# skygazer42/realtime-video-analytics-32streams

Hardware: AMD Instinct MI355X
Metric: aggregate detected FPS across streams + p99 per-frame latency, 32x1080p30 (higher is better)
Workload: dtype f16

## Files before the change

### include/rva.h

```cpp
#ifndef RVA_H
#define RVA_H

#include <stdint.h>

#ifdef __cplusplus
extern "C" {
#endif

#define RVA_ABI_VERSION 1

enum rva_status {
    RVA_OK = 0,
    RVA_ERR_ARG = 1,
    RVA_ERR_HIP = 2,
    RVA_ERR_CAPACITY = 3,
    RVA_ERR_UNAVAILABLE = 4
};

enum rva_dtype { RVA_F16 = 0, RVA_F32 = 1, RVA_F64 = 2  };

typedef struct rva_ctx rva_ctx;
typedef struct rva_tracker rva_tracker;
typedef void *rva_stream_t;

int rva_abi_version(void);
int rva_create(int device, rva_ctx **out);
void rva_destroy(rva_ctx *ctx);
const char *rva_last_error(const rva_ctx *ctx);

int rva_reserve(rva_ctx *ctx, int batch, int anchors);

typedef struct rva_letterbox {
    int32_t src_w, src_h;
    int32_t dst_w, dst_h;
    int32_t new_w, new_h;
    int32_t pad_left, pad_top;
    double scale;
} rva_letterbox;

int rva_letterbox_meta(int src_w, int src_h, int dst_w, int dst_h, rva_letterbox *out);

#define RVA_MAX_BATCH 64

int rva_preprocess_nv12_batch(rva_ctx *ctx, const void *const *y_ptrs, const void *const *uv_ptrs,
                              const int32_t *pitches, int n, int src_w, int src_h, void *out,
                              int out_dtype, int dst_w, int dst_h, rva_letterbox *meta_out,
                              rva_stream_t stream);

int rva_preprocess_nv12_content_batch(rva_ctx *ctx, const void *const *y_ptrs, const void *const *uv_ptrs,
                                      const int32_t *pitches, int n, int src_w, int src_h, void *out,
                                      int out_dtype, int dst_w, int dst_h, rva_letterbox *meta_out,
                                      rva_stream_t stream);

int rva_preprocess_bgr_batch(rva_ctx *ctx, const void *const *frames, const int32_t *row_bytes, int n,
                             int src_w, int src_h, void *out, int out_dtype, int dst_w, int dst_h,
                             rva_letterbox *meta_out, rva_stream_t stream);

int rva_profile_next_preprocess(rva_ctx *ctx, void *start_event, void *stop_event);

int rva_preprocess_clip_nv12_batch(rva_ctx *ctx, const void *const *y_ptrs, const void *const *uv_ptrs,
                                   const int32_t *pitches, int n, int src_w, int src_h, void *out,
                                   int out_dtype, int dst_w, int dst_h, rva_stream_t stream);

int rva_preprocess_clip_bgr_batch(rva_ctx *ctx, const void *const *frames, const int32_t *row_bytes,
                                  int n, int src_w, int src_h, void *out, int out_dtype, int dst_w,
                                  int dst_h, rva_stream_t stream);

enum rva_frame_norm { RVA_NORM_IMAGENET_F32 = 0, RVA_NORM_VIDEO_F32 = 1, RVA_NORM_IMAGENET_F64 = 2 };
enum rva_frame_layout { RVA_LAYOUT_NCHW = 0, RVA_LAYOUT_CNHW = 1 };
int rva_preprocess_frames_nv12_batch(rva_ctx *ctx, const void *const *y_ptrs, const void *const *uv_ptrs,
                                     const int32_t *pitches, int n, int src_w, int src_h, void *out,
                                     int out_dtype, int dst_w, int dst_h, int norm, int layout,
                                     rva_stream_t stream);
int rva_preprocess_frames_bgr_batch(rva_ctx *ctx, const void *const *frames, const int32_t *row_bytes,
                                    int n, int src_w, int src_h, void *out, int out_dtype, int dst_w,
                                    int dst_h, int norm, int layout, rva_stream_t stream);

int rva_postprocess_batch(rva_ctx *ctx, const void *raw, int raw_dtype, int batch, int d1, int d2,
                          double conf_thr, double iou_thr, const int32_t *classes, int n_classes,
                          const rva_letterbox *metas, int n_metas, int max_det, float *out_boxes,
                          float *out_scores, int32_t *out_cls, int32_t *out_anchor, int32_t *out_cand,
                          int32_t *out_counts, int32_t *out_ncand, rva_stream_t stream);

int rva_postprocess_boxes_batch(rva_ctx *ctx, const void *raw, int raw_dtype, const float *boxes, int batch, int channels,
                                int anchors, double conf_thr, double iou_thr, const int32_t *classes, int n_classes,
                                const rva_letterbox *metas, int n_metas, int max_det, float *out_boxes, float *out_scores,
                                int32_t *out_cls, int32_t *out_anchor, int32_t *out_cand, int32_t *out_counts,
                                int32_t *out_ncand, rva_stream_t stream);

int rva_post_status(rva_ctx *ctx, rva_stream_t stream, int *flags);

int rva_post_filter_stats(rva_ctx *ctx, rva_stream_t stream, int *binned_images);

int rva_tracker_create(rva_ctx *ctx, int n_streams, int capacity, int max_age, double max_iou_distance,
                       int min_hits, rva_tracker **out);
void rva_tracker_destroy(rva_tracker *trk);

int rva_tracker_update_f32(rva_tracker *trk, const int32_t *slot_of_stream, const float *boxes,
                           const float *scores, const int32_t *cls, const int32_t *counts, int max_det,
                           double filter_thr, rva_stream_t stream);

int rva_tracker_update_gated_f32(rva_tracker *trk, const int32_t *slot_of_stream, const float *boxes,
                                 const float *scores, const int32_t *cls, const int32_t *counts, int max_det,
                                 double filter_thr, const int32_t *motion_counts, const int32_t *motion_row,
                                 rva_stream_t stream);

int rva_tracker_set_gates(rva_tracker *trk, const int32_t *adaptive_enabled, const int32_t *max_process_every,
                          const int32_t *idle_tolerance, const int32_t *motion_min_count, int reset_state);

int rva_tracker_update_f64(rva_tracker *trk, const int32_t *active, const int32_t *offsets,
                           const double *boxes, const double *conf, const int64_t *cls,
                           rva_stream_t stream);

int rva_tracker_set_box_scale(rva_tracker *trk, const double *scales);

int32_t *rva_tracker_new_counts(rva_tracker *trk);

int rva_tracker_assign_ids(rva_tracker *trk, const int32_t *counts_all, int n_global,
                           const int32_t *global_index, rva_stream_t stream);

int rva_tracker_read(rva_tracker *trk, int stream_id, int cap, int64_t *ids, int32_t *cls, int32_t *age,
                     int32_t *hits, double *conf, double *boxes, int32_t *last_det, int32_t *n,
                     rva_stream_t stream);

int rva_tracker_read_all(rva_tracker *trk, int64_t *ids, int32_t *cls, int32_t *age, int32_t *hits,
                         double *conf, double *boxes, int32_t *last_det, int32_t *counts,
                         rva_stream_t stream);

#define RVA_SNAPSHOT_SLOTS 8
int rva_tracker_snapshot_async(rva_tracker *trk, int slot, rva_stream_t stream);
int rva_tracker_snapshot_fetch(rva_tracker *trk, int slot, int wait, int64_t *ids, int32_t *cls, int32_t *age,
                               int32_t *hits, double *conf, double *boxes, int32_t *last_det,
                               int32_t *counts);

int rva_tracker_snapshot_status(rva_tracker *trk, int slot, int32_t *emitted, int32_t *processed, int32_t *flags);

int rva_tracker_state(rva_tracker *trk, int64_t *next_id, int *flags, rva_stream_t stream);
int rva_tracker_set_next_id(rva_tracker *trk, int64_t next_id, rva_stream_t stream);

int rva_conv_cout_pad(int Cout);
int rva_conv_num_variants(void);
const char *rva_conv_variant_name(int variant);
int rva_conv2d_nhwc_f16(rva_ctx *ctx, const void *in, int ldi, const void *weights, const float *bias,
                        void *out, int ldo, const void *residual, int ldr, int batch, int H, int W, int Cin,
                        int Cout, int ksize, int stride, int act, rva_stream_t stream);
int rva_conv2d_nhwc_f16_v(rva_ctx *ctx, const void *in, int ldi, const void *weights, const float *bias,
                          void *out, int ldo, const void *residual, int ldr, int batch, int H, int W, int Cin,
                          int Cout, int ksize, int stride, int act, int variant, rva_stream_t stream);
int rva_conv2d_nhwc_f16_rows(rva_ctx *ctx, const void *in, int ldi, const void *weights, const float *bias,
                             void *out, int ldo, const void *residual, int ldr, int batch, int H, int W, int Cin,
                             int Cout, int ksize, int stride, int act, int variant, int y0, int y1, rva_stream_t stream);
int rva_conv_rows_through(int k, int stride, int H_in, int lo, int hi, int32_t *out_lo, int32_t *out_hi);
int rva_conv1x1_upcat_f16(rva_ctx *ctx, const void *low, int ld_low, int c_low, const void *skip, int ld_skip,
                          int c_skip, const void *weights, const float *bias, void *out, int ldo, int batch,
                          int H, int W, int Cout, int act, int variant, rva_stream_t stream);
int rva_conv1x1_head_f16(rva_ctx *ctx, const void *in, int ldi, const void *weights, const float *bias, int batch,
                         int H, int W, int Cin, int Cout, int mode, void *out, int nc, int anchors_total,
                         int anchor_offset, float stride_px, int variant, rva_stream_t stream);
int rva_conv1x1_head_box32_f16(rva_ctx *ctx, const void *in, int ldi, const void *weights, const float *bias, int batch,
                               int H, int W, int Cin, void *out, float *boxes32, int nc, int anchors_total, int anchor_offset,
                               float stride_px, int variant, rva_stream_t stream);
int rva_stem_conv_f16(rva_ctx *ctx, const void *in_planar, const void *weights, const float *bias,
                      void *out, int ldo, int batch, int H, int W, int Cout, rva_stream_t stream);

int rva_c2f_pair32_f16(rva_ctx *ctx, const void *in, int ldi, const void *w1, const float *b1, const void *w2, const float *b2, void *out,
                       int ldo, int batch, int H, int W, rva_stream_t stream);

int rva_stem2_f16(rva_ctx *ctx, const void *in_planar, const void *w1, const float *b1, const void *w2, const float *b2,
                  void *out, int ldo, int batch, int H, int W, rva_stream_t stream);
int rva_stem2_f16_rows(rva_ctx *ctx, const void *in_planar, const void *w1, const float *b1, const void *w2, const float *b2,
                       void *out, int ldo, int batch, int H, int W, int y0, int y1, rva_stream_t stream);

int rva_sppf_pool3_nhwc_f16(rva_ctx *ctx, const void *in, int ldi, void *out1, void *out2, void *out3, int ldo,
                            int batch, int H, int W, int C, rva_stream_t stream);
int rva_maxpool5_nhwc_f16(rva_ctx *ctx, const void *in, int ldi, void *out, int ldo, int batch, int H,
                          int W, int C, rva_stream_t stream);
int rva_upsample2x_nhwc_f16(rva_ctx *ctx, const void *in, int ldi, void *out, int ldo, int batch, int H,
                            int W, int C, rva_stream_t stream);
int rva_yolo_head_f16(rva_ctx *ctx, const void *box_logits, int ldb, const void *cls_logits, int ldc,
                      void *out, int batch, int h, int w, int nc, int anchors_total, int anchor_offset,
                      float stride, rva_stream_t stream);
int rva_yolo_head3_f16(rva_ctx *ctx, const void *const *box_logits, const int32_t *ldb, const void *const *cls_logits,
                       const int32_t *ldc, void *out, int batch, const int32_t *h, const int32_t *w, int nc,
                       int anchors_total, const float *strides, rva_stream_t stream);
int rva_yolo_head_box32_f16(rva_ctx *ctx, const void *box_logits, int ldb, const void *cls_logits, int ldc, void *out,
                            float *boxes32, int batch, int h, int w, int nc, int anchors_total, int anchor_offset, float stride,
                            rva_stream_t stream);
int rva_yolo_head3_box32_f16(rva_ctx *ctx, const void *const *box_logits, const int32_t *ldb, const void *const *cls_logits,
                             const int32_t *ldc, void *out, float *boxes32, int batch, const int32_t *h, const int32_t *w, int nc,
                             int anchors_total, const float *strides, rva_stream_t stream);

int rva_conv_f32_num_variants(void);
int rva_conv2d_nhwc_f32_v(rva_ctx *ctx, const void *in, int ldi, const void *weights, const float *bias,
                          void *out, int ldo, const void *residual, int ldr, int batch, int H, int W, int Cin,
                          int Cout, int ksize, int stride, int act, int variant, rva_stream_t stream);
int rva_stem_conv_f32(rva_ctx *ctx, const void *in_planar, const void *weights, const float *bias,
                      void *out, int ldo, int batch, int H, int W, int Cout, rva_stream_t stream);
int rva_maxpool5_nhwc_f32(rva_ctx *ctx, const void *in, int ldi, void *out, int ldo, int batch, int H,
                          int W, int C, rva_stream_t stream);
int rva_upsample2x_nhwc_f32(rva_ctx *ctx, const void *in, int ldi, void *out, int ldo, int batch, int H,
                            int W, int C, rva_stream_t stream);
int rva_yolo_head_f32(rva_ctx *ctx, const void *box_logits, int ldb, const void *cls_logits, int ldc,
                      void *out, int batch, int h, int w, int nc, int anchors_total, int anchor_offset,
                      float stride, rva_stream_t stream);

#define RVA_PLAN_NO_STEM2 1
#define RVA_PLAN_NO_CIN_PAD 2
#define RVA_PLAN_NO_PAIR32 4
#define RVA_PLAN_F32 8
#define RVA_PLAN_BOX_F32 16
typedef struct rva_yolov8_plan rva_yolov8_plan;
typedef struct rva_yolov8_desc {
    int32_t batch, height, width;
    int32_t widths[5];
    int32_t depth_backbone[4];
    int32_t depth_head;
    int32_t nc, reg_max;
    int32_t n_convs;
    int32_t flags;
} rva_yolov8_desc;
typedef struct rva_conv_weights {
    const float *weight;
    const float *bias;
    int32_t cout, cin, k, stride;
} rva_conv_weights;
int rva_yolov8_plan_create(rva_ctx *ctx, const rva_yolov8_desc *desc, const rva_conv_weights *convs, rva_yolov8_plan **out);
void rva_yolov8_plan_destroy(rva_yolov8_plan *plan);
int rva_yolov8_plan_info(const rva_yolov8_plan *plan, int32_t *anchors, int32_t *out_rows, int32_t *n_steps, int32_t *n_tunable,
                         int32_t *quiet_step);
int rva_yolov8_plan_output_layout(const rva_yolov8_plan *plan, int64_t *total_bytes, int64_t *boxes_offset);
int rva_yolov8_plan_run(rva_yolov8_plan *plan, const void *input, void *output, rva_stream_t stream);
int rva_yolov8_plan_run_lanes(rva_yolov8_plan *plan, const void *input, void *output, rva_stream_t stream, rva_stream_t side1,
                              rva_stream_t side2);
int rva_yolov8_plan_run_range(rva_yolov8_plan *plan, const void *input, void *output, int first, int last, rva_stream_t stream);
int rva_yolov8_plan_tunable_desc(const rva_yolov8_plan *plan, int index, char *buf, int len);
int rva_yolov8_plan_launch_tunable(rva_yolov8_plan *plan, int index, int variant, void *output, rva_stream_t stream);
int rva_yolov8_plan_set_variant(rva_yolov8_plan *plan, int index, int variant);
int rva_yolov8_plan_get_variant(const rva_yolov8_plan *plan, int index);
int rva_yolov8_plan_set_static_rows(rva_yolov8_plan *plan, int top, int bottom);
int rva_yolov8_plan_run_n(rva_yolov8_plan *plan, const void *input, void *output, int n, rva_stream_t stream);
int rva_yolov8_plan_run_lanes_n(rva_yolov8_plan *plan, const void *input, void *output, int n, rva_stream_t stream, rva_stream_t side1,
                                rva_stream_t side2);
int rva_yolov8_plan_run_range_n(rva_yolov8_plan *plan, const void *input, void *output, int n, int first, int last, rva_stream_t stream);
int rva_yolov8_plan_primed_images(const rva_yolov8_plan *plan);
int rva_yolov8_plan_step_rows(const rva_yolov8_plan *plan, int step, int32_t *y0, int32_t *y1);

typedef struct rva_cnnlstm_plan rva_cnnlstm_plan;
typedef struct rva_cnnlstm_desc {
    int32_t height, width;
    int32_t frames;
    int32_t hidden, classes;
    int32_t max_clips;
} rva_cnnlstm_desc;
typedef struct rva_cnnlstm_weights {
    const float *conv1_w, *conv1_b, *conv2_w, *conv2_b;
    const float *w_ih1, *b1, *w_hh1;
    const float *w_ih2, *w_hh2, *b2;
    const float *head_w, *head_b;
} rva_cnnlstm_weights;
int rva_cnnlstm_plan_create(rva_ctx *ctx, const rva_cnnlstm_desc *desc, const rva_cnnlstm_weights *weights, rva_cnnlstm_plan **out);
void rva_cnnlstm_plan_destroy(rva_cnnlstm_plan *plan);
int rva_cnnlstm_plan_info(const rva_cnnlstm_plan *plan, int32_t *pooled_h, int32_t *pooled_w, int32_t *conv2_tiles,
                          int32_t *n_launches);
int rva_cnnlstm_plan_run(rva_cnnlstm_plan *plan, const void *frames, const int32_t *frame_index, int n_clips, void *logits,
                         rva_stream_t stream);
int rva_cnnlstm_plan_run_post(rva_cnnlstm_plan *plan, const void *logits, const int32_t *rows, int n_rows, int max_det,
                              void *scores, void *cls, void *boxes, void *counts, rva_stream_t stream);
enum rva_cnnlstm_stage {
    RVA_CNNLSTM_STAGE_POOLED = 0, RVA_CNNLSTM_STAGE_PARTIAL = 1, RVA_CNNLSTM_STAGE_FEAT = 2, RVA_CNNLSTM_STAGE_GX = 3,
    RVA_CNNLSTM_STAGE_H1 = 4, RVA_CNNLSTM_STAGE_H2 = 5
};
int rva_cnnlstm_plan_stage(rva_cnnlstm_plan *plan, int stage, int n_clips, void *dst, int64_t dst_floats, int64_t *n_floats,
                           rva_stream_t stream);

typedef struct rva_cnnlstm_f16_plan rva_cnnlstm_f16_plan;
int rva_cnnlstm_f16_plan_create(rva_ctx *ctx, const rva_cnnlstm_desc *desc, const rva_cnnlstm_weights *weights,
                                rva_cnnlstm_f16_plan **out);
void rva_cnnlstm_f16_plan_destroy(rva_cnnlstm_f16_plan *plan);
int rva_cnnlstm_f16_plan_info(const rva_cnnlstm_f16_plan *plan, int32_t *pooled_h, int32_t *pooled_w, int32_t *conv2_tiles,
                              int32_t *n_launches);
int rva_cnnlstm_f16_plan_run(rva_cnnlstm_f16_plan *plan, const void *frames, const int32_t *frame_index, int n_clips, void *logits,
                             rva_stream_t stream);
int rva_cnnlstm_f16_plan_run_post(rva_cnnlstm_f16_plan *plan, const void *logits, const int32_t *rows, int n_rows, int max_det,
                                  void *scores, void *cls, void *boxes, void *counts, rva_stream_t stream);
int rva_cnnlstm_f16_plan_stage(rva_cnnlstm_f16_plan *plan, int stage, int n_clips, void *dst, int64_t dst_elems, int64_t *n_elems,
                               rva_stream_t stream);

typedef struct rva_cnn3d_plan rva_cnn3d_plan;
typedef struct rva_cnn3d_desc {
    int32_t height, width;
    int32_t frames;
    int32_t classes;
    int32_t max_clips;
} rva_cnn3d_desc;
typedef struct rva_cnn3d_weights {
    const float *conv1_w, *conv1_b, *conv2_w, *conv2_b, *conv3_w, *conv3_b;
    const float *head_w, *head_b;
} rva_cnn3d_weights;
int rva_cnn3d_plan_create(rva_ctx *ctx, const rva_cnn3d_desc *desc, const rva_cnn3d_weights *weights, rva_cnn3d_plan **out);
void rva_cnn3d_plan_destroy(rva_cnn3d_plan *plan);
int rva_cnn3d_plan_info(const rva_cnn3d_plan *plan, int32_t *pool1, int32_t *pool2, int32_t *tiles, int32_t *n_launches);
int rva_cnn3d_plan_run(rva_cnn3d_plan *plan, const void *frames, const int32_t *frame_index, int n_clips, void *logits,
                       rva_stream_t stream);
int rva_cnn3d_plan_run_post(rva_cnn3d_plan *plan, const void *logits, const int32_t *rows, int n_rows, int max_det,
                            void *scores, void *cls, void *boxes, void *counts, rva_stream_t stream);
enum rva_cnn3d_stage { RVA_CNN3D_STAGE_ACT1 = 0, RVA_CNN3D_STAGE_ACT2 = 1, RVA_CNN3D_STAGE_PARTIAL = 2, RVA_CNN3D_STAGE_FEAT = 3 };
int rva_cnn3d_plan_stage(rva_cnn3d_plan *plan, int stage, int n_clips, void *dst, int64_t dst_floats, int64_t *n_floats,
                         rva_stream_t stream);

typedef struct rva_cnn3d_f16_plan rva_cnn3d_f16_plan;
int rva_cnn3d_f16_plan_create(rva_ctx *ctx, const rva_cnn3d_desc *desc, const rva_cnn3d_weights *weights, rva_cnn3d_f16_plan **out);
void rva_cnn3d_f16_plan_destroy(rva_cnn3d_f16_plan *plan);
int rva_cnn3d_f16_plan_info(const rva_cnn3d_f16_plan *plan, int32_t *pool1, int32_t *pool2, int32_t *tiles, int32_t *n_launches);
int rva_cnn3d_f16_plan_run(rva_cnn3d_f16_plan *plan, const void *frames, const int32_t *frame_index, int n_clips, void *logits,
                           rva_stream_t stream);
int rva_cnn3d_f16_plan_run_post(rva_cnn3d_f16_plan *plan, const void *logits, const int32_t *rows, int n_rows, int max_det,
                                void *scores, void *cls, void *boxes, void *counts, rva_stream_t stream);
int rva_cnn3d_f16_plan_stage(rva_cnn3d_f16_plan *plan, int stage, int n_clips, void *dst, int64_t dst_elems, int64_t *n_elems,
                             rva_stream_t stream);

typedef struct rva_resnet_plan rva_resnet_plan;
typedef struct rva_resnet_desc {
    int32_t height, width;
    int32_t classes, top_k;
    int32_t max_frames;
} rva_resnet_desc;
typedef struct rva_resnet_conv {
    const float *w, *b;
} rva_resnet_conv;
typedef struct rva_resnet_weights {
    const float *stem_w, *stem_b;
    rva_resnet_conv conv[19];
    const float *head_w, *head_b;
} rva_resnet_weights;
int rva_resnet_plan_create(rva_ctx *ctx, const rva_resnet_desc *desc, const rva_resnet_weights *weights, rva_resnet_plan **out);
void rva_resnet_plan_destroy(rva_resnet_plan *plan);
int rva_resnet_plan_info(const rva_resnet_plan *plan, int32_t *maps, int64_t *workspace_bytes, int32_t *n_launches);
int rva_resnet_plan_run(rva_resnet_plan *plan, const void *frames, const int32_t *frame_index, int n, void *logits,
                        rva_stream_t stream);
int rva_resnet_plan_run_post(rva_resnet_plan *plan, const void *logits, const int32_t *rows, int n_rows, int max_det,
                             void *scores, void *cls, void *boxes, void *counts, rva_stream_t stream);
enum rva_resnet_stage {
    RVA_RESNET_STAGE_POOLED = 0, RVA_RESNET_STAGE_MID0 = 1, RVA_RESNET_STAGE_DOWN2 = 9, RVA_RESNET_STAGE_DOWN4 = 10,
    RVA_RESNET_STAGE_DOWN6 = 11, RVA_RESNET_STAGE_OUT0 = 12, RVA_RESNET_STAGE_FEAT = 20
};
int rva_resnet_plan_stage(rva_resnet_plan *plan, int stage, int n, void *dst, int64_t dst_floats, int64_t *n_floats,
                          rva_stream_t stream);

int rva_motion_nv12_batch(rva_ctx *ctx, const void *const *y_ptrs, const void *const *uv_ptrs,
                          const int32_t *pitches, const void *const *prev_blur, void *const *blur_out, int n,
                          int w, int h, int32_t *counts, rva_stream_t stream);
int rva_motion_nv12_masked_batch(rva_ctx *ctx, const void *const *y_ptrs, const void *const *uv_ptrs,
                                 const int32_t *pitches, const void *const *masks, const void *const *prev_blur,
                                 void *const *blur_out, int n, int w, int h, int32_t *counts, rva_stream_t stream);
int rva_motion_bgr_batch(rva_ctx *ctx, const void *const *frames, const int32_t *row_bytes,
                         const void *const *prev_blur, void *const *blur_out, int n, int w, int h, int32_t *counts,
                         rva_stream_t stream);

int rva_preprocess_nv12_masked_batch(rva_ctx *ctx, const void *const *y_ptrs, const void *const *uv_ptrs,
                                     const int32_t *pitches, const void *const *masks, int n, int src_w, int src_h,
                                     void *out, int out_dtype, int dst_w, int dst_h, rva_letterbox *meta_out,
                                     rva_stream_t stream);
int rva_resize_nv12_to_bgr_batch(rva_ctx *ctx, const void *const *y_ptrs, const void *const *uv_ptrs,
                                 const int32_t *pitches, const void *const *masks, int n, int src_w, int src_h,
                                 void *out_bgr, int dst_w, int dst_h, rva_stream_t stream);

int rva_preview_nv12(rva_ctx *ctx, const void *y, const void *uv, int pitch, int src_w, int src_h, int ratio,
                     void *out_bgr, int dst_w, int dst_h, const int32_t *rects, const uint8_t *colors, int n_rects,
                     const int32_t *glyphs, int n_glyphs, int glyph_scale, rva_stream_t stream);

typedef struct rva_preview_item {
    const void *y, *uv;
    void *out_bgr;
    int32_t pitch, src_w, src_h, ratio, dst_w, dst_h;
    int32_t rect_first, n_rects, glyph_first, n_glyphs;
} rva_preview_item;
int rva_preview_nv12_batch(rva_ctx *ctx, const void *table_host, void *table_dev, int64_t table_bytes, int n, int n_rects,
                           int n_glyphs, int glyph_scale, rva_stream_t stream);

typedef struct rva_decoder rva_decoder;
enum rva_codec { RVA_CODEC_H264 = 0, RVA_CODEC_HEVC = 1 };

int rva_decode_available(char *detail, int detail_len);

int rva_decoder_create(rva_ctx *ctx, int codec, int num_surfaces, rva_decoder **out);
void rva_decoder_destroy(rva_decoder *dec);

int rva_decoder_feed(rva_decoder *dec, const uint8_t *data, int size, int64_t pts, int end_of_stream);

int rva_decoder_next_frame(rva_decoder *dec, void **y, void **uv, int32_t *pitch, int32_t *width, int32_t *height,
                           int64_t *pts, int32_t *pic_index);
int rva_decoder_release(rva_decoder *dec, int pic_index);

int rva_jpeg_max_bytes(int width, int height);
int rva_jpeg_encode_bgr(rva_ctx *ctx, const void *bgr, int pitch, int width, int height, int quality, void *out,
                        int out_capacity, int32_t *out_size, rva_stream_t stream);
int rva_jpeg_status(rva_ctx *ctx, rva_stream_t stream, int *flags);

typedef struct rva_jpeg_batch rva_jpeg_batch;
int rva_jpeg_batch_create(rva_ctx *ctx, int max_images, int max_width, int max_height, rva_jpeg_batch **out);
void rva_jpeg_batch_destroy(rva_jpeg_batch *enc);
int rva_jpeg_batch_encode(rva_jpeg_batch *enc, int n, const void *const *bgr, const int32_t *pitch, const int32_t *width,
                          const int32_t *height, const int32_t *quality, void *out, int64_t out_capacity, int32_t *out_sizes,
                          rva_stream_t stream);

#ifdef __cplusplus
}
#endif
#endif
```

### realtime_video_analytics_32streams_amd/_native.py

```python
from __future__ import annotations

import ctypes as C
import os
import shutil
import subprocess
from pathlib import Path
from typing import Optional

PKG = Path(__file__).resolve().parent
ROOT = PKG.parent
CSRC = PKG / "csrc"
LIB_PATH = Path(os.environ["RVA_LIB_PATH"]) if os.environ.get("RVA_LIB_PATH") else PKG / "librva.so"
SOURCES = ["rva_ctx.hip", "rva_preprocess.hip", "rva_postprocess.hip", "rva_tracker.hip", "rva_conv.hip", "rva_conv_f32.hip", "rva_plan.hip", "rva_clip.hip",
           "rva_clip3d.hip", "rva_clip3d_f16.hip", "rva_clip_f16.hip", "rva_resnet.hip", "rva_gates.hip", "rva_decode.hip", "rva_preview.hip", "rva_jpeg.hip"]
HIPCC_FLAGS = ["--offload-arch=gfx950", "-O3", "-fPIC", "-shared", "-std=c++17", "-ffp-contract=off",
               "-Wall", "-Wno-unused-function"]

RVA_OK, RVA_ERR_ARG, RVA_ERR_HIP, RVA_ERR_CAPACITY, RVA_ERR_UNAVAILABLE = range(5)
RVA_F16, RVA_F32, RVA_F64 = 0, 1, 2
NORM_IMAGENET_F32, NORM_VIDEO_F32, NORM_IMAGENET_F64 = 0, 1, 2
LAYOUT_NCHW, LAYOUT_CNHW = 0, 1
RVA_MAX_BATCH = 64
RVA_CODEC_H264, RVA_CODEC_HEVC = 0, 1


class Letterbox(C.Structure):
    _fields_ = [("src_w", C.c_int32), ("src_h", C.c_int32), ("dst_w", C.c_int32), ("dst_h", C.c_int32),
                ("new_w", C.c_int32), ("new_h", C.c_int32), ("pad_left", C.c_int32), ("pad_top", C.c_int32),
                ("scale", C.c_double)]

    def as_meta(self) -> dict:
        return {"orig_shape": (self.src_h, self.src_w), "scale": self.scale, "pad": (self.pad_left, self.pad_top)}


class YoloV8Desc(C.Structure):
    _fields_ = [("batch", C.c_int32), ("height", C.c_int32), ("width", C.c_int32), ("widths", C.c_int32 * 5),
                ("depth_backbone", C.c_int32 * 4), ("depth_head", C.c_int32), ("nc", C.c_int32), ("reg_max", C.c_int32),
                ("n_convs", C.c_int32), ("flags", C.c_int32)]


class ConvWeights(C.Structure):
    _fields_ = [("weight", C.POINTER(C.c_float)), ("bias", C.POINTER(C.c_float)), ("cout", C.c_int32), ("cin", C.c_int32),
                ("k", C.c_int32), ("stride", C.c_int32)]


class CnnLstmDesc(C.Structure):
    _fields_ = [("height", C.c_int32), ("width", C.c_int32), ("frames", C.c_int32), ("hidden", C.c_int32), ("classes", C.c_int32),
                ("max_clips", C.c_int32)]


class CnnLstmWeights(C.Structure):
    NAMES = ("conv1_w", "conv1_b", "conv2_w", "conv2_b", "w_ih1", "b1", "w_hh1", "w_ih2", "w_hh2", "b2", "head_w", "head_b")
    _fields_ = [(n, C.POINTER(C.c_float)) for n in NAMES]


class Cnn3dDesc(C.Structure):
    _fields_ = [("height", C.c_int32), ("width", C.c_int32), ("frames", C.c_int32), ("classes", C.c_int32), ("max_clips", C.c_int32)]


class Cnn3dWeights(C.Structure):
    NAMES = ("conv1_w", "conv1_b", "conv2_w", "conv2_b", "conv3_w", "conv3_b", "head_w", "head_b")
    _fields_ = [(n, C.POINTER(C.c_float)) for n in NAMES]


class ResNetDesc(C.Structure):
    _fields_ = [("height", C.c_int32), ("width", C.c_int32), ("classes", C.c_int32), ("top_k", C.c_int32), ("max_frames", C.c_int32)]


class ResNetWeights(C.Structure):
    NAMES = ("stem_w", "stem_b") + tuple(f"c{i}_{x}" for i in range(19) for x in "wb") + ("head_w", "head_b")
    _fields_ = [(n, C.POINTER(C.c_float)) for n in NAMES]


class PreviewItem(C.Structure):
    _fields_ = [("y", C.c_void_p), ("uv", C.c_void_p), ("out_bgr", C.c_void_p)] + [
        (n, C.c_int32) for n in ("pitch", "src_w", "src_h", "ratio", "dst_w", "dst_h", "rect_first", "n_rects", "glyph_first", "n_glyphs")]


RVA_PLAN_NO_STEM2 = 1
RVA_PLAN_NO_CIN_PAD = 2
RVA_PLAN_NO_PAIR32 = 4
RVA_PLAN_F32 = 8
RVA_PLAN_BOX_F32 = 16


def _stale() -> bool:
    if not LIB_PATH.exists():
        return True
    t = LIB_PATH.stat().st_mtime
    deps = [CSRC / s for s in SOURCES] + [CSRC / "rva_internal.h", CSRC / "rva_mfma_f32.h", CSRC / "rva_mfma_f16.h", ROOT / "include" / "rva.h"]
    return any(d.exists() and d.stat().st_mtime > t for d in deps)


def build(force: bool = False, verbose: bool = False) -> Path:
    if not force and not _stale():
        return LIB_PATH
    hipcc = shutil.which("hipcc") or "/opt/rocm/bin/hipcc"
    if not Path(hipcc).exists():
        if LIB_PATH.exists():
            return LIB_PATH
        raise RuntimeError("hipcc not found and librva.so is not built")
    cmd = [hipcc, *HIPCC_FLAGS, f"-I{ROOT / 'include'}", "-o", str(LIB_PATH), *[str(CSRC / s) for s in SOURCES], "-ldl"]
    if verbose:
        print(" ".join(cmd))
    subprocess.check_call(cmd, cwd=str(CSRC))
    return LIB_PATH


_LIB: Optional[C.CDLL] = None
_P = C.c_void_p


def lib() -> C.CDLL:
    global _LIB
    if _LIB is not None:
        return _LIB
    if not LIB_PATH.exists():
        if os.environ.get("RVA_NO_AUTOBUILD"):
            raise RuntimeError(f"{LIB_PATH} is missing: run `python -c 'import __graft_entry__ as g; g.build()'`")
        build()
    try:
        L = C.CDLL(str(LIB_PATH))
    except OSError as exc:
        raise RuntimeError(f"cannot load {LIB_PATH}: {exc}. The HIP hot path has no CPU fallback.") from exc
    i32p, i64p, f32p, f64p = (C.POINTER(C.c_int32), C.POINTER(C.c_int64), C.POINTER(C.c_float), C.POINTER(C.c_double))
    pp = C.POINTER(_P)
    sig = {
        "rva_abi_version": (C.c_int, []),
        "rva_create": (C.c_int, [C.c_int, C.POINTER(_P)]),
        "rva_destroy": (None, [_P]),
        "rva_last_error": (C.c_char_p, [_P]),
        "rva_reserve": (C.c_int, [_P, C.c_int, C.c_int]),
        "rva_letterbox_meta": (C.c_int, [C.c_int] * 4 + [C.POINTER(Letterbox)]),
        "rva_preprocess_nv12_batch": (C.c_int, [_P, pp, pp, i32p, C.c_int, C.c_int, C.c_int, _P, C.c_int, C.c_int,
                                                C.c_int, C.POINTER(Letterbox), _P]),
        "rva_preprocess_nv12_content_batch": (C.c_int, [_P, pp, pp, i32p, C.c_int, C.c_int, C.c_int, _P, C.c_int, C.c_int,
                                                        C.c_int, C.POINTER(Letterbox), _P]),
        "rva_preprocess_bgr_batch": (C.c_int, [_P, pp, i32p, C.c_int, C.c_int, C.c_int, _P, C.c_int, C.c_int, C.c_int,
                                               C.POINTER(Letterbox), _P]),
        "rva_preprocess_clip_nv12_batch": (C.c_int, [_P, pp, pp, i32p, C.c_int, C.c_int, C.c_int, _P, C.c_int, C.c_int,
                                                     C.c_int, _P]),
        "rva_preprocess_clip_bgr_batch": (C.c_int, [_P, pp, i32p, C.c_int, C.c_int, C.c_int, _P, C.c_int, C.c_int,
                                                    C.c_int, _P]),
        "rva_profile_next_preprocess": (C.c_int, [_P, _P, _P]),
        "rva_preprocess_frames_nv12_batch": (C.c_int, [_P, pp, pp, i32p, C.c_int, C.c_int, C.c_int, _P, C.c_int, C.c_int,
                                                       C.c_int, C.c_int, C.c_int, _P]),
        "rva_preprocess_frames_bgr_batch": (C.c_int, [_P, pp, i32p, C.c_int, C.c_int, C.c_int, _P, C.c_int, C.c_int,
                                                      C.c_int, C.c_int, C.c_int, _P]),
        "rva_postprocess_batch": (C.c_int, [_P, _P, C.c_int, C.c_int, C.c_int, C.c_int, C.c_double, C.c_double, i32p,
                                            C.c_int, C.POINTER(Letterbox), C.c_int, C.c_int, _P, _P, _P, _P, _P, _P, _P,
                                            _P]),
        "rva_postprocess_boxes_batch": (C.c_int, [_P, _P, C.c_int, _P, C.c_int, C.c_int, C.c_int, C.c_double, C.c_double, i32p,
                                                  C.c_int, C.POINTER(Letterbox), C.c_int, C.c_int, _P, _P, _P, _P, _P, _P, _P,
                                                  _P]),
        "rva_post_status": (C.c_int, [_P, _P, C.POINTER(C.c_int)]),
        "rva_post_filter_stats": (C.c_int, [_P, _P, C.POINTER(C.c_int)]),
        "rva_tracker_create": (C.c_int, [_P, C.c_int, C.c_int, C.c_int, C.c_double, C.c_int, C.POINTER(_P)]),
        "rva_tracker_destroy": (None, [_P]),
        "rva_tracker_update_f32": (C.c_int, [_P, i32p, _P, _P, _P, _P, C.c_int, C.c_double, _P]),
        "rva_tracker_update_f64": (C.c_int, [_P, i32p, i32p, _P, _P, _P, _P]),
        "rva_tracker_update_gated_f32": (C.c_int, [_P, i32p, _P, _P, _P, _P, C.c_int, C.c_double, _P, i32p, _P]),
        "rva_tracker_set_gates": (C.c_int, [_P, i32p, i32p, i32p, i32p, C.c_int]),
        "rva_tracker_snapshot_status": (C.c_int, [_P, C.c_int, _P, _P, C.POINTER(C.c_int32)]),
        "rva_tracker_new_counts": (_P, [_P]),
        "rva_tracker_assign_ids": (C.c_int, [_P, _P, C.c_int, i32p, _P]),
        "rva_tracker_read": (C.c_int, [_P, C.c_int, C.c_int, _P, _P, _P, _P, _P, _P, _P, i32p, _P]),
        "rva_tracker_read_all": (C.c_int, [_P, _P, _P, _P, _P, _P, _P, _P, _P, _P]),
        "rva_tracker_snapshot_async": (C.c_int, [_P, C.c_int, _P]),
        "rva_tracker_snapshot_fetch": (C.c_int, [_P, C.c_int, C.c_int, _P, _P, _P, _P, _P, _P, _P, _P]),
        "rva_tracker_state": (C.c_int, [_P, i64p, C.POINTER(C.c_int), _P]),
        "rva_tracker_set_next_id": (C.c_int, [_P, C.c_int64, _P]),
        "rva_preview_nv12": (C.c_int, [_P, _P, _P, C.c_int, C.c_int, C.c_int, C.c_int, _P, C.c_int, C.c_int, _P, _P, C.c_int, _P, C.c_int,
                                       C.c_int, _P]),
        "rva_decode_available": (C.c_int, [C.c_char_p, C.c_int]),
        "rva_decoder_create": (C.c_int, [_P, C.c_int, C.c_int, C.POINTER(_P)]),
        "rva_decoder_destroy": (None, [_P]),
        "rva_decoder_feed": (C.c_int, [_P, C.c_char_p, C.c_int, C.c_int64, C.c_int]),
        "rva_decoder_next_frame": (C.c_int, [_P, C.POINTER(_P), C.POINTER(_P), i32p, i32p, i32p, i64p, i32p]),
        "rva_decoder_release": (C.c_int, [_P, C.c_int]),
        "rva_motion_nv12_batch": (C.c_int, [_P, pp, pp, i32p, pp, pp, C.c_int, C.c_int, C.c_int, _P, _P]),
        "rva_motion_nv12_masked_batch": (C.c_int, [_P, pp, pp, i32p, pp, pp, pp, C.c_int, C.c_int, C.c_int, _P, _P]),
        "rva_motion_bgr_batch": (C.c_int, [_P, pp, i32p, pp, pp, C.c_int, C.c_int, C.c_int, _P, _P]),
        "rva_preprocess_nv12_masked_batch": (C.c_int, [_P, pp, pp, i32p, pp, C.c_int, C.c_int, C.c_int, _P, C.c_int, C.c_int,
                                                       C.c_int, C.POINTER(Letterbox), _P]),
        "rva_resize_nv12_to_bgr_batch": (C.c_int, [_P, pp, pp, i32p, pp, C.c_int, C.c_int, C.c_int, _P, C.c_int, C.c_int, _P]),
        "rva_tracker_set_box_scale": (C.c_int, [_P, f64p]),
        "rva_conv_cout_pad": (C.c_int, [C.c_int]),
        "rva_conv_num_variants": (C.c_int, []),
        "rva_conv_variant_name": (C.c_char_p, [C.c_int]),
        "rva_conv2d_nhwc_f16": (C.c_int, [_P, _P, C.c_int, _P, _P, _P, C.c_int, _P, C.c_int] + [C.c_int] * 8 + [_P]),
        "rva_conv2d_nhwc_f16_v": (C.c_int, [_P, _P, C.c_int, _P, _P, _P, C.c_int, _P, C.c_int] + [C.c_int] * 9 + [_P]),
        "rva_conv2d_nhwc_f16_rows": (C.c_int, [_P, _P, C.c_int, _P, _P, _P, C.c_int, _P, C.c_int] + [C.c_int] * 11 + [_P]),
        "rva_conv_rows_through": (C.c_int, [C.c_int] * 5 + [i32p, i32p]),
        "rva_stem2_f16_rows": (C.c_int, [_P, _P, _P, _P, _P, _P, _P, C.c_int, C.c_int, C.c_int, C.c_int, C.c_int, C.c_int, _P]),
        "rva_stem_conv_f16": (C.c_int, [_P, _P, _P, _P, _P, C.c_int, C.c_int, C.c_int, C.c_int, C.c_int, _P]),
        "rva_stem2_f16": (C.c_int, [_P, _P, _P, _P, _P, _P, _P, C.c_int, C.c_int, C.c_int, C.c_int, _P]),
        "rva_c2f_pair32_f16": (C.c_int, [_P, _P, C.c_int, _P, _P, _P, _P, _P, C.c_int, C.c_int, C.c_int, C.c_int, _P]),
        "rva_conv1x1_head_f16": (C.c_int, [_P, _P, C.c_int, _P, _P, C.c_int, C.c_int, C.c_int, C.c_int, C.c_int, C.c_int, _P, C.c_int,
                                           C.c_int, C.c_int, C.c_float, C.c_int, _P]),
        "rva_conv1x1_head_box32_f16": (C.c_int, [_P, _P, C.c_int, _P, _P, C.c_int, C.c_int, C.c_int, C.c_int, _P, _P, C.c_int,
                                                 C.c_int, C.c_int, C.c_float, C.c_int, _P]),
        "rva_yolo_head_box32_f16": (C.c_int, [_P, _P, C.c_int, _P, C.c_int, _P, _P, C.c_int, C.c_int, C.c_int, C.c_int, C.c_int,
                                              C.c_int, C.c_float, _P]),
        "rva_yolo_head3_box32_f16": (C.c_int, [_P, pp, i32p, pp, i32p, _P, _P, C.c_int, i32p, i32p, C.c_int, C.c_int,
                                               C.POINTER(C.c_float), _P]),
        "rva_conv1x1_upcat_f16": (C.c_int, [_P, _P, C.c_int, C.c_int, _P, C.c_int, C.c_int, _P, _P, _P, C.c_int, C.c_int, C.c_int,
                                            C.c_int, C.c_int, C.c_int, C.c_int, _P]),
        "rva_yolo_head3_f16": (C.c_int, [_P, pp, i32p, pp, i32p, _P, C.c_int, i32p, i32p, C.c_int, C.c_int, C.POINTER(C.c_float), _P]),
        "rva_sppf_pool3_nhwc_f16": (C.c_int, [_P, _P, C.c_int, _P, _P, _P, C.c_int, C.c_int, C.c_int, C.c_int, C.c_int, _P]),
        "rva_maxpool5_nhwc_f16": (C.c_int, [_P, _P, C.c_int, _P, C.c_int, C.c_int, C.c_int, C.c_int, C.c_int, _P]),
        "rva_upsample2x_nhwc_f16": (C.c_int, [_P, _P, C.c_int, _P, C.c_int, C.c_int, C.c_int, C.c_int, C.c_int, _P]),
        "rva_yolo_head_f16": (C.c_int, [_P, _P, C.c_int, _P, C.c_int, _P, C.c_int, C.c_int, C.c_int, C.c_int, C.c_int,
                                        C.c_int, C.c_float, _P]),
        "rva_conv_f32_num_variants": (C.c_int, []),
        "rva_conv2d_nhwc_f32_v": (C.c_int, [_P, _P, C.c_int, _P, _P, _P, C.c_int, _P, C.c_int] + [C.c_int] * 9 + [_P]),
        "rva_stem_conv_f32": (C.c_int, [_P, _P, _P, _P, _P, C.c_int, C.c_int, C.c_int, C.c_int, C.c_int, _P]),
        "rva_maxpool5_nhwc_f32": (C.c_int, [_P, _P, C.c_int, _P, C.c_int, C.c_int, C.c_int, C.c_int, C.c_int, _P]),
        "rva_upsample2x_nhwc_f32": (C.c_int, [_P, _P, C.c_int, _P, C.c_int, C.c_int, C.c_int, C.c_int, C.c_int, _P]),
        "rva_yolo_head_f32": (C.c_int, [_P, _P, C.c_int, _P, C.c_int, _P, C.c_int, C.c_int, C.c_int, C.c_int, C.c_int,
                                        C.c_int, C.c_float, _P]),
        "rva_yolov8_plan_create": (C.c_int, [_P, C.POINTER(YoloV8Desc), C.POINTER(ConvWeights), C.POINTER(_P)]),
        "rva_yolov8_plan_destroy": (None, [_P]),
        "rva_yolov8_plan_info": (C.c_int, [_P, i32p, i32p, i32p, i32p, i32p]),
        "rva_yolov8_plan_output_layout": (C.c_int, [_P, i64p, i64p]),
        "rva_yolov8_plan_run": (C.c_int, [_P, _P, _P, _P]),
        "rva_yolov8_plan_run_lanes": (C.c_int, [_P, _P, _P, _P, _P, _P]),
        "rva_yolov8_plan_run_range": (C.c_int, [_P, _P, _P, C.c_int, C.c_int, _P]),
        "rva_yolov8_plan_tunable_desc": (C.c_int, [_P, C.c_int, C.c_char_p, C.c_int]),
        "rva_yolov8_plan_launch_tunable": (C.c_int, [_P, C.c_int, C.c_int, _P, _P]),
        "rva_yolov8_plan_set_variant": (C.c_int, [_P, C.c_int, C.c_int]),
        "rva_yolov8_plan_get_variant": (C.c_int, [_P, C.c_int]),
        "rva_yolov8_plan_set_static_rows": (C.c_int, [_P, C.c_int, C.c_int]),
        "rva_yolov8_plan_step_rows": (C.c_int, [_P, C.c_int, i32p, i32p]),
        "rva_yolov8_plan_run_n": (C.c_int, [_P, _P, _P, C.c_int, _P]),
        "rva_yolov8_plan_run_lanes_n": (C.c_int, [_P, _P, _P, C.c_int, _P, _P, _P]),
        "rva_yolov8_plan_run_range_n": (C.c_int, [_P, _P, _P, C.c_int, C.c_int, C.c_int, _P]),
        "rva_yolov8_plan_primed_images": (C.c_int, [_P]),
        "rva_cnnlstm_plan_create": (C.c_int, [_P, C.POINTER(CnnLstmDesc), C.POINTER(CnnLstmWeights), C.POINTER(_P)]),
        "rva_cnnlstm_plan_destroy": (None, [_P]),
        "rva_cnnlstm_plan_info": (C.c_int, [_P, i32p, i32p, i32p, i32p]),
        "rva_cnnlstm_plan_run": (C.c_int, [_P, _P, _P, C.c_int, _P, _P]),
        "rva_cnnlstm_plan_run_post": (C.c_int, [_P, _P, _P, C.c_int, C.c_int, _P, _P, _P, _P, _P]),
        "rva_cnnlstm_plan_stage": (C.c_int, [_P, C.c_int, C.c_int, _P, C.c_int64, i64p, _P]),
        "rva_cnnlstm_f16_plan_create": (C.c_int, [_P, C.POINTER(CnnLstmDesc), C.POINTER(CnnLstmWeights), C.POINTER(_P)]),
        "rva_cnnlstm_f16_plan_destroy": (None, [_P]),
        "rva_cnnlstm_f16_plan_info": (C.c_int, [_P, i32p, i32p, i32p, i32p]),
        "rva_cnnlstm_f16_plan_run": (C.c_int, [_P, _P, _P, C.c_int, _P, _P]),
        "rva_cnnlstm_f16_plan_run_post": (C.c_int, [_P, _P, _P, C.c_int, C.c_int, _P, _P, _P, _P, _P]),
        "rva_cnnlstm_f16_plan_stage": (C.c_int, [_P, C.c_int, C.c_int, _P, C.c_int64, i64p, _P]),
        "rva_cnn3d_plan_create": (C.c_int, [_P, C.POINTER(Cnn3dDesc), C.POINTER(Cnn3dWeights), C.POINTER(_P)]),
        "rva_cnn3d_plan_destroy": (None, [_P]),
        "rva_cnn3d_plan_info": (C.c_int, [_P, i32p, i32p, i32p, i32p]),
        "rva_cnn3d_plan_run": (C.c_int, [_P, _P, _P, C.c_int, _P, _P]),
        "rva_cnn3d_plan_run_post": (C.c_int, [_P, _P, _P, C.c_int, C.c_int, _P, _P, _P, _P, _P]),
        "rva_cnn3d_plan_stage": (C.c_int, [_P, C.c_int, C.c_int, _P, C.c_int64, i64p, _P]),
        "rva_cnn3d_f16_plan_create": (C.c_int, [_P, C.POINTER(Cnn3dDesc), C.POINTER(Cnn3dWeights), C.POINTER(_P)]),
        "rva_cnn3d_f16_plan_destroy": (None, [_P]),
        "rva_cnn3d_f16_plan_info": (C.c_int, [_P, i32p, i32p, i32p, i32p]),
        "rva_cnn3d_f16_plan_run": (C.c_int, [_P, _P, _P, C.c_int, _P, _P]),
        "rva_cnn3d_f16_plan_run_post": (C.c_int, [_P, _P, _P, C.c_int, C.c_int, _P, _P, _P, _P, _P]),
        "rva_cnn3d_f16_plan_stage": (C.c_int, [_P, C.c_int, C.c_int, _P, C.c_int64, i64p, _P]),
        "rva_resnet_plan_create": (C.c_int, [_P, C.POINTER(ResNetDesc), C.POINTER(ResNetWeights), C.POINTER(_P)]),
        "rva_resnet_plan_destroy": (None, [_P]),
        "rva_resnet_plan_info": (C.c_int, [_P, i32p, i64p, i32p]),
        "rva_resnet_plan_run": (C.c_int, [_P, _P, _P, C.c_int, _P, _P]),
        "rva_resnet_plan_run_post": (C.c_int, [_P, _P, _P, C.c_int, C.c_int, _P, _P, _P, _P, _P]),
        "rva_resnet_plan_stage": (C.c_int, [_P, C.c_int, C.c_int, _P, C.c_int64, i64p, _P]),
        "rva_jpeg_max_bytes": (C.c_int, [C.c_int, C.c_int]),
        "rva_jpeg_encode_bgr": (C.c_int, [_P, _P, C.c_int, C.c_int, C.c_int, C.c_int, _P, C.c_int, _P, _P]),
        "rva_jpeg_status": (C.c_int, [_P, _P, C.POINTER(C.c_int)]),
        "rva_jpeg_batch_create": (C.c_int, [_P, C.c_int, C.c_int, C.c_int, C.POINTER(_P)]),
        "rva_jpeg_batch_destroy": (None, [_P]),
        "rva_jpeg_batch_encode": (C.c_int, [_P, C.c_int, pp, i32p, i32p, i32p, i32p, _P, C.c_int64, _P, _P]),
        "rva_preview_nv12_batch": (C.c_int, [_P, _P, _P, C.c_int64, C.c_int, C.c_int, C.c_int, C.c_int, _P]),
    }
    for name, (res, args) in sig.items():
        fn = getattr(L, name)
        fn.restype = res
        fn.argtypes = args
    if L.rva_abi_version() != 1:
        raise RuntimeError("librva.so ABI version mismatch; rebuild it")
    _LIB = L
    return L


EXPORTS = [
    "rva_abi_version", "rva_create", "rva_destroy", "rva_last_error", "rva_reserve", "rva_letterbox_meta",
    "rva_preprocess_nv12_batch", "rva_preprocess_nv12_content_batch", "rva_preprocess_bgr_batch", "rva_preprocess_clip_nv12_batch",
    "rva_preprocess_clip_bgr_batch", "rva_profile_next_preprocess", "rva_preprocess_frames_nv12_batch", "rva_preprocess_frames_bgr_batch", "rva_postprocess_batch", "rva_post_status", "rva_post_filter_stats", "rva_tracker_create",
    "rva_tracker_destroy", "rva_tracker_update_f32", "rva_tracker_update_f64", "rva_tracker_update_gated_f32",
    "rva_tracker_set_gates", "rva_tracker_snapshot_status", "rva_tracker_new_counts",
    "rva_tracker_assign_ids", "rva_tracker_read", "rva_tracker_read_all", "rva_tracker_snapshot_async",
    "rva_tracker_snapshot_fetch", "rva_tracker_state",
    "rva_tracker_set_next_id", "rva_preview_nv12", "rva_decode_available", "rva_decoder_create", "rva_decoder_destroy", "rva_decoder_feed",
    "rva_decoder_next_frame", "rva_decoder_release", "rva_motion_nv12_batch", "rva_motion_nv12_masked_batch", "rva_motion_bgr_batch",
    "rva_preprocess_nv12_masked_batch", "rva_resize_nv12_to_bgr_batch", "rva_tracker_set_box_scale", "rva_conv_cout_pad", "rva_conv_num_variants", "rva_conv_variant_name", "rva_conv2d_nhwc_f16", "rva_conv2d_nhwc_f16_v", "rva_stem_conv_f16", "rva_stem2_f16", "rva_c2f_pair32_f16",
    "rva_conv1x1_head_f16", "rva_conv1x1_upcat_f16", "rva_sppf_pool3_nhwc_f16", "rva_maxpool5_nhwc_f16", "rva_upsample2x_nhwc_f16", "rva_yolo_head_f16", "rva_yolo_head3_f16",
    "rva_conv_f32_num_variants", "rva_conv2d_nhwc_f32_v", "rva_stem_conv_f32", "rva_maxpool5_nhwc_f32", "rva_upsample2x_nhwc_f32",
    "rva_yolo_head_f32",
    "rva_postprocess_boxes_batch", "rva_conv1x1_head_box32_f16", "rva_yolo_head_box32_f16", "rva_yolo_head3_box32_f16",
    "rva_yolov8_plan_output_layout",
    "rva_yolov8_plan_create", "rva_yolov8_plan_destroy", "rva_yolov8_plan_info", "rva_yolov8_plan_run", "rva_yolov8_plan_run_lanes",
    "rva_yolov8_plan_run_range", "rva_yolov8_plan_tunable_desc", "rva_yolov8_plan_launch_tunable", "rva_yolov8_plan_set_variant",
    "rva_yolov8_plan_get_variant", "rva_yolov8_plan_set_static_rows", "rva_yolov8_plan_step_rows", "rva_yolov8_plan_run_n",
    "rva_yolov8_plan_run_lanes_n", "rva_yolov8_plan_run_range_n", "rva_yolov8_plan_primed_images", "rva_conv2d_nhwc_f16_rows",
    "rva_stem2_f16_rows", "rva_conv_rows_through", "rva_cnnlstm_plan_create", "rva_cnnlstm_plan_destroy", "rva_cnnlstm_plan_info", "rva_cnnlstm_plan_run",
    "rva_cnnlstm_plan_run_post", "rva_cnnlstm_plan_stage", "rva_cnnlstm_f16_plan_create", "rva_cnnlstm_f16_plan_destroy", "rva_cnnlstm_f16_plan_info",
    "rva_cnnlstm_f16_plan_run", "rva_cnnlstm_f16_plan_run_post", "rva_cnnlstm_f16_plan_stage", "rva_cnn3d_plan_create", "rva_cnn3d_plan_destroy", "rva_cnn3d_plan_info", "rva_cnn3d_plan_run",
    "rva_cnn3d_plan_run_post", "rva_cnn3d_plan_stage", "rva_cnn3d_f16_plan_create", "rva_cnn3d_f16_plan_destroy", "rva_cnn3d_f16_plan_info",
    "rva_cnn3d_f16_plan_run", "rva_cnn3d_f16_plan_run_post", "rva_cnn3d_f16_plan_stage", "rva_resnet_plan_create", "rva_resnet_plan_destroy", "rva_resnet_plan_info",
    "rva_resnet_plan_run", "rva_resnet_plan_run_post", "rva_resnet_plan_stage", "rva_jpeg_max_bytes", "rva_jpeg_encode_bgr", "rva_jpeg_status",
    "rva_jpeg_batch_create", "rva_jpeg_batch_destroy", "rva_jpeg_batch_encode", "rva_preview_nv12_batch",
]


class Context:

    def __init__(self, device: int = 0):
        L = lib()
        h = _P()
        rc = L.rva_create(device, C.byref(h))
        if rc != RVA_OK or not h:
            raise RuntimeError(
                f"rva_create(device={device}) failed with status {rc}: no usable HIP device. "
                "The MI355X hot path has no CPU fallback.")
        self.handle = h
        self.device = device

    def check(self, rc: int, what: str = "") -> None:
        if rc != RVA_OK:
            msg = lib().rva_last_error(self.handle)
            raise RuntimeError(f"{what or 'librva'} failed (status {rc}): {msg.decode() if msg else ''}")

    def close(self) -> None:
        if getattr(self, "handle", None):
            lib().rva_destroy(self.handle)
            self.handle = None

    def __del__(self):
        try:
            self.close()
        except Exception:
            pass


def letterbox(src_w: int, src_h: int, dst_w: int, dst_h: int) -> Letterbox:
    m = Letterbox()
    rc = lib().rva_letterbox_meta(src_w, src_h, dst_w, dst_h, C.byref(m))
    if rc != RVA_OK:
        raise ValueError(f"bad letterbox geometry {(src_w, src_h)} -> {(dst_w, dst_h)}")
    return m


def ptr_array(ptrs):
    arr = (_P * len(ptrs))(*[_P(int(p)) for p in ptrs])
    return C.cast(arr, C.POINTER(_P)), arr


def i32_array(vals):
    arr = (C.c_int32 * len(vals))(*[int(v) for v in vals])
    return C.cast(arr, C.POINTER(C.c_int32)), arr
```

### realtime_video_analytics_32streams_amd/csrc/rva_internal.h

```cpp
#pragma once

#include <hip/hip_runtime.h>

#include <algorithm>
#include <cstdarg>
#include <cstdint>
#include <cstdio>
#include <map>
#include <string>
#include <vector>

#include "rva.h"

struct rva_resize_table {
    int32_t *ofs = nullptr;
    int16_t *w0 = nullptr;
    int16_t *w1 = nullptr;
    int n = 0;
};

struct rva_geom_cache {
    rva_resize_table x, y;
};

struct rva_jpeg_state;

struct rva_ctx {
    int device = 0;
    rva_jpeg_state *jpeg = nullptr;
    std::string err;
    int cap_batch = 0, cap_anchors = 0;
    float *sp_box = nullptr;
    float *sp_score = nullptr;
    int32_t *sp_cls = nullptr;
    uint32_t *cand_bits = nullptr;
    int32_t *post_flags = nullptr;
    std::map<uint64_t, rva_resize_table> taps_x, taps_y;
    hipEvent_t k1_start = nullptr, k1_stop = nullptr;
    int k1_px = -1;
    int k1_nt = -1;
    int num_cus = 0;
};

inline int rva_fail(rva_ctx *ctx, int code, const char *fmt, ...)
{
    char buf[512];
    va_list ap;
    va_start(ap, fmt);
    vsnprintf(buf, sizeof buf, fmt, ap);
    va_end(ap);
    if (ctx) ctx->err = buf;
    return code;
}

#define RVA_HIP(ctx, call)                                                                          \
    do {                                                                                            \
        hipError_t e_ = (call);                                                                     \
        if (e_ != hipSuccess)                                                                       \
            return rva_fail((ctx), RVA_ERR_HIP, "%s failed: %s (%s:%d)", #call, hipGetErrorString(e_), \
                            __FILE__, __LINE__);                                                    \
    } while (0)

int rva_get_taps(rva_ctx *ctx, int src, int dst, bool is_x, rva_resize_table *out);

static inline int rva_ceil_div(int a, int b) { return (a + b - 1) / b; }

hipError_t rva_func_smem(const void *fn, size_t bytes);

int rva_num_cus(rva_ctx *ctx);

bool rva_conv_variant_is_gather64(int variant);
bool rva_conv_variant_rows(int variant, int Cin, int ksize, int stride);

int rva_conv2d_nhwc_f16_sel(rva_ctx *ctx, const void *in, int ldi, const void *weights, const float *bias, void *out, int ldo,
                            const void *residual, int ldr, int batch, int sel_batch, int H, int W, int Cin, int Cout, int ksize, int stride,
                            int act, int variant, int y0, int y1, rva_stream_t stream);

void rva_jpeg_free(rva_ctx *ctx);

struct rva_dev_arena {
    std::vector<void *> allocs;

    int alloc(rva_ctx *ctx, float **dst, size_t n)
    {
        void *m = nullptr;
        RVA_HIP(ctx, hipMalloc(&m, std::max<size_t>(n, 1) * sizeof(float)));
        allocs.push_back(m);
        *dst = (float *)m;
        return RVA_OK;
    }

    int upload(rva_ctx *ctx, float **dst, const float *src, size_t n)
    {
        const int rc = alloc(ctx, dst, n);
        if (rc != RVA_OK) return rc;
        RVA_HIP(ctx, hipMemcpy(*dst, src, n * sizeof(float), hipMemcpyHostToDevice));
        return RVA_OK;
    }

    void release()
    {
        for (void *m : allocs) (void)hipFree(m);
        allocs.clear();
    }
};

int rva_clip_stem_prepare(rva_ctx *ctx);
int rva_clip_stem_launch(rva_ctx *ctx, const float *frames, const int32_t *frame_index, const float *w1, const float *b1, float *pooled,
                         int H, int W, int n_frames, hipStream_t st);
int rva_clip_mean_launch(rva_ctx *ctx, const float *partial, int tiles, float n, float *feat, int rows, int channels, hipStream_t st);
int rva_clip_head_prepare(rva_ctx *ctx, int hidden);
int rva_clip_head_launch(rva_ctx *ctx, const float *x, const float *wh, const float *bh, float *logits, int hidden, int classes,
                         int n_clips, hipStream_t st);
int rva_clip_post_prepare(rva_ctx *ctx, int classes);
int rva_clip_post_launch(rva_ctx *ctx, const char *who, const float *logits, int classes, int k, const int32_t *rows, int n_rows,
                         int max_det, float *scores, int32_t *cls, float *boxes, int32_t *counts, hipStream_t st);

int rva_clip_stage_copy(rva_ctx *ctx, const char *who, int stage, int n_clips, const float *src, int64_t count, int64_t rows,
                        int64_t row_floats, int64_t pitch_floats, void *dst, int64_t dst_floats, int64_t *n_floats, hipStream_t st);
```

### realtime_video_analytics_32streams_amd/csrc/rva_plan.hip

```cpp
#include <cstring>
#include <memory>

#include "rva_internal.h"

namespace {

enum StepKind { K_CONV, K_UPCAT, K_HEAD, K_STEM2, K_STEM, K_SPPF3, K_POOL5, K_UP2, K_HEAD3, K_PAIR32,
                K_CONV_F32, K_STEM_F32, K_POOL5_F32, K_UP2_F32, K_HEAD_F32 };

struct View {
    char *base = nullptr; int ld = 0, off = 0, ch = 0, es = 2;
    void *ptr() const { return base + (size_t)es * off; }
    View sub(int o, int c) const { View v = *this; v.off += o; v.ch = c; return v; }
};

struct Step {
    StepKind kind;
    int lane = 0;
    int tunable = -1;
    const void *in = nullptr, *in2 = nullptr; int ldi = 0, ldi2 = 0, c_in = 0, c_in2 = 0;
    const void *w = nullptr, *w2 = nullptr; const float *b = nullptr, *b2 = nullptr;
    void *out = nullptr, *out2 = nullptr, *out3 = nullptr; int ldo = 0;
    const void *res = nullptr; int ldr = 0;
    int H = 0, W = 0, Cin = 0, Cout = 0, k = 0, stride = 0, act = 0, variant = 0;
    int mode = 0, a0 = 0; float stride_px = 0.f;
    int c_real = 0;
    int Ho = 0, y0 = 0, y1 = 0;
    const void *hb[3] = {nullptr, nullptr, nullptr}, *hk[3] = {nullptr, nullptr, nullptr};
    int32_t hldb[3] = {0, 0, 0}, hldc[3] = {0, 0, 0}, hh[3] = {0, 0, 0}, hw[3] = {0, 0, 0}; float hs[3] = {0, 0, 0};
};

struct Tunable { int step; std::string base, desc; };

}

struct rva_yolov8_plan {
    rva_ctx *ctx = nullptr;
    rva_yolov8_desc d{};
    int B = 0, H = 0, W = 0, nc = 0, A = 0;
    std::vector<void *> allocs;
    std::vector<Step> steps;
    std::vector<Tunable> tunables;
    int fork_step[3] = {-1, -1, -1};
    int quiet_step = 0;
    hipEvent_t fork_ev[3] = {nullptr, nullptr, nullptr}, join_ev[3] = {nullptr, nullptr, nullptr};
    bool fused_stem = false, fused_head = false;
    bool f32 = false;
    bool box32 = false;
    size_t box_off = 0;
    int rows_top = 0, rows_bottom = 0;
    bool windowed = false;
    int primed = 0;
};

namespace {

struct Builder {
    rva_yolov8_plan *p;
    const rva_conv_weights *convs;
    int next = 0;
    int lane = 0;
    std::string err;

    bool fail(const std::string &m) { if (err.empty()) err = m; return false; }

    void *dev_alloc(size_t bytes, bool zero)
    {
        void *ptr = nullptr;
        if (hipMalloc(&ptr, bytes ? bytes : 16) != hipSuccess) { fail("hipMalloc failed"); return nullptr; }
        p->allocs.push_back(ptr);
        if (zero && hipMemset(ptr, 0, bytes) != hipSuccess) { fail("hipMemset failed"); return nullptr; }
        return ptr;
    }
    View buf(long m, int ch)
    {
        View v;
        v.es = p->f32 ? 4 : 2;
        v.base = (char *)dev_alloc((size_t)m * ch * v.es + 64, true);
        v.ld = ch; v.off = 0; v.ch = ch;
        return v;
    }
    bool upload(const void *host, size_t bytes, const void **dev)
    {
        void *d = dev_alloc(bytes, false);
        if (!d) return false;
        if (hipMemcpy(d, host, bytes, hipMemcpyHostToDevice) != hipSuccess) return fail("weight upload failed");
        *dev = d;
        return true;
    }
    bool pack_f32(const rva_conv_weights *const *cv, int n, const void **w_dev, const float **b_dev, int *cin, int *cout, int *k, int *stride)
    {
        const rva_conv_weights &c0 = *cv[0];
        int co = 0;
        for (int i = 0; i < n; ++i) {
            if (!cv[i]->weight || cv[i]->cin != c0.cin || cv[i]->k != c0.k || cv[i]->stride != c0.stride) return fail("sibling convolutions differ");
            co += cv[i]->cout;
        }
        const int kk = c0.k * c0.k;
        std::vector<float> hw((size_t)co * kk * c0.cin, 0.f), hb(co, 0.f);
        int o = 0;
        for (int i = 0; i < n; ++i) {
            const rva_conv_weights &c = *cv[i];
            for (int oc = 0; oc < c.cout; ++oc) {
                for (int ic = 0; ic < c.cin; ++ic)
                    for (int t = 0; t < kk; ++t)
                        hw[((size_t)(o + oc) * kk + t) * c.cin + ic] = c.weight[((size_t)oc * c.cin + ic) * kk + t];
                if (c.bias) hb[o + oc] = c.bias[oc];
            }
            o += c.cout;
        }
        const void *db = nullptr;
        if (!upload(hw.data(), hw.size() * 4, w_dev) || !upload(hb.data(), hb.size() * 4, &db)) return false;
        *b_dev = (const float *)db; *cin = c0.cin; *cout = co; *k = c0.k; *stride = c0.stride;
        return true;
    }
    bool pack(const rva_conv_weights *const *cv, int n, const void **w_dev, const float **b_dev, int *cin, int *cout, int *k, int *stride)
    {
        const rva_conv_weights &c0 = *cv[0];
        int co = 0;
        for (int i = 0; i < n; ++i) {
            if (!cv[i]->weight || cv[i]->cin != c0.cin || cv[i]->k != c0.k || cv[i]->stride != c0.stride) return fail("sibling convolutions differ");
            co += cv[i]->cout;
        }
        const int kk = c0.k * c0.k, cpad = rva_conv_cout_pad(co), cinp = (c0.cin + 31) / 32 * 32;
        std::vector<_Float16> hw((size_t)cpad * kk * cinp, (_Float16)0.f);
        std::vector<float> hb(cpad, 0.f);
        int o = 0;
        for (int i = 0; i < n; ++i) {
            const rva_conv_weights &c = *cv[i];
            for (int oc = 0; oc < c.cout; ++oc) {
                for (int ic = 0; ic < c.cin; ++ic)
                    for (int t = 0; t < kk; ++t)
                        hw[((size_t)(o + oc) * kk + t) * cinp + ic] = (_Float16)c.weight[((size_t)oc * c.cin + ic) * kk + t];
                if (c.bias) hb[o + oc] = c.bias[oc];
            }
            o += c.cout;
        }
        void *dw = dev_alloc(hw.size() * 2, false), *db = dev_alloc(hb.size() * 4, false);
        if (!dw || !db) return false;
        if (hipMemcpy(dw, hw.data(), hw.size() * 2, hipMemcpyHostToDevice) != hipSuccess ||
            hipMemcpy(db, hb.data(), hb.size() * 4, hipMemcpyHostToDevice) != hipSuccess) return fail("weight upload failed");
        *w_dev = dw; *b_dev = (const float *)db; *cin = c0.cin; *cout = co; *k = c0.k; *stride = c0.stride;
        return true;
    }
    const rva_conv_weights *take(int cin, int cout, int k, int stride, const char *what)
    {
        if (next >= p->d.n_convs) { fail(std::string("convolution list too short at ") + what); return nullptr; }
        const rva_conv_weights *c = &convs[next++];
        if (c->cin != cin || c->cout != cout || c->k != k || c->stride != stride) {
            char m[200];
            snprintf(m, sizeof m, "convolution %d (%s): expected %d->%d k%d s%d, got %d->%d k%d s%d", next - 1, what, cin, cout, k, stride,
                     c->cin, c->cout, c->k, c->stride);
            fail(m);
            return nullptr;
        }
        return c;
    }
    void push(Step &s, const char *desc_fmt, ...)
    {
        s.lane = lane;
        if (desc_fmt) {
            char d[96];
            va_list ap; va_start(ap, desc_fmt); vsnprintf(d, sizeof d, desc_fmt, ap); va_end(ap);
            s.tunable = (int)p->tunables.size();
            p->tunables.push_back(Tunable{(int)p->steps.size(), d, d});
        }
        p->steps.push_back(s);
    }
    bool conv(const rva_conv_weights *const *cv, int n, View src, View dst, int h, int w, int act, const View *res = nullptr)
    {
        Step s{}; s.kind = p->f32 ? K_CONV_F32 : K_CONV;
        const bool packed = p->f32 ? pack_f32(cv, n, &s.w, &s.b, &s.Cin, &s.Cout, &s.k, &s.stride)
                                   : pack(cv, n, &s.w, &s.b, &s.Cin, &s.Cout, &s.k, &s.stride);
        if (!packed) return false;
        if (s.Cin != src.ch || s.Cout != dst.ch) return fail("convolution does not fit its buffers");
        s.in = src.ptr(); s.ldi = src.ld; s.out = dst.ptr(); s.ldo = dst.ld; s.H = h; s.W = w; s.act = act;
        if (res) { s.res = res->ptr(); s.ldr = res->ld; }
        const int cin_real = s.Cin;
        s.c_real = cin_real;
        if (p->f32) {
            if (s.Cin % 16) return fail("fp32 plan: convolution input channels must be multiples of 16");
            push(s, "%d->%d k%ds%d %dx%d", cin_real, s.Cout, s.k, s.stride, h, w);
            return true;
        }
        if (s.Cin % 32 && !(p->d.flags & RVA_PLAN_NO_CIN_PAD)) s.Cin = (s.Cin + 31) / 32 * 32;
        push(s, "%d->%d k%ds%d %dx%d", cin_real, s.Cout, s.k, s.stride, h, w);
        return true;
    }
    bool conv1(const rva_conv_weights *c, View src, View dst, int h, int w, int act, const View *res = nullptr)
    {
        return c && conv(&c, 1, src, dst, h, w, act, res);
    }
    bool upcat(const rva_conv_weights *c, View low, View skip, View dst, int h, int w)
    {
        if (!c) return false;
        Step s{}; s.kind = K_UPCAT;
        if (!pack(&c, 1, &s.w, &s.b, &s.Cin, &s.Cout, &s.k, &s.stride)) return false;
        if (s.k != 1 || s.stride != 1 || s.Cin != low.ch + skip.ch || s.Cout != dst.ch) return fail("upsample + concat convolution does not fit");
        s.in = low.ptr(); s.ldi = low.ld; s.c_in = low.ch; s.in2 = skip.ptr(); s.ldi2 = skip.ld; s.c_in2 = skip.ch;
        s.out = dst.ptr(); s.ldo = dst.ld; s.H = h; s.W = w; s.act = 1;
        push(s, "up%d+%d->%d k1s1 %dx%d", low.ch, skip.ch, s.Cout, h, w);
        return true;
    }
    bool head(const rva_conv_weights *c, View src, int mode, int h, int w, int a0, float stride_px)
    {
        if (!c) return false;
        Step s{}; s.kind = K_HEAD;
        if (!pack(&c, 1, &s.w, &s.b, &s.Cin, &s.Cout, &s.k, &s.stride)) return false;
        if (s.k != 1 || s.stride != 1 || s.Cin != src.ch) return fail("head convolution does not fit");
        s.in = src.ptr(); s.ldi = src.ld; s.H = h; s.W = w; s.mode = mode; s.a0 = a0; s.stride_px = stride_px;
        push(s, "head%d:%d->%d k1s1 %dx%d", mode, s.Cin, s.Cout, h, w);
        return true;
    }
    bool c2f(int c1, int c2, int n, bool shortcut, const View *src, const View *low, const View *skip, View dst, int h, int w, const char *what)
    {
        const int c = c2 / 2;
        const long m = (long)p->B * h * w;
        const rva_conv_weights *cv1 = take(c1, 2 * c, 1, 1, what), *cv2 = take((2 + n) * c, c2, 1, 1, what);
        if (!cv1 || !cv2) return false;
        View cat = buf(m, (2 + n) * c);
        if (!cat.base) return false;
        if (low) { if (!upcat(cv1, *low, *skip, cat.sub(0, 2 * c), h, w)) return false; }
        else if (!conv1(cv1, *src, cat.sub(0, 2 * c), h, w, 1)) return false;
        for (int i = 0; i < n; ++i) {
            const rva_conv_weights *b1 = take(c, c, 3, 1, what), *b2 = take(c, c, 3, 1, what);
            View x = cat.sub((1 + i) * c, c);
            if (c == 32 && shortcut && !p->f32 && !(p->d.flags & RVA_PLAN_NO_PAIR32)) {
                Step s{}; s.kind = K_PAIR32;
                int ci, co, kk, st;
                if (!pack(&b1, 1, &s.w, &s.b, &ci, &co, &kk, &st) || !pack(&b2, 1, &s.w2, &s.b2, &ci, &co, &kk, &st)) return false;
                View y = cat.sub((2 + i) * c, c);
                s.in = x.ptr(); s.ldi = x.ld; s.out = y.ptr(); s.ldo = y.ld; s.H = h; s.W = w; s.Cin = s.Cout = c; s.k = 3; s.stride = 1; s.act = 1;
                push(s, nullptr);
                continue;
            }
            View tmp = buf(m, c);
            if (!tmp.base) return false;
            if (!conv1(b1, x, tmp, h, w, 1)) return false;
            if (!conv1(b2, tmp, cat.sub((2 + i) * c, c), h, w, 1, shortcut ? &x : nullptr)) return false;
        }
        return conv1(cv2, cat, dst, h, w, 1);
    }

    bool build()
    {
        const rva_yolov8_desc &d = p->d;
        const int B = d.batch, H = d.height, W = d.width;
        const int c1 = d.widths[0], c2 = d.widths[1], c3 = d.widths[2], c4 = d.widths[3], c5 = d.widths[4];
        const int h1 = H / 2, w1 = W / 2, h2 = H / 4, w2 = W / 4, h3 = H / 8, w3 = W / 8, h4 = H / 16, w4 = W / 16, h5 = H / 32, w5 = W / 32;
        const int nh = d.depth_head;
        const rva_conv_weights *b0 = take(3, c1, 3, 2, "b0"), *b1 = take(c1, c2, 3, 2, "b1");
        if (!b0 || !b1) return false;
        View x1;
        if (p->f32) {
            Step s{}; s.kind = K_STEM_F32;
            std::vector<float> sb(c1, 0.f);
            if (b0->bias) memcpy(sb.data(), b0->bias, sizeof(float) * c1);
            const void *db = nullptr;
            if (!b0->weight || !upload(b0->weight, sizeof(float) * c1 * 27, &s.w) || !upload(sb.data(), sizeof(float) * c1, &db)) return false;
            s.b = (const float *)db;
            View x0 = buf((long)B * h1 * w1, c1);
            x1 = buf((long)B * h2 * w2, c2);
            if (!x0.base || !x1.base) return false;
            s.out = x0.ptr(); s.ldo = x0.ld; s.H = H; s.W = W; s.Cout = c1;
            push(s, nullptr);
            if (!conv1(b1, x0, x1, h1, w1, 1)) return false;
        } else {
            if (c1 > 64) return fail("stem wider than 64 channels");
            std::vector<_Float16> sw(64 * 32, (_Float16)0.f);
            std::vector<float> sb(64, 0.f);
            for (int co = 0; co < c1; ++co) {
                for (int j = 0; j < 9; ++j)
                    for (int kx = 0; kx < 3; ++kx) {
                        const float v = b0->weight[((size_t)co * 3 + j / 3) * 9 + (j % 3) * 3 + kx];
                        sw[co * 32 + (kx < 2 ? 2 * j + kx : 18 + j)] = (_Float16)v;
                    }
                if (b0->bias) sb[co] = b0->bias[co];
            }
            void *dsw = dev_alloc(sw.size() * 2, false), *dsb = dev_alloc(sb.size() * 4, false);
            if (!dsw || !dsb) return false;
            if (hipMemcpy(dsw, sw.data(), sw.size() * 2, hipMemcpyHostToDevice) != hipSuccess ||
                hipMemcpy(dsb, sb.data(), sb.size() * 4, hipMemcpyHostToDevice) != hipSuccess) return fail("stem upload failed");
            x1 = buf((long)B * h2 * w2, c2);
            if (!x1.base) return false;
            p->fused_stem = c1 == 32 && c2 == 64 && !(d.flags & RVA_PLAN_NO_STEM2);
            if (p->fused_stem) {
                Step s{}; s.kind = K_STEM2; s.w = dsw; s.b = (const float *)dsb; s.out = x1.ptr(); s.ldo = x1.ld; s.H = H; s.W = W;
                int ci, co, k, st;
                if (!pack(&b1, 1, &s.w2, &s.b2, &ci, &co, &k, &st)) return false;
                push(s, nullptr);
            } else {
                View x0 = buf((long)B * h1 * w1, c1);
                if (!x0.base) return false;
                Step s{}; s.kind = K_STEM; s.w = dsw; s.b = (const float *)dsb; s.out = x0.ptr(); s.ldo = x0.ld; s.H = H; s.W = W; s.Cout = c1;
                push(s, nullptr);
                if (!conv1(b1, x0, x1, h1, w1, 1)) return false;
            }
        }
        View x2 = buf((long)B * h2 * w2, c2);
        if (!x2.base || !c2f(c2, c2, d.depth_backbone[0], true, &x1, nullptr, nullptr, x2, h2, w2, "b2")) return false;
        View cat15 = buf((long)B * h3 * w3, c4 + c3), cat12 = buf((long)B * h4 * w4, c5 + c4), cat18 = buf((long)B * h4 * w4, c3 + c4),
             cat21 = buf((long)B * h5 * w5, c4 + c5);
        if (!cat15.base || !cat12.base || !cat18.base || !cat21.base) return false;
        View p3 = cat15.sub(c4, c3), p4 = cat12.sub(c5, c4), n4 = cat18.sub(c3, c4), p5 = cat21.sub(c4, c5);
        View t3 = buf((long)B * h3 * w3, c3);
        if (!t3.base || !conv1(take(c2, c3, 3, 2, "b3"), x2, t3, h2, w2, 1)) return false;
        if (!c2f(c3, c3, d.depth_backbone[1], true, &t3, nullptr, nullptr, p3, h3, w3, "b4")) return false;
        View t4 = buf((long)B * h4 * w4, c4);
        if (!t4.base || !conv1(take(c3, c4, 3, 2, "b5"), p3, t4, h3, w3, 1)) return false;
        if (!c2f(c4, c4, d.depth_backbone[2], true, &t4, nullptr, nullptr, p4, h4, w4, "b6")) return false;
        View t5 = buf((long)B * h5 * w5, c5);
        p->quiet_step = (int)p->steps.size();
        if (!t5.base || !conv1(take(c4, c5, 3, 2, "b7"), p4, t5, h4, w4, 1)) return false;
        View t5b = buf((long)B * h5 * w5, c5);
        if (!t5b.base || !c2f(c5, c5, d.depth_backbone[3], true, &t5, nullptr, nullptr, t5b, h5, w5, "b8")) return false;
        {
            const int c_ = c5 / 2;
            const rva_conv_weights *cv1 = take(c5, c_, 1, 1, "b9.cv1"), *cv2 = take(4 * c_, c5, 1, 1, "b9.cv2");
            View cat = buf((long)B * h5 * w5, 4 * c_);
            if (!cat.base || !conv1(cv1, t5b, cat.sub(0, c_), h5, w5, 1)) return false;
            if (h5 * w5 <= 2400 && !p->f32) {
                Step s{}; s.kind = K_SPPF3; s.in = cat.sub(0, c_).ptr(); s.ldi = cat.ld; s.out = cat.sub(c_, c_).ptr(); s.out2 = cat.sub(2 * c_, c_).ptr();
                s.out3 = cat.sub(3 * c_, c_).ptr(); s.ldo = cat.ld; s.H = h5; s.W = w5; s.Cin = c_;
                push(s, nullptr);
            } else {
                for (int i = 0; i < 3; ++i) {
                    Step s{}; s.kind = p->f32 ? K_POOL5_F32 : K_POOL5; s.in = cat.sub(i * c_, c_).ptr(); s.ldi = cat.ld; s.out = cat.sub((i + 1) * c_, c_).ptr(); s.ldo = cat.ld;
                    s.H = h5; s.W = w5; s.Cin = c_;
                    push(s, nullptr);
                }
            }
            if (!conv1(cv2, cat, p5, h5, w5, 1)) return false;
        }
        const bool fuse_up = !p->f32 && c5 % 64 == 0 && c4 % 64 == 0 && c3 % 64 == 0 && h4 == 2 * h5 && w4 == 2 * w5 && h3 == 2 * h4 && w3 == 2 * w4;
        View n3 = buf((long)B * h3 * w3, c3);
        if (!n3.base) return false;
        if (fuse_up) {
            if (!c2f(c5 + c4, c4, nh, false, nullptr, &p5, &p4, n4, h4, w4, "h12")) return false;
            if (!c2f(c4 + c3, c3, nh, false, nullptr, &n4, &p3, n3, h3, w3, "h15")) return false;
        } else {
            Step u1{}; u1.kind = p->f32 ? K_UP2_F32 : K_UP2; u1.in = p5.ptr(); u1.ldi = p5.ld; u1.out = cat12.sub(0, c5).ptr(); u1.ldo = cat12.ld; u1.H = h5; u1.W = w5; u1.Cin = c5;
            push(u1, nullptr);
            if (!c2f(c5 + c4, c4, nh, false, &cat12, nullptr, nullptr, n4, h4, w4, "h12")) return false;
            Step u2{}; u2.kind = p->f32 ? K_UP2_F32 : K_UP2; u2.in = n4.ptr(); u2.ldi = n4.ld; u2.out = cat15.sub(0, c4).ptr(); u2.ldo = cat15.ld; u2.H = h4; u2.W = w4; u2.Cin = c4;
            push(u2, nullptr);
            if (!c2f(c4 + c3, c3, nh, false, &cat15, nullptr, nullptr, n3, h3, w3, "h15")) return false;
        }
        const int fork_n3 = (int)p->steps.size();
        if (!conv1(take(c3, c3, 3, 2, "h16"), n3, cat18.sub(0, c3), h3, w3, 1)) return false;
        View m4 = buf((long)B * h4 * w4, c4);
        if (!m4.base || !c2f(c3 + c4, c4, nh, false, &cat18, nullptr, nullptr, m4, h4, w4, "h18")) return false;
        const int fork_m4 = (int)p->steps.size();
        if (!conv1(take(c4, c4, 3, 2, "h19"), m4, cat21.sub(0, c4), h4, w4, 1)) return false;
        View m5 = buf((long)B * h5 * w5, c5);
        if (!m5.base || !c2f(c4 + c5, c5, nh, false, &cat21, nullptr, nullptr, m5, h5, w5, "h21")) return false;
        const int rm4 = 4 * d.reg_max;
        int cb = c3 / 4 > rm4 ? c3 / 4 : rm4;
        if (cb < 16) cb = 16;
        int cc = c3 > (d.nc < 100 ? d.nc : 100) ? c3 : (d.nc < 100 ? d.nc : 100);
        p->A = h3 * w3 + h4 * w4 + h5 * w5;
        const rva_conv_weights *box[3][3], *cls[3][3];
        const int chs[3] = {c3, c4, c5};
        for (int l = 0; l < 3; ++l) {
            box[l][0] = take(chs[l], cb, 3, 1, "detect.box.0"); box[l][1] = take(cb, cb, 3, 1, "detect.box.1"); box[l][2] = take(cb, rm4, 1, 1, "detect.box.2");
            if (!box[l][0] || !box[l][1] || !box[l][2]) return false;
        }
        for (int l = 0; l < 3; ++l) {
            cls[l][0] = take(chs[l], cc, 3, 1, "detect.cls.0"); cls[l][1] = take(cc, cc, 3, 1, "detect.cls.1"); cls[l][2] = take(cc, d.nc, 1, 1, "detect.cls.2");
            if (!cls[l][0] || !cls[l][1] || !cls[l][2]) return false;
        }
        if (next != d.n_convs) return fail("convolution list longer than the architecture");
        p->fused_head = !p->f32 && cb % 64 == 0 && cc % 64 == 0 && rm4 == 64 && d.nc % 8 == 0;
        const View feats[3] = {n3, m4, m5};
        const int hs[3] = {h3, h4, h5}, ws[3] = {w3, w4, w5};
        const float strides[3] = {8.f, 16.f, 32.f};
        Step h3s{}; h3s.kind = K_HEAD3;
        int a0 = 0;
        for (int l = 0; l < 3; ++l) {
            lane = ((p->fused_head || p->f32) && l < 2) ? l + 1 : 0;
            if (lane) p->fork_step[lane] = l == 0 ? fork_n3 : fork_m4;
            const long m = (long)B * hs[l] * ws[l];
            View first = buf(m, cb + cc), b2 = buf(m, cb), k2 = buf(m, cc);
            if (!first.base || !b2.base || !k2.base) return false;
            const rva_conv_weights *sib[2] = {box[l][0], cls[l][0]};
            if (!conv(sib, 2, feats[l], first, hs[l], ws[l], 1)) return false;
            if (p->fused_head) {
                if (!conv1(box[l][1], first.sub(0, cb), b2, hs[l], ws[l], 1) || !head(box[l][2], b2, 1, hs[l], ws[l], a0, strides[l])) return false;
                if (!conv1(cls[l][1], first.sub(cb, cc), k2, hs[l], ws[l], 1) || !head(cls[l][2], k2, 2, hs[l], ws[l], a0, strides[l])) return false;
            } else {
                View bo = buf(m, rm4), ko = buf(m, d.nc);
                if (!bo.base || !ko.base) return false;
                if (!conv1(box[l][1], first.sub(0, cb), b2, hs[l], ws[l], 1) || !conv1(box[l][2], b2, bo, hs[l], ws[l], 0)) return false;
                if (!conv1(cls[l][1], first.sub(cb, cc), k2, hs[l], ws[l], 1) || !conv1(cls[l][2], k2, ko, hs[l], ws[l], 0)) return false;
                h3s.hb[l] = bo.ptr(); h3s.hldb[l] = bo.ld; h3s.hk[l] = ko.ptr(); h3s.hldc[l] = ko.ld; h3s.hh[l] = hs[l]; h3s.hw[l] = ws[l]; h3s.hs[l] = strides[l];
                if (p->f32) {
                    Step hs1{}; hs1.kind = K_HEAD_F32; hs1.in = bo.ptr(); hs1.ldi = bo.ld; hs1.in2 = ko.ptr(); hs1.ldi2 = ko.ld;
                    hs1.H = hs[l]; hs1.W = ws[l]; hs1.a0 = a0; hs1.stride_px = strides[l];
                    push(hs1, nullptr);
                }
            }
            a0 += hs[l] * ws[l];
        }
        lane = 0;
        if (!p->fused_head && !p->f32) push(h3s, nullptr);
        return err.empty();
    }
};

bool step_takes_rows(const Step &s, int variant)
{
    if (s.kind == K_STEM2) return true;
    return s.kind == K_CONV && rva_conv_variant_rows(variant, s.Cin, s.k, s.stride);
}

int launch_step(rva_yolov8_plan *p, const Step &s, int variant, const void *input, void *output, int n, rva_stream_t st, bool win)
{
    rva_ctx *c = p->ctx;
    if (win && (s.y0 > 0 || s.y1 < s.Ho) && step_takes_rows(s, variant)) {
        if (s.kind == K_STEM2) return rva_stem2_f16_rows(c, input, s.w, s.b, s.w2, s.b2, s.out, s.ldo, n, s.H, s.W, s.y0, s.y1, st);
        return rva_conv2d_nhwc_f16_sel(c, s.in, s.ldi, s.w, s.b, s.out, s.ldo, s.res, s.ldr, n, p->B, s.H, s.W, s.Cin, s.Cout, s.k, s.stride, s.act,
                                       variant, s.y0, s.y1, st);
    }
    if (p->box32 && output) {
        float *boxes = (float *)((char *)output + p->box_off);
        if (s.kind == K_HEAD && s.mode == 1)
            return rva_conv1x1_head_box32_f16(c, s.in, s.ldi, s.w, s.b, n, s.H, s.W, s.Cin, output, boxes, p->nc, p->A, s.a0, s.stride_px, variant, st);
        if (s.kind == K_HEAD3)
            return rva_yolo_head3_box32_f16(c, s.hb, s.hldb, s.hk, s.hldc, output, boxes, n, s.hh, s.hw, p->nc, p->A, s.hs, st);
    }
    switch (s.kind) {
    case K_CONV: return rva_conv2d_nhwc_f16_sel(c, s.in, s.ldi, s.w, s.b, s.out, s.ldo, s.res, s.ldr, n, p->B, s.H, s.W, s.Cin, s.Cout, s.k, s.stride, s.act, variant,
                                                0, -1, st);
    case K_UPCAT: return rva_conv1x1_upcat_f16(c, s.in, s.ldi, s.c_in, s.in2, s.ldi2, s.c_in2, s.w, s.b, s.out, s.ldo, n, s.H, s.W, s.Cout, s.act, variant, st);
    case K_HEAD: return rva_conv1x1_head_f16(c, s.in, s.ldi, s.w, s.b, n, s.H, s.W, s.Cin, s.Cout, s.mode, output, p->nc, p->A, s.a0, s.stride_px, variant, st);
    case K_PAIR32: return rva_c2f_pair32_f16(c, s.in, s.ldi, s.w, s.b, s.w2, s.b2, s.out, s.ldo, n, s.H, s.W, st);
    case K_STEM2: return rva_stem2_f16(c, input, s.w, s.b, s.w2, s.b2, s.out, s.ldo, n, s.H, s.W, st);
    case K_STEM: return rva_stem_conv_f16(c, input, s.w, s.b, s.out, s.ldo, n, s.H, s.W, s.Cout, st);
    case K_SPPF3: return rva_sppf_pool3_nhwc_f16(c, s.in, s.ldi, s.out, s.out2, s.out3, s.ldo, n, s.H, s.W, s.Cin, st);
    case K_POOL5: return rva_maxpool5_nhwc_f16(c, s.in, s.ldi, s.out, s.ldo, n, s.H, s.W, s.Cin, st);
    case K_UP2: return rva_upsample2x_nhwc_f16(c, s.in, s.ldi, s.out, s.ldo, n, s.H, s.W, s.Cin, st);
    case K_HEAD3: return rva_yolo_head3_f16(c, s.hb, s.hldb, s.hk, s.hldc, output, n, s.hh, s.hw, p->nc, p->A, s.hs, st);
    case K_CONV_F32: return rva_conv2d_nhwc_f32_v(c, s.in, s.ldi, s.w, s.b, s.out, s.ldo, s.res, s.ldr, n, s.H, s.W, s.Cin, s.Cout, s.k, s.stride, s.act, variant, st);
    case K_STEM_F32: return rva_stem_conv_f32(c, input, s.w, s.b, s.out, s.ldo, n, s.H, s.W, s.Cout, st);
    case K_POOL5_F32: return rva_maxpool5_nhwc_f32(c, s.in, s.ldi, s.out, s.ldo, n, s.H, s.W, s.Cin, st);
    case K_UP2_F32: return rva_upsample2x_nhwc_f32(c, s.in, s.ldi, s.out, s.ldo, n, s.H, s.W, s.Cin, st);
    case K_HEAD_F32: return rva_yolo_head_f32(c, s.in, s.ldi, s.in2, s.ldi2, output, n, s.H, s.W, p->nc, p->A, s.a0, s.stride_px, st);
    }
    return RVA_ERR_ARG;
}

bool variant_fits(const Step &s, int variant)
{
    if (s.kind == K_CONV) return variant >= 0;
    if (s.kind == K_CONV_F32) return variant >= 0 && variant <= rva_conv_f32_num_variants();
    return variant == 0 || rva_conv_variant_is_gather64(variant);
}

int out_rows(int H, int k, int stride) { return (H + 2 * (k / 2) - k) / stride + 1; }

void propagate_rows(rva_yolov8_plan *p)
{
    struct Slice { const char *lo, *hi; int H, y0, y1; };
    std::vector<Slice> written;
    const int es = p->f32 ? 4 : 2;
    const bool off = p->f32 || (p->rows_top <= 0 && p->rows_bottom >= p->H);
    auto read = [&](const void *ptr, int ch, int H, int *lo, int *hi) {
        const char *a = (const char *)ptr, *b = a + (size_t)ch * es;
        long covered = 0;
        int y0 = H, y1 = 0;
        for (const Slice &w : written) {
            const char *l = w.lo > a ? w.lo : a, *h = w.hi < b ? w.hi : b;
            if (l >= h) continue;
            if (w.H != H) return false;
            covered += h - l;
            if (w.y0 < y0) y0 = w.y0;
            if (w.y1 > y1) y1 = w.y1;
        }
        if (covered != b - a || y0 >= y1) return false;
        *lo = y0; *hi = y1;
        return true;
    };
    auto through = [](int k, int stride, int H, int *lo, int *hi) {
        int32_t a = 0, b = 0;
        (void)rva_conv_rows_through(k, stride, H, *lo, *hi, &a, &b);
        *lo = a; *hi = b;
        return out_rows(H, k, stride);
    };
    p->windowed = false;
    for (Step &s : p->steps) {
        int lo = 0, hi = 0, Ho = s.H;
        bool known = false;
        switch (s.kind) {
        case K_STEM2: case K_STEM:
            lo = p->rows_top; hi = p->rows_bottom; known = true;
            Ho = through(3, 2, s.H, &lo, &hi);
            if (s.kind == K_STEM2) Ho = through(3, 2, Ho, &lo, &hi);
            break;
        case K_CONV:
            known = read(s.in, s.c_real, s.H, &lo, &hi);
            Ho = out_rows(s.H, s.k, s.stride);
            if (known) {
                (void)through(s.k, s.stride, s.H, &lo, &hi);
                int rl = 0, rh = 0;
                if (s.res) {
                    known = read(s.res, s.Cout, Ho, &rl, &rh);
                    if (rl < lo) lo = rl;
                    if (rh > hi) hi = rh;
                }
            }
            break;
        case K_PAIR32:
            known = read(s.in, 32, s.H, &lo, &hi);
            if (known) { (void)through(3, 1, s.H, &lo, &hi); (void)through(3, 1, s.H, &lo, &hi); }
            break;
        case K_UPCAT: {
            int l2 = 0, h2 = 0;
            known = read(s.in, s.c_in, s.H / 2, &lo, &hi) && read(s.in2, s.c_in2, s.H, &l2, &h2);
            lo = 2 * lo < l2 ? 2 * lo : l2;
            hi = 2 * hi > h2 ? 2 * hi : h2;
            break;
        }
        default: break;
        }
        s.Ho = Ho;
        if (off || !known || lo >= hi) { lo = 0; hi = Ho; }
        s.y0 = lo; s.y1 = hi;
        if (lo > 0 || hi < Ho) p->windowed = true;
        if (s.kind == K_STEM2 || s.kind == K_STEM || s.kind == K_CONV || s.kind == K_PAIR32 || s.kind == K_UPCAT) {
            const int ch = s.kind == K_STEM2 ? 64 : s.kind == K_PAIR32 ? 32 : s.Cout;
            written.push_back(Slice{(const char *)s.out, (const char *)s.out + (size_t)ch * es, Ho, lo, hi});
        }
    }
    for (Tunable &t : p->tunables) {
        const Step &s = p->steps[t.step];
        t.desc = t.base;
        if (s.y0 > 0 || s.y1 < s.Ho) {
            char w[32];
            snprintf(w, sizeof w, " r[%d,%d)", s.y0, s.y1);
            t.desc += w;
        }
    }
    p->primed = 0;
}

bool stream_is_capturing(rva_stream_t stream)
{
    hipStreamCaptureStatus cs = hipStreamCaptureStatusNone;
    if (hipStreamIsCapturing((hipStream_t)stream, &cs) != hipSuccess) { (void)hipGetLastError(); return false; }
    return cs != hipStreamCaptureStatusNone;
}

int run_steps(rva_yolov8_plan *p, const void *input, void *output, int n, int first, int last, rva_stream_t stream, bool win)
{
    for (int i = first; i < last; ++i) {
        const Step &s = p->steps[i];
        const int rc = launch_step(p, s, s.variant, input, output, n, stream, win);
        if (rc != RVA_OK) return rc;
    }
    return RVA_OK;
}

int check_run(rva_yolov8_plan *p, const void *input, void *output, int n)
{
    if (!p || !input || !output) return RVA_ERR_ARG;
    if (n <= 0 || n > p->B) return rva_fail(p->ctx, RVA_ERR_ARG, "rva_yolov8_plan_run: n = %d is not 1 .. %d, the plan's capacity", n, p->B);
    if (((uintptr_t)input | (uintptr_t)output) % 16) return rva_fail(p->ctx, RVA_ERR_ARG, "rva_yolov8_plan_run: input and output must be 16-byte aligned");
    return RVA_OK;
}

void note_complete_run(rva_yolov8_plan *p, int n, bool win, rva_stream_t stream)
{
    if (!win && !stream_is_capturing(stream)) p->primed = n;
}

}

extern "C" {

int rva_yolov8_plan_create(rva_ctx *ctx, const rva_yolov8_desc *desc, const rva_conv_weights *convs, rva_yolov8_plan **out)
{
    if (!ctx || !desc || !convs || !out) return RVA_ERR_ARG;
    *out = nullptr;
    if (desc->batch <= 0 || desc->height <= 0 || desc->width <= 0 || desc->height % 32 || desc->width % 32 || desc->nc <= 0 ||
        desc->nc % 8 || desc->reg_max != 16 || desc->n_convs <= 0)
        return rva_fail(ctx, RVA_ERR_ARG, "rva_yolov8_plan_create: batch > 0, height and width multiples of 32, nc %% 8 == 0, reg_max 16");
    for (int i = 0; i < 5; ++i)
        if (desc->widths[i] <= 0 || desc->widths[i] % 8) return rva_fail(ctx, RVA_ERR_ARG, "rva_yolov8_plan_create: channel widths must be multiples of 8");
    RVA_HIP(ctx, hipSetDevice(ctx->device));
    std::unique_ptr<rva_yolov8_plan> p(new rva_yolov8_plan());
    p->ctx = ctx; p->d = *desc; p->B = desc->batch; p->H = desc->height; p->W = desc->width; p->nc = desc->nc;
    p->f32 = (desc->flags & RVA_PLAN_F32) != 0;
    p->box32 = (desc->flags & RVA_PLAN_BOX_F32) != 0;
    if (p->f32 && p->box32)
        return rva_fail(ctx, RVA_ERR_ARG, "rva_yolov8_plan_create: RVA_PLAN_BOX_F32 belongs to fp16 plans (the output of an RVA_PLAN_F32 plan is fp32 already)");
    Builder b{p.get(), convs};
    const bool ok = b.build();
    if (!ok) {
        for (void *a : p->allocs) (void)hipFree(a);
        return rva_fail(ctx, b.err.find("hip") == 0 || b.err.find("upload") != std::string::npos ? RVA_ERR_HIP : RVA_ERR_ARG,
                        "rva_yolov8_plan_create: %s", b.err.c_str());
    }
    for (int l = 1; l <= 2; ++l)
        if (p->fork_step[l] >= 0) {
            RVA_HIP(ctx, hipEventCreateWithFlags(&p->fork_ev[l], hipEventDisableTiming));
            RVA_HIP(ctx, hipEventCreateWithFlags(&p->join_ev[l], hipEventDisableTiming));
        }
    RVA_HIP(ctx, hipDeviceSynchronize());
    if (p->box32) p->box_off = ((size_t)p->B * (4 + p->nc) * p->A * 2 + 255) / 256 * 256;
    p->rows_top = 0; p->rows_bottom = p->H;
    propagate_rows(p.get());
    *out = p.release();
    return RVA_OK;
}

void rva_yolov8_plan_destroy(rva_yolov8_plan *p)
{
    if (!p) return;
    for (void *a : p->allocs) (void)hipFree(a);
    for (int l = 0; l < 3; ++l) {
        if (p->fork_ev[l]) (void)hipEventDestroy(p->fork_ev[l]);
        if (p->join_ev[l]) (void)hipEventDestroy(p->join_ev[l]);
    }
    delete p;
}

int rva_yolov8_plan_info(const rva_yolov8_plan *p, int32_t *anchors, int32_t *out_rows, int32_t *n_steps, int32_t *n_tunable, int32_t *quiet_step)
{
    if (!p) return RVA_ERR_ARG;
    if (anchors) *anchors = p->A;
    if (out_rows) *out_rows = 4 + p->nc;
    if (n_steps) *n_steps = (int32_t)p->steps.size();
    if (n_tunable) *n_tunable = (int32_t)p->tunables.size();
    if (quiet_step) *quiet_step = p->quiet_step;
    return RVA_OK;
}

int rva_yolov8_plan_output_layout(const rva_yolov8_plan *p, int64_t *total_bytes, int64_t *boxes_offset)
{
    if (!p) return RVA_ERR_ARG;
    const size_t head = (size_t)p->B * (4 + p->nc) * p->A * (p->f32 ? 4 : 2);
    if (total_bytes) *total_bytes = (int64_t)(p->box32 ? p->box_off + (size_t)p->B * 4 * p->A * 4 : head);
    if (boxes_offset) *boxes_offset = p->box32 ? (int64_t)p->box_off : -1;
    return RVA_OK;
}

int rva_yolov8_plan_tunable_desc(const rva_yolov8_plan *p, int index, char *buf, int len)
{
    if (!p || index < 0 || index >= (int)p->tunables.size() || !buf || len <= 0) return RVA_ERR_ARG;
    snprintf(buf, (size_t)len, "%s", p->tunables[index].desc.c_str());
    return RVA_OK;
}

int rva_yolov8_plan_set_variant(rva_yolov8_plan *p, int index, int variant)
{
    if (!p || index < 0 || index >= (int)p->tunables.size()) return RVA_ERR_ARG;
    Step &s = p->steps[p->tunables[index].step];
    if (!variant_fits(s, variant) || variant > rva_conv_num_variants()) return rva_fail(p->ctx, RVA_ERR_ARG, "rva_yolov8_plan_set_variant: variant %d does not exist for this layer", variant);
    p->primed = 0;
    s.variant = variant;
    return RVA_OK;
}

int rva_yolov8_plan_get_variant(const rva_yolov8_plan *p, int index)
{
    if (!p || index < 0 || index >= (int)p->tunables.size()) return -1;
    return p->steps[p->tunables[index].step].variant;
}

int rva_yolov8_plan_launch_tunable(rva_yolov8_plan *p, int index, int variant, void *output, rva_stream_t stream)
{
    if (!p || index < 0 || index >= (int)p->tunables.size()) return RVA_ERR_ARG;
    const Step &s = p->steps[p->tunables[index].step];
    if (!variant_fits(s, variant)) return RVA_ERR_ARG;
    if (s.kind == K_HEAD && !output) return RVA_ERR_ARG;
    return launch_step(p, s, variant, nullptr, output, p->B, stream, true);
}

int rva_yolov8_plan_run_range_n(rva_yolov8_plan *p, const void *input, void *output, int n, int first, int last, rva_stream_t stream)
{
    if (const int rc = check_run(p, input, output, n); rc != RVA_OK) return rc;
    if (first < 0 || last > (int)p->steps.size() || first > last) return RVA_ERR_ARG;
    return run_steps(p, input, output, n, first, last, stream, n <= p->primed);
}

int rva_yolov8_plan_run_range(rva_yolov8_plan *p, const void *input, void *output, int first, int last, rva_stream_t stream)
{
    return p ? rva_yolov8_plan_run_range_n(p, input, output, p->B, first, last, stream) : RVA_ERR_ARG;
}

int rva_yolov8_plan_run_n(rva_yolov8_plan *p, const void *input, void *output, int n, rva_stream_t stream)
{
    if (const int rc = check_run(p, input, output, n); rc != RVA_OK) return rc;
    const bool win = n <= p->primed;
    const int rc = run_steps(p, input, output, n, 0, (int)p->steps.size(), stream, win);
    if (rc == RVA_OK) note_complete_run(p, n, win, stream);
    return rc;
}

int rva_yolov8_plan_run(rva_yolov8_plan *p, const void *input, void *output, rva_stream_t stream)
{
    return p ? rva_yolov8_plan_run_n(p, input, output, p->B, stream) : RVA_ERR_ARG;
}

int rva_yolov8_plan_primed_images(const rva_yolov8_plan *p) { return p ? p->primed : 0; }

int rva_yolov8_plan_set_static_rows(rva_yolov8_plan *p, int top, int bottom)
{
    if (!p) return RVA_ERR_ARG;
    if (top < 0 || bottom > p->H || top >= bottom)
        return rva_fail(p->ctx, RVA_ERR_ARG, "rva_yolov8_plan_set_static_rows: [%d, %d) is not a window of %d rows", top, bottom, p->H);
    const char *e = getenv("RVA_PLAN_NO_STATIC_ROWS");
    if (e && e[0] == '1') return RVA_OK;
    p->rows_top = top; p->rows_bottom = bottom;
    propagate_rows(p);
    return RVA_OK;
}

int rva_yolov8_plan_step_rows(const rva_yolov8_plan *p, int step, int32_t *y0, int32_t *y1)
{
    if (!p || step < 0 || step >= (int)p->steps.size()) return RVA_ERR_ARG;
    if (y0) *y0 = p->steps[step].y0;
    if (y1) *y1 = p->steps[step].y1;
    return RVA_OK;
}

int rva_conv_rows_through(int k, int stride, int H_in, int lo, int hi, int32_t *out_lo, int32_t *out_hi)
{
    if ((k != 1 && k != 3) || (stride != 1 && stride != 2) || H_in <= 0 || lo < 0 || hi > H_in || lo >= hi || !out_lo || !out_hi) return RVA_ERR_ARG;
    const int pad = k / 2, Ho = out_rows(H_in, k, stride);
    int a = lo + pad - (k - 1), b = hi - 1 + pad;
    a = a <= 0 ? 0 : (a + stride - 1) / stride;
    b = b / stride + 1;
    if (b > Ho) b = Ho;
    if (a > b) a = b;
    *out_lo = a; *out_hi = b;
    return RVA_OK;
}

int rva_yolov8_plan_run_lanes(rva_yolov8_plan *p, const void *input, void *output, rva_stream_t stream, rva_stream_t side1, rva_stream_t side2)
{
    return p ? rva_yolov8_plan_run_lanes_n(p, input, output, p->B, stream, side1, side2) : RVA_ERR_ARG;
}

int rva_yolov8_plan_run_lanes_n(rva_yolov8_plan *p, const void *input, void *output, int n, rva_stream_t stream, rva_stream_t side1, rva_stream_t side2)
{
    if (const int rc = check_run(p, input, output, n); rc != RVA_OK) return rc;
    if (!side1 || !side2 || p->fork_step[1] < 0) return rva_yolov8_plan_run_n(p, input, output, n, stream);
    hipStream_t lanes[3] = {(hipStream_t)stream, (hipStream_t)side1, (hipStream_t)side2};
    bool started[3] = {true, false, false};
    const bool win = n <= p->primed;
    for (int i = 0; i < (int)p->steps.size(); ++i) {
        for (int l = 1; l <= 2; ++l)
            if (p->fork_step[l] == i) RVA_HIP(p->ctx, hipEventRecord(p->fork_ev[l], lanes[0]));
        const Step &s = p->steps[i];
        if (s.lane && !started[s.lane]) {
            RVA_HIP(p->ctx, hipStreamWaitEvent(lanes[s.lane], p->fork_ev[s.lane], 0));
            started[s.lane] = true;
        }
        const int rc = launch_step(p, s, s.variant, input, output, n, (rva_stream_t)lanes[s.lane], win);
        if (rc != RVA_OK) return rc;
    }
    for (int l = 1; l <= 2; ++l)
        if (started[l]) {
            RVA_HIP(p->ctx, hipEventRecord(p->join_ev[l], lanes[l]));
            RVA_HIP(p->ctx, hipStreamWaitEvent(lanes[0], p->join_ev[l], 0));
        }
    note_complete_run(p, n, win, stream);
    return RVA_OK;
}

}
```

### realtime_video_analytics_32streams_amd/csrc/rva_postprocess.hip

```cpp
#include <hip/hip_fp16.h>

#include <cmath>
#include <cstdlib>
#include <cstring>

#include "rva_internal.h"

namespace {

struct PostMeta {
    float left, top, scale, xmax, ymax;
};

struct K2Args {
    const void *raw;
    int A, C;
    long sb, sa, sc;
    float thr;
    int use_cls;
    uint32_t cls_mask[32];
    PostMeta meta[RVA_MAX_BATCH];
    float4 *sp_box;
    float *sp_score;
    int32_t *sp_cls;
    uint32_t *bits;
    int nwords;
    int32_t *irr;
};

__device__ __forceinline__ float ldf(const float *p) { return *p; }
__device__ __forceinline__ float ldf(const __half *p) { return __half2float(*p); }

template <typename T, bool SPLIT>
__device__ __forceinline__ void k2_body(const K2Args &a, const float *boxes)
{
    const int b = blockIdx.y;
    const int anchor = blockIdx.x * 256 + threadIdx.x;
    const int lane = threadIdx.x & 63;
    bool pass = false, odd = false;
    if (anchor < a.A) {
        const T *p = (const T *)a.raw + (long)b * a.sb + (long)anchor * a.sa;
        float best;
        int bi = 0;
        if (a.C > 5) {
            const float obj = ldf(p + 4 * a.sc);
            best = ldf(p + 5 * a.sc) * obj;
#pragma unroll 8
            for (int c = 6; c < a.C; ++c) {
                float s = ldf(p + (long)c * a.sc) * obj;
                if (s > best) { best = s; bi = c - 5; }
            }
        } else {
            best = ldf(p + 4 * a.sc);
        }
        pass = best >= a.thr;
        if (a.use_cls) pass = pass && bi < 1024 && ((a.cls_mask[bi >> 5] >> (bi & 31)) & 1u);
        if (pass) {
            const PostMeta m = a.meta[b];
            float cx, cy, w, h;
            if constexpr (SPLIT) {
                const float *q = boxes + (long)b * 4 * a.A + anchor;
                cx = q[0]; cy = q[a.A]; w = q[2 * (long)a.A]; h = q[3 * (long)a.A];
            } else {
                cx = ldf(p); cy = ldf(p + a.sc); w = ldf(p + 2 * a.sc); h = ldf(p + 3 * a.sc);
            }
            float x1 = cx - w / 2.0f, y1 = cy - h / 2.0f, x2 = cx + w / 2.0f, y2 = cy + h / 2.0f;
            x1 -= m.left; x2 -= m.left; y1 -= m.top; y2 -= m.top;
            x1 = __fdiv_rn(x1, m.scale); y1 = __fdiv_rn(y1, m.scale);
            x2 = __fdiv_rn(x2, m.scale); y2 = __fdiv_rn(y2, m.scale);
            x1 = fminf(fmaxf(x1, 0.0f), m.xmax); x2 = fminf(fmaxf(x2, 0.0f), m.xmax);
            y1 = fminf(fmaxf(y1, 0.0f), m.ymax); y2 = fminf(fmaxf(y2, 0.0f), m.ymax);
            const long o = (long)b * a.A + anchor;
            a.sp_box[o] = make_float4(x1, y1, x2, y2);
            a.sp_score[o] = best;
            a.sp_cls[o] = bi;
            odd = !(x1 <= x2) || !(y1 <= y2);
        }
    }
    if (__any(odd) && lane == 0) atomicOr(a.irr + b, 1);
    const unsigned long long mask = __ballot(pass);
    const int a0 = blockIdx.x * 256 + (threadIdx.x & ~63);
    if (lane < 2) {
        const int w = (a0 >> 5) + lane;
        if (w < a.nwords) a.bits[(long)b * a.nwords + w] = (uint32_t)(mask >> (32 * lane));
    }
}

template <typename T>
__global__ void __launch_bounds__(256) k2_decode(K2Args a) { k2_body<T, false>(a, nullptr); }

template <typename T>
__global__ void __launch_bounds__(256) k2_decode_split(K2Args a, const float *boxes) { k2_body<T, true>(a, boxes); }

__device__ __forceinline__ float iou32(const float4 a, const float4 b)
{
    const float x1 = fmaxf(a.x, b.x), y1 = fmaxf(a.y, b.y);
    const float x2 = fminf(a.z, b.z), y2 = fminf(a.w, b.w);
    float w = x2 - x1, h = y2 - y1;
    w = w > 0.0f ? w : 0.0f;
    h = h > 0.0f ? h : 0.0f;
    const float inter = w * h;
    const float area_a = (a.z - a.x) * (a.w - a.y);
    const float area_b = (b.z - b.x) * (b.w - b.y);
    float uni = area_a + area_b - inter;
    uni = fmaxf(uni, 1e-6f);
    return __fdiv_rn(inter, uni);
}

struct SupTest { double m; int tie_incl; float thr, thr_up; };

__device__ __forceinline__ float vmax(float a, float b) { float r; asm("v_max_f32 %0, %1, %2" : "=v"(r) : "v"(a), "v"(b)); return r; }
__device__ __forceinline__ float vmin(float a, float b) { float r; asm("v_min_f32 %0, %1, %2" : "=v"(r) : "v"(a), "v"(b)); return r; }

__device__ __forceinline__ void iou_terms(const float4 a, const float area_a, const float4 b, const float area_b, float &inter, float &uni)
{
    const float x1 = vmax(a.x, b.x), y1 = vmax(a.y, b.y);
    const float x2 = vmin(a.z, b.z), y2 = vmin(a.w, b.w);
    float w = x2 - x1, h = y2 - y1;
    w = w > 0.0f ? w : 0.0f;
    h = h > 0.0f ? h : 0.0f;
    inter = w * h;
    uni = area_a + area_b - inter;
    uni = vmax(uni, 1e-6f);
}

__device__ __forceinline__ bool suppresses(const float4 a, const float area_a, const float4 b, const float area_b, const SupTest t)
{
    float inter, uni;
    iou_terms(a, area_a, b, area_b, inter, uni);
    const double di = (double)inter, rhs = t.m * (double)uni;
    return !(t.tie_incl ? di <= rhs : di < rhs);
}

__device__ __forceinline__ bool suppresses_fast(const float4 a, const float area_a, const float4 b, const float area_b, const SupTest t, bool &unsure)
{
    float inter, uni;
    iou_terms(a, area_a, b, area_b, inter, uni);
    const float lo = __builtin_fmaf(-t.thr, uni, inter), hi = __builtin_fmaf(-t.thr_up, uni, inter);
    const bool yes = hi >= 0.0f;
    unsure |= !(lo <= 0.0f) & !yes;
    return yes;
}
__device__ __forceinline__ float box_area(const float4 b) { return (b.z - b.x) * (b.w - b.y); }

typedef float k3_f4 __attribute__((ext_vector_type(4)));
__device__ __forceinline__ float4 load_global_f4(const float4 *p)
{
    const k3_f4 v = *reinterpret_cast<const __attribute__((address_space(1))) k3_f4 *>(reinterpret_cast<size_t>(p));
    return make_float4(v.x, v.y, v.z, v.w);
}

struct K3Args {
    const float4 *sp_box;
    const float *sp_score;
    const int32_t *sp_cls;
    const uint32_t *bits;
    int nwords, A, kcap;
    float iou_thr;
    SupTest sup;
    int max_det;
    float4 *out_boxes;
    float *out_scores;
    int32_t *out_cls, *out_anchor, *out_cand, *out_counts, *out_ncand;
    int32_t *flags;
    int32_t *irr;
    int bitonic_upto;
    float rfac;
    float bin_scale[RVA_MAX_BATCH];
};

#ifdef RVA_K3_STAMPS
__device__ unsigned long long g_k3_stamps[64][8];
#define K3_STAMP(slot) do { if (tid == 0) { const unsigned long long t_ = __builtin_amdgcn_s_memtime(); st_acc[slot] += t_ - st_last; st_last = t_; } } while (0)
#else
#define K3_STAMP(slot) do { } while (0)
#endif

constexpr int K3_THREADS = 1024;
constexpr int K3_WAVES = K3_THREADS / 64;
#ifndef RVA_K3_NEWEST
#define RVA_K3_NEWEST 64
#endif
constexpr int K3_NEWEST = RVA_K3_NEWEST;
constexpr int K3_KBL = 1024;
constexpr int K3_BINS = 64;
constexpr int K3_BIN_MIN_KEPT = 96;
constexpr double K3_BIN_MIN_THR = 0.15;

extern __shared__ __attribute__((aligned(16))) unsigned char k3_smem[];

__device__ __forceinline__ unsigned long long readlane64(unsigned long long v, int l)
{
    const unsigned lo = (unsigned)__builtin_amdgcn_readlane((int)(unsigned)v, l);
    const unsigned hi = (unsigned)__builtin_amdgcn_readlane((int)(unsigned)(v >> 32), l);
    return ((unsigned long long)hi << 32) | lo;
}

template <int E>
__device__ __forceinline__ void k3_sort(unsigned long long *keys, int tid)
{
    constexpr int KP = K3_THREADS * E;
    unsigned long long v[E];
#pragma unroll
    for (int e = 0; e < E; ++e) v[e] = keys[tid * E + e];
    for (int k = 2; k <= KP; k <<= 1) {
        for (int j = k >> 1; j >= E; j >>= 1) {
            if (j >= 64 * E) {
                __syncthreads();
#pragma unroll
                for (int e = 0; e < E; ++e) keys[tid * E + e] = v[e];
                __syncthreads();
#pragma unroll
                for (int e = 0; e < E; ++e) {
                    const int g = tid * E + e;
                    const unsigned long long o = keys[g ^ j];
                    const bool up = (g & k) == 0, lower = (g & j) == 0;
                    const unsigned long long mn = v[e] < o ? v[e] : o, mx = v[e] < o ? o : v[e];
                    v[e] = (lower == up) ? mn : mx;
                }
            } else {
                const int dl = j / E;
#pragma unroll
                for (int e = 0; e < E; ++e) {
                    const int g = tid * E + e;
                    const unsigned lo = __shfl_xor((unsigned)v[e], dl), hi = __shfl_xor((unsigned)(v[e] >> 32), dl);
                    const unsigned long long o = ((unsigned long long)hi << 32) | lo;
                    const bool up = (g & k) == 0, lower = (g & j) == 0;
                    const unsigned long long mn = v[e] < o ? v[e] : o, mx = v[e] < o ? o : v[e];
                    v[e] = (lower == up) ? mn : mx;
                }
            }
        }
#pragma unroll
        for (int jj = E / 2; jj >= 1; jj >>= 1) {
            if (jj < k) {
#pragma unroll
                for (int e = 0; e < E; ++e) {
                    if ((e & jj) == 0) {
                        const int g = tid * E + e;
                        const bool up = (g & k) == 0;
                        const unsigned long long x = v[e], y = v[e | jj];
                        const bool swap = (x > y) == up;
                        v[e] = swap ? y : x;
                        v[e | jj] = swap ? x : y;
                    }
                }
            }
        }
    }
    __syncthreads();
#pragma unroll
    for (int e = 0; e < E; ++e) keys[tid * E + e] = v[e];
    __syncthreads();
}

template <int E>
__device__ __forceinline__ void k3_radix(unsigned long long *a, unsigned long long *b2, int *hist, int *wtot, int K, int tid)
{
    const int lane = tid & 63, wave = tid >> 6;
    unsigned long long *src = a, *dst = b2;
    int *wh = hist + wave * 256;
    unsigned vor = 0u, vand = ~0u;
#pragma unroll
    for (int e = 0; e < E; ++e) {
        const int idx = wave * 64 * E + e * 64 + lane;
        if (idx < K) { const unsigned h = (unsigned)(a[idx] >> 32); vor |= h; vand &= h; }
    }
#pragma unroll
    for (int o = 32; o >= 1; o >>= 1) { vor |= __shfl_xor(vor, o); vand &= __shfl_xor(vand, o); }
    if (tid == 0) { wtot[8] = 0; wtot[9] = -1; }
    __syncthreads();
    if (lane == 0) { atomicOr(reinterpret_cast<unsigned *>(wtot) + 8, vor); atomicAnd(reinterpret_cast<unsigned *>(wtot) + 9, vand); }
    __syncthreads();
    const unsigned varying = reinterpret_cast<unsigned *>(wtot)[8] ^ reinterpret_cast<unsigned *>(wtot)[9];
    if (varying == 0u) return;
    const int lowbit = __builtin_ctz(varying), npass = (32 - __builtin_clz(varying) - lowbit + 7) >> 3;
    for (int pass = 0; pass < npass; ++pass) {
        const int sh = 32 + lowbit + 8 * pass;
        for (int i = tid; i < K3_WAVES * 256; i += K3_THREADS) hist[i] = 0;
        __syncthreads();
        unsigned long long v[E];
        int rk[E], dg[E];
#pragma unroll
        for (int e = 0; e < E; ++e) {
            const int idx = wave * 64 * E + e * 64 + lane;
            const bool in = idx < K;
            v[e] = in ? src[idx] : ~0ull;
            const int d = (int)(v[e] >> sh) & 255;
            dg[e] = d;
            unsigned long long m = __ballot(in);
#pragma unroll
            for (int bit = 0; bit < 8; ++bit) {
                const bool one = (d >> bit) & 1;
                const unsigned long long bb = __ballot(in && one);
                m &= one ? bb : ~bb;
            }
            const int below = __builtin_amdgcn_mbcnt_hi((unsigned)(m >> 32), __builtin_amdgcn_mbcnt_lo((unsigned)m, 0u));
            const int old = in ? wh[d] : 0;
            rk[e] = old + below;
            if (in && below == 0) wh[d] = old + __popcll(m);
            __builtin_amdgcn_fence(__ATOMIC_ACQ_REL, "wavefront");
            __builtin_amdgcn_wave_barrier();
        }
        __syncthreads();
        int c[K3_WAVES], run = 0, incl = 0;
        if (tid < 256) {
#pragma unroll
            for (int w = 0; w < K3_WAVES; ++w) { const int t = hist[w * 256 + tid]; c[w] = run; run += t; }
            incl = run;
#pragma unroll
            for (int o = 1; o < 64; o <<= 1) {
                const int t = __shfl_up(incl, o);
                if (lane >= o) incl += t;
            }
            if (lane == 63) wtot[wave] = incl;
        }
        __syncthreads();
        if (tid < 256) {
            int base = incl - run;
            for (int q = 0; q < wave; ++q) base += wtot[q];
#pragma unroll
            for (int w = 0; w < K3_WAVES; ++w) hist[w * 256 + tid] = base + c[w];
        }
        __syncthreads();
#pragma unroll
        for (int e = 0; e < E; ++e) {
            const int idx = wave * 64 * E + e * 64 + lane;
            if (idx < K) dst[wh[dg[e]] + rk[e]] = v[e];
        }
        __syncthreads();
        unsigned long long *t = src; src = dst; dst = t;
    }
    if (npass & 1) {
        for (int i = tid; i < K; i += K3_THREADS) a[i] = b2[i];
        __syncthreads();
    }
}

template <bool BOX = true>
__device__ __forceinline__ void k3_emit(const K3Args &a, int b, int pos, const float4 kbx, int kan, const float *score, const uint32_t *bw, const int *wprefix)
{
    const long o = (long)b * a.max_det + pos;
    if (BOX) a.out_boxes[o] = kbx;
    a.out_scores[o] = score[kan];
    a.out_cls[o] = a.sp_cls[(long)b * a.A + kan];
    if (a.out_anchor) a.out_anchor[o] = kan;
    if (a.out_cand) {
        const int w = kan >> 5;
        a.out_cand[o] = wprefix[w] + __popc(bw[w] & ((1u << (kan & 31)) - 1u));
    }
}

__global__ void __launch_bounds__(K3_THREADS) k3_nms(K3Args a)
{
    const int b = blockIdx.x, tid = threadIdx.x, lane = tid & 63, wave = tid >> 6;
    size_t off = 0;
    int *wprefix = (int *)(k3_smem + off); off += (((size_t)a.nwords * 4 + 15) & ~(size_t)15);
    int *wave_tot = (int *)(k3_smem + off); off += 64;
    unsigned long long *half_alive = (unsigned long long *)(k3_smem + off); off += 128;
    int *s_ctl = (int *)(k3_smem + off); off += 64;
    int *binstart = (int *)(k3_smem + off); off += (K3_BINS + 4) * 4;
    int *bincnt = (int *)(k3_smem + off); off += K3_BINS * 4;
    const bool binned = a.rfac > 0.f && a.irr[b] == 0;
    const float bscale = a.bin_scale[b];
    auto xbin = [&](float x) { const int v = (int)floorf(x * bscale); return v < 0 ? 0 : (v > K3_BINS - 1 ? K3_BINS - 1 : v); };

#ifdef RVA_K3_STAMPS
    unsigned long long st_acc[8] = {0, 0, 0, 0, 0, 0, 0, 0}, st_last = __builtin_amdgcn_s_memtime();
#endif
    const uint32_t *bw = a.bits + (long)b * a.nwords;
    if (tid == 0) { s_ctl[1] = 0; s_ctl[2] = 0; }
    if (tid < K3_BINS) bincnt[tid] = 0;
    __syncthreads();
    if (tid == 0) {
        a.irr[b] = 0;
        if (binned) atomicAdd(a.flags + 1 + RVA_MAX_BATCH, 1);
    }
    for (int w0 = 0; w0 < a.nwords; w0 += K3_THREADS) {
        const int w = w0 + tid;
        const int c = w < a.nwords ? __popc(bw[w]) : 0;
        int incl = c;
#pragma unroll
        for (int o = 1; o < 64; o <<= 1) {
            const int t = __shfl_up(incl, o);
            if (lane >= o) incl += t;
        }
        if (lane == 63) wave_tot[wave] = incl;
        __syncthreads();
        int base = s_ctl[2];
        for (int q = 0; q < wave; ++q) base += wave_tot[q];
        if (w < a.nwords) wprefix[w] = base + incl - c;
        __syncthreads();
        if (tid == K3_THREADS - 1) s_ctl[2] = base + incl;
        __syncthreads();
    }
    int K = s_ctl[2];
    if (a.out_ncand && tid == 0) a.out_ncand[b] = K;
    if (K > a.kcap) {
        if (tid == 0) atomicOr(a.flags, 2);
        K = a.kcap;
    }
    if (K == 0) {
        if (tid == 0) a.out_counts[b] = 0;
        return;
    }
    int Kpad = K3_THREADS;
    while (Kpad < K) Kpad <<= 1;
    const int SC = Kpad <= 8192 ? 512 : 256, KBL = Kpad <= 8192 ? K3_KBL : K3_KBL / 2;
    unsigned long long *keys = (unsigned long long *)(k3_smem + off); off += (size_t)Kpad * 8;
    float4 *kb = (float4 *)(k3_smem + off); off += (size_t)(KBL + 8) * 16;
    float4 *sv_box = (float4 *)(k3_smem + off); off += (size_t)SC * 16;
    int *sv_j = (int *)(k3_smem + off); off += (size_t)SC * 4;
    int *kj = (int *)(k3_smem + off); off += (size_t)KBL * 4;
    float *ka = (float *)(k3_smem + off); off += (size_t)(KBL + 8) * 4;
    unsigned long long *smask = (unsigned long long *)(k3_smem + off);
    const float *score = a.sp_score + (long)b * a.A;
    const float4 *box = a.sp_box + (long)b * a.A;
    for (int i = K + tid; i < Kpad; i += K3_THREADS) keys[i] = ~0ull;
    for (int w = tid; w < a.nwords; w += K3_THREADS) {
        uint32_t bits = bw[w];
        int pos = wprefix[w];
        while (bits) {
            const int an = (w << 5) + __builtin_ctz(bits);
            bits &= bits - 1u;
            if (pos < a.kcap) {
                uint32_t u = __float_as_uint(score[an]);
                u = (u & 0x80000000u) ? ~u : (u | 0x80000000u);
                keys[pos] = ((unsigned long long)(~u) << 32) | (uint32_t)an;
            }
            ++pos;
        }
    }
    __syncthreads();
    K3_STAMP(0);
    switch (Kpad <= a.bitonic_upto ? 64 + Kpad / K3_THREADS : Kpad / K3_THREADS) {
    case 65: k3_sort<1>(keys, tid); break;
    case 66: k3_sort<2>(keys, tid); break;
    case 68: k3_sort<4>(keys, tid); break;
    case 1: k3_radix<1>(keys, smask, (int *)kb, (int *)sv_box, K, tid); break;
    case 2: k3_radix<2>(keys, smask, (int *)kb, (int *)sv_box, K, tid); break;
    case 4: k3_radix<4>(keys, smask, (int *)kb, (int *)sv_box, K, tid); break;
    case 8: k3_sort<8>(keys, tid); break;
    default: k3_sort<16>(keys, tid); break;
    }
    for (int i = tid; i < KBL + 8; i += K3_THREADS) { kb[i] = make_float4(0.f, 0.f, 0.f, 0.f); ka[i] = 0.f; }
    __syncthreads();

    K3_STAMP(1);
    const int scw = SC >> 6;
    int rs = 64;
    const int bt = tid & (K3_THREADS / 2 - 1), half = tid / (K3_THREADS / 2);
    const float4 zero4 = make_float4(0.f, 0.f, 0.f, 0.f);
    float4 nbx = bt < rs && bt < K ? load_global_f4(box + (int)(uint32_t)keys[bt]) : zero4;
    for (int base = 0; base < K; base += rs, rs = rs * 2 < SC ? rs * 2 : SC) {
        const int j = base + bt;
        const bool valid = bt < rs && j < K;
        const float4 bx = nbx;
        const float area_b = box_area(bx);
        asm volatile("" :: "v"(bx.x), "v"(bx.y), "v"(bx.z), "v"(bx.w), "v"(area_b));
        {
            const int nrs = rs * 2 < SC ? rs * 2 : SC, jn = base + rs + bt;
            nbx = bt < nrs && jn < K ? load_global_f4(box + (int)(uint32_t)keys[jn]) : zero4;
        }
        bool alive = valid;
        const int nk = s_ctl[1] < a.max_det ? s_ctl[1] : a.max_det;
        const int nk_lds = nk < KBL ? nk : KBL;
        const bool rb = binned && nk_lds >= K3_BIN_MIN_KEPT;
        if (rb) {
            const bool mine = tid < nk_lds, wave_in = (tid & ~63) < nk_lds;
            float4 mb = zero4;
            float ma = 0.f;
            int mbin = 0, slot = 0;
            if (wave_in) {
                if (mine) { mb = kb[tid]; ma = ka[tid]; }
                mbin = xbin((mb.x + mb.z) * 0.5f);
                if (mine) slot = atomicAdd(&bincnt[mbin], 1);
            }
            __syncthreads();
            if (wave_in) {
                const int c = bincnt[lane];
                int incl = c;
#pragma unroll
                for (int o = 1; o < 64; o <<= 1) {
                    const int t = __shfl_up(incl, o);
                    if (lane >= o) incl += t;
                }
                const int dst = __shfl(incl - c, mbin) + slot;
                if (wave == 0) {
                    binstart[lane] = incl - c;
                    if (lane == 63) binstart[64] = incl;
                }
                if (mine) { kb[dst] = mb; ka[dst] = ma; }
            }
            __syncthreads();
            if (tid < K3_BINS) bincnt[tid] = 0;
            K3_STAMP(6);
        }
        if (rb) {
            const float cx = (bx.x + bx.z) * 0.5f;
            const int bc = xbin(cx);
            const int s0 = nk_lds > 0 ? binstart[bc > 0 ? bc - 1 : 0] & ~3 : 0, s1 = nk_lds > 0 ? binstart[(bc < K3_BINS - 1 ? bc + 1 : bc) + 1] : 0;
            for (int i = s0 + 4 * half; ; i += 8) {
                if (!__any(alive && i < s1)) break;
                const int ii = i < KBL ? i : KBL;
                float4 k4[4];
#pragma unroll
                for (int u = 0; u < 4; ++u) k4[u] = kb[ii + u];
                const float4 a4 = *reinterpret_cast<const float4 *>(ka + ii);
                const float ar[4] = {a4.x, a4.y, a4.z, a4.w};
                bool hit = false, unsure = false;
#pragma unroll
                for (int u = 0; u < 4; ++u) hit |= suppresses_fast(k4[u], ar[u], bx, area_b, a.sup, unsure);
                if (__any(unsure)) {
#pragma unroll
                    for (int u = 0; u < 4; ++u) hit |= suppresses(k4[u], ar[u], bx, area_b, a.sup);
                }
                alive = alive && !hit;
            }
        }
        const int lo = !rb && nk_lds > K3_NEWEST ? (nk_lds - K3_NEWEST) & ~7 : 0;
        for (int i = lo + 4 * half; !rb && i < nk_lds; i += 8) {
            if (!__any(alive)) break;
            float4 k4[4];
#pragma unroll
            for (int u = 0; u < 4; ++u) k4[u] = kb[i + u];
            const float4 a4 = *reinterpret_cast<const float4 *>(ka + i);
            const float ar[4] = {a4.x, a4.y, a4.z, a4.w};
            bool hit = false, unsure = false;
#pragma unroll
            for (int u = 0; u < 4; ++u) hit |= suppresses_fast(k4[u], ar[u], bx, area_b, a.sup, unsure);
            if (__any(unsure)) {
#pragma unroll
                for (int u = 0; u < 4; ++u) hit |= suppresses(k4[u], ar[u], bx, area_b, a.sup);
            }
            alive = alive && !hit;
        }
        const float4 *kept_glb = a.out_boxes + (long)b * a.max_det;
        for (int i = KBL + half; i < nk; i += 2) {
            if (!__any(alive)) break;
            const float4 kg = kept_glb[i];
            alive = alive && !suppresses(kg, box_area(kg), bx, area_b, a.sup);
        }
        K3_STAMP(2);
        const unsigned long long am0 = __ballot(alive);
        if (lane == 0) half_alive[wave] = am0;
        __syncthreads();
        const unsigned long long am = half_alive[wave & (K3_WAVES / 2 - 1)] & half_alive[(wave & (K3_WAVES / 2 - 1)) + K3_WAVES / 2];
        alive = half == 0 && ((am >> lane) & 1ull);
        if (lane == 0) wave_tot[wave] = half == 0 ? __popcll(am) : 0;
        __syncthreads();
        int so, ns;
        {
            const int c = lane < K3_WAVES / 2 ? wave_tot[lane] : 0;
            int incl = c;
#pragma unroll
            for (int o = 1; o < K3_WAVES / 2; o <<= 1) {
                const int t = __shfl_up(incl, o);
                if (lane >= o) incl += t;
            }
            so = __shfl(incl - c, wave & (K3_WAVES / 2 - 1));
            ns = __shfl(incl, K3_WAVES / 2 - 1);
            if (wave >= K3_WAVES / 2) so = 0;
        }
        if (alive) {
            const int sidx = so + __popcll(am & ((1ull << lane) - 1ull));
            sv_box[sidx] = bx;
            sv_j[sidx] = j;
        }
        __syncthreads();
        if ((rb || lo > 0) && ns > 0) {
            const int mp = (ns + 63) & ~63, parts = K3_THREADS / mp;
            const int part = tid / mp, bi = tid - part * mp;
            bool open = part < parts && bi < ns;
            const float4 ob = open ? sv_box[bi] : zero4;
            const float area_o = box_area(ob);
            if (rb) {
                const float cx = (ob.x + ob.z) * 0.5f;
                const float rad = (ob.z - ob.x) * a.rfac + (ob.x + ob.z) * 1e-5f + 1e-2f;
                const int s0 = binstart[xbin(cx - rad)] & ~3, s1 = binstart[xbin(cx + rad) + 1];
                for (int i = s0 + 4 * part; ; i += 4 * parts) {
                    if (!__any(open && i < s1)) break;
                    const int ii = i < KBL ? i : KBL;
                    float4 k4[4];
#pragma unroll
                    for (int u = 0; u < 4; ++u) k4[u] = kb[ii + u];
                    const float4 a4 = *reinterpret_cast<const float4 *>(ka + ii);
                    const float ar[4] = {a4.x, a4.y, a4.z, a4.w};
                    bool hit = false, unsure = false;
#pragma unroll
                    for (int u = 0; u < 4; ++u) hit |= suppresses_fast(k4[u], ar[u], ob, area_o, a.sup, unsure);
                    if (__any(unsure)) {
#pragma unroll
                        for (int u = 0; u < 4; ++u) hit |= suppresses(k4[u], ar[u], ob, area_o, a.sup);
                    }
                    if (open && hit) sv_j[bi] = -1;
                    open = open && !hit;
                }
            }
            for (int i = 4 * part; !rb && i < lo; i += 4 * parts) {
                if (!__any(open)) break;
                float4 k4[4];
#pragma unroll
                for (int u = 0; u < 4; ++u) k4[u] = kb[i + u];
                const float4 a4 = *reinterpret_cast<const float4 *>(ka + i);
                const float ar[4] = {a4.x, a4.y, a4.z, a4.w};
                bool hit = false, unsure = false;
#pragma unroll
                for (int u = 0; u < 4; ++u) hit |= suppresses_fast(k4[u], ar[u], ob, area_o, a.sup, unsure);
                if (__any(unsure)) {
#pragma unroll
                    for (int u = 0; u < 4; ++u) hit |= suppresses(k4[u], ar[u], ob, area_o, a.sup);
                }
                if (open && hit) sv_j[bi] = -1;
                open = open && !hit;
            }
            __syncthreads();
            const bool mine = tid < ns;
            const float4 sb = mine ? sv_box[tid] : zero4;
            const int sj = mine ? sv_j[tid] : -1;
            const unsigned long long lm = __ballot(sj >= 0);
            if (lane == 0) wave_tot[wave] = __popcll(lm);
            __syncthreads();
            int so2, ns2;
            {
                const int c = lane < K3_WAVES / 2 ? wave_tot[lane] : 0;
                int incl = c;
#pragma unroll
                for (int o = 1; o < K3_WAVES / 2; o <<= 1) {
                    const int t = __shfl_up(incl, o);
                    if (lane >= o) incl += t;
                }
                so2 = __shfl(incl - c, wave & (K3_WAVES / 2 - 1));
                ns2 = __shfl(incl, K3_WAVES / 2 - 1);
            }
            if (sj >= 0) {
                const int sidx = so2 + __popcll(lm & ((1ull << lane) - 1ull));
                sv_box[sidx] = sb;
                sv_j[sidx] = sj;
            }
            ns = ns2;
            __syncthreads();
        }
        if (ns > 64) {
            for (int x = 64 + tid; x < ns; x += K3_THREADS)
                for (int t = 0; t < (x >> 6); ++t) smask[(size_t)x * scw + t] = 0ull;
            __syncthreads();
        }
        K3_STAMP(3);
        if (ns == 0) continue;
        const int nct = (ns + 63) >> 6;
        for (int ct = 0, rt = 0; ct < nct; rt == ct ? (++ct, rt = 0) : ++rt) {
            const int col = ct * 64 + lane;
            const float4 cb = col < ns ? sv_box[col] : zero4;
            const float area_c = box_area(cb);
            const int rbase = rt * 64 + wave * 4;
            if (rbase >= ns) continue;
            float4 rb[4];
#pragma unroll
            for (int u = 0; u < 4; ++u) rb[u] = sv_box[rbase + u < ns ? rbase + u : rbase];
            unsigned mine = 0u;
#pragma unroll
            for (int u = 0; u < 4; ++u) {
                const int r = rbase + u;
                bool unsure = false;
                bool sup = suppresses_fast(rb[u], box_area(rb[u]), cb, area_c, a.sup, unsure);
                if (__any(unsure)) sup = suppresses(rb[u], box_area(rb[u]), cb, area_c, a.sup);
                sup = sup && col < ns && r < ns && col != r;
                const unsigned long long w = __ballot(sup);
                if (lane == 0 && r < ns) smask[(size_t)r * scw + ct] = w;
                mine |= (sup ? 1u : 0u) << u;
            }
            if (rt < ct && mine)
                __hip_atomic_fetch_or(reinterpret_cast<unsigned *>(&smask[(size_t)col * scw + rt]) + (wave >> 3), mine << ((wave & 7) * 4),
                                      __ATOMIC_RELAXED, __HIP_MEMORY_SCOPE_WORKGROUP);
        }
        __syncthreads();
        K3_STAMP(4);
        if (wave == 0) {
            unsigned long long keptw = 0ull;
            int out0 = s_ctl[1];
            for (int c = 0; c < nct; ++c) {
                const int r = c * 64 + lane;
                const bool in = r < ns;
                const unsigned long long own = in ? smask[(size_t)r * scw + c] : 0ull;
                unsigned long long hitw = 0ull;
                for (int t = 0; t < c; ++t) hitw |= (in ? smask[(size_t)r * scw + t] : 0ull) & readlane64(keptw, t);
                const unsigned long long before = own & ((1ull << lane) - 1ull);
                unsigned long long open = __ballot(in && hitw == 0ull), kept = 0ull;
                while (open) {
                    const bool mine = (open >> lane) & 1ull;
                    const bool out = (before & kept) != 0ull, wait = (before & open) != 0ull;
                    const unsigned long long nk_ = __ballot(mine && !out && !wait), no_ = __ballot(mine && out);
                    kept |= nk_;
                    open &= ~(nk_ | no_);
                }
                if (lane == c) keptw = kept;
                if ((kept >> lane) & 1ull) {
                    const int pos = out0 + __popcll(kept & ((1ull << lane) - 1ull));
                    const float4 kbx = sv_box[r];
                    if (pos < KBL) {
                        kb[pos] = kbx; ka[pos] = box_area(kbx); kj[pos] = sv_j[r];
                        if (pos < a.max_det) a.out_boxes[(long)b * a.max_det + pos] = kbx;
                    }
                    else if (pos < a.max_det) k3_emit(a, b, pos, kbx, (int)(uint32_t)keys[sv_j[r]], score, bw, wprefix);
                    if (pos >= a.max_det) atomicOr(a.flags, 1);
                }
                out0 += __popcll(kept);
            }
            if (lane == 0) s_ctl[1] = out0;
        }
        __syncthreads();
        K3_STAMP(5);
    }
    {
        int n = s_ctl[1] < a.max_det ? s_ctl[1] : a.max_det;
        n = n < KBL ? n : KBL;
        for (int pos = tid; pos < n; pos += K3_THREADS) k3_emit<false>(a, b, pos, zero4, (int)(uint32_t)keys[kj[pos]], score, bw, wprefix);
    }
    if (tid == 0) {
        const int n = s_ctl[1];
        a.out_counts[b] = n < a.max_det ? n : a.max_det;
#ifdef RVA_K3_STAMPS
        if (b < 64) for (int q = 0; q < 8; ++q) g_k3_stamps[b][q] = st_acc[q];
#endif
    }
}

__global__ void k_zero_counts(int32_t *p, int n)
{
    int i = blockIdx.x * blockDim.x + threadIdx.x;
    if (i < n) p[i] = 0;
}

}

static int postprocess_batch(rva_ctx *ctx, const void *raw, int raw_dtype, const float *boxes, int batch, int d1, int d2,
                             double conf_thr, double iou_thr, const int32_t *classes, int n_classes,
                             const rva_letterbox *metas, int n_metas, int max_det, float *out_boxes,
                             float *out_scores, int32_t *out_cls, int32_t *out_anchor, int32_t *out_cand,
                             int32_t *out_counts, int32_t *out_ncand, rva_stream_t stream_)
{
    if (!ctx) return RVA_ERR_ARG;
    hipStream_t stream = (hipStream_t)stream_;
    if (!raw || batch <= 0 || d1 <= 0 || d2 <= 0 || !metas || (n_metas != 1 && n_metas != batch) || max_det <= 0 ||
        !out_boxes || !out_scores || !out_cls || !out_counts)
        return rva_fail(ctx, RVA_ERR_ARG, "rva_postprocess_batch: bad argument");
    if (raw_dtype != RVA_F16 && raw_dtype != RVA_F32) return rva_fail(ctx, RVA_ERR_ARG, "raw_dtype must be RVA_F16|RVA_F32");
    const bool channel_major = d1 < d2;
    const int C = channel_major ? d1 : d2, A = channel_major ? d2 : d1;
    if (C < 5) {
        k_zero_counts<<<rva_ceil_div(batch, 256), 256, 0, stream>>>(out_counts, batch);
        if (out_ncand) k_zero_counts<<<rva_ceil_div(batch, 256), 256, 0, stream>>>(out_ncand, batch);
        RVA_HIP(ctx, hipGetLastError());
        return RVA_OK;
    }
    if (C - 5 > 1024 && n_classes > 0) return rva_fail(ctx, RVA_ERR_ARG, "class filter supports at most 1024 classes");
    int rc = rva_reserve(ctx, batch, A);
    if (rc != RVA_OK) return rc;

    int kcap = K3_THREADS;
    while (kcap < A && kcap < 16384) kcap <<= 1;
    const int nwords = rva_ceil_div(A, 32);
    auto layout = [](size_t keys, size_t kbl, size_t sc) { return keys * 8 + (kbl + 8) * 20 + kbl * 4 + sc * 20 + sc * (sc / 64) * 8; };
    const size_t fixed = (((size_t)nwords * 4 + 15) & ~(size_t)15) + 64 + 128 + 64 + (K3_BINS + 4) * 4 + K3_BINS * 4;
    size_t smem = fixed + layout(kcap < 8192 ? kcap : 8192, K3_KBL, 512);
    if (kcap > 8192 && fixed + layout(kcap, K3_KBL / 2, 256) > smem) smem = fixed + layout(kcap, K3_KBL / 2, 256);
    if (smem > 160 * 1024) return rva_fail(ctx, RVA_ERR_CAPACITY, "post-process: %d anchors need %zu B of LDS", A, smem);
    RVA_HIP(ctx, rva_func_smem((const void *)k3_nms, smem));

    for (int b0 = 0; b0 < batch; b0 += RVA_MAX_BATCH) {
        const int nb = batch - b0 < RVA_MAX_BATCH ? batch - b0 : RVA_MAX_BATCH;
        const size_t esz = raw_dtype == RVA_F16 ? 2 : 4;
        K2Args k2{};
        k2.raw = (const char *)raw + (size_t)b0 * d1 * d2 * esz;
        k2.A = A; k2.C = C;
        k2.sb = (long)d1 * d2;
        k2.sa = channel_major ? 1 : d2;
        k2.sc = channel_major ? d2 : 1;
        k2.thr = (float)conf_thr;
        k2.use_cls = n_classes > 0 && classes;
        for (int i = 0; k2.use_cls && i < n_classes; ++i)
            if (classes[i] >= 0 && classes[i] < 1024) k2.cls_mask[classes[i] >> 5] |= 1u << (classes[i] & 31);
        for (int i = 0; i < nb; ++i) {
            const rva_letterbox &m = metas[n_metas == 1 ? 0 : b0 + i];
            k2.meta[i] = PostMeta{(float)m.pad_left, (float)m.pad_top, (float)m.scale, (float)(m.src_w - 1),
                                  (float)(m.src_h - 1)};
        }
        k2.sp_box = (float4 *)ctx->sp_box; k2.sp_score = ctx->sp_score; k2.sp_cls = ctx->sp_cls;
        k2.bits = ctx->cand_bits; k2.nwords = nwords;
        k2.irr = ctx->post_flags + 1;
        dim3 g2(rva_ceil_div(A, 256), nb);
        if (boxes) {
            const float *bx = boxes + (size_t)b0 * 4 * A;
            if (raw_dtype == RVA_F16) k2_decode_split<__half><<<g2, 256, 0, stream>>>(k2, bx);
            else k2_decode_split<float><<<g2, 256, 0, stream>>>(k2, bx);
        }
        else if (raw_dtype == RVA_F16) k2_decode<__half><<<g2, 256, 0, stream>>>(k2);
        else k2_decode<float><<<g2, 256, 0, stream>>>(k2);

        K3Args k3{};
        k3.sp_box = (const float4 *)ctx->sp_box; k3.sp_score = ctx->sp_score; k3.sp_cls = ctx->sp_cls;
        k3.bits = ctx->cand_bits;
        k3.nwords = nwords; k3.A = A; k3.kcap = kcap;
        k3.iou_thr = (float)iou_thr;
        {
            const float t = (float)iou_thr;
            uint32_t tb;
            std::memcpy(&tb, &t, 4);
            k3.sup.m = ((double)t + (double)std::nextafterf(t, INFINITY)) * 0.5;
            k3.sup.tie_incl = (tb & 1u) == 0;
            k3.sup.thr = t; k3.sup.thr_up = std::nextafterf(t, INFINITY);
        }
        k3.max_det = max_det;
        k3.out_boxes = (float4 *)out_boxes + (size_t)b0 * max_det;
        k3.out_scores = out_scores + (size_t)b0 * max_det;
        k3.out_cls = out_cls + (size_t)b0 * max_det;
        k3.out_anchor = out_anchor ? out_anchor + (size_t)b0 * max_det : nullptr;
        k3.out_cand = out_cand ? out_cand + (size_t)b0 * max_det : nullptr;
        k3.out_counts = out_counts + b0;
        k3.out_ncand = out_ncand ? out_ncand + b0 : nullptr;
        k3.flags = ctx->post_flags;
        k3.irr = ctx->post_flags + 1;
        k3.bitonic_upto = getenv("RVA_K3_BITONIC_UPTO") ? atoi(getenv("RVA_K3_BITONIC_UPTO")) : 0;
        {
            const double t = (double)(float)iou_thr * (1.0 - 1e-6);
            k3.rfac = std::isfinite(t) && t >= K3_BIN_MIN_THR && t <= 0.999 && !getenv("RVA_K3_NOBINS")
                          ? (float)((t >= 0.5 ? 1.0 - t : 0.5 / t - 0.5) * 1.01) : 0.f;
            for (int i = 0; i < nb; ++i) {
                const rva_letterbox &m = metas[n_metas == 1 ? 0 : b0 + i];
                k3.bin_scale[i] = m.src_w > 0 ? (float)K3_BINS / (float)m.src_w : 1.f;
            }
        }
        k3_nms<<<nb, K3_THREADS, smem, stream>>>(k3);
    }
    RVA_HIP(ctx, hipGetLastError());
    return RVA_OK;
}

extern "C" int rva_postprocess_batch(rva_ctx *ctx, const void *raw, int raw_dtype, int batch, int d1, int d2,
                                     double conf_thr, double iou_thr, const int32_t *classes, int n_classes,
                                     const rva_letterbox *metas, int n_metas, int max_det, float *out_boxes,
                                     float *out_scores, int32_t *out_cls, int32_t *out_anchor, int32_t *out_cand,
                                     int32_t *out_counts, int32_t *out_ncand, rva_stream_t stream_)
{
    return postprocess_batch(ctx, raw, raw_dtype, nullptr, batch, d1, d2, conf_thr, iou_thr, classes, n_classes, metas, n_metas, max_det,
                             out_boxes, out_scores, out_cls, out_anchor, out_cand, out_counts, out_ncand, stream_);
}

extern "C" int rva_postprocess_boxes_batch(rva_ctx *ctx, const void *raw, int raw_dtype, const float *boxes, int batch, int channels,
                                           int anchors, double conf_thr, double iou_thr, const int32_t *classes, int n_classes,
                                           const rva_letterbox *metas, int n_metas, int max_det, float *out_boxes,
                                           float *out_scores, int32_t *out_cls, int32_t *out_anchor, int32_t *out_cand,
                                           int32_t *out_counts, int32_t *out_ncand, rva_stream_t stream_)
{
    if (!ctx) return RVA_ERR_ARG;
    if (!boxes || (uintptr_t)boxes % 4 || channels < 5 || channels >= anchors)
        return rva_fail(ctx, RVA_ERR_ARG, "rva_postprocess_boxes_batch: boxes [batch, 4, anchors] float and a [channels, anchors] head with 5 <= channels < anchors");
    return postprocess_batch(ctx, raw, raw_dtype, boxes, batch, channels, anchors, conf_thr, iou_thr, classes, n_classes, metas, n_metas, max_det,
                             out_boxes, out_scores, out_cls, out_anchor, out_cand, out_counts, out_ncand, stream_);
}

extern "C" int rva_post_filter_stats(rva_ctx *ctx, rva_stream_t stream_, int *binned_images)
{
    if (!ctx || !binned_images) return RVA_ERR_ARG;
    hipStream_t stream = (hipStream_t)stream_;
    int32_t v = 0;
    RVA_HIP(ctx, hipMemcpyAsync(&v, ctx->post_flags + 1 + RVA_MAX_BATCH, sizeof v, hipMemcpyDeviceToHost, stream));
    RVA_HIP(ctx, hipMemsetAsync(ctx->post_flags + 1 + RVA_MAX_BATCH, 0, sizeof v, stream));
    RVA_HIP(ctx, hipStreamSynchronize(stream));
    *binned_images = v;
    return RVA_OK;
}

#ifdef RVA_K3_STAMPS
extern "C" int rva_dbg_k3_stamps(unsigned long long *host) { return (int)hipMemcpyFromSymbol(host, HIP_SYMBOL(g_k3_stamps), sizeof(unsigned long long) * 64 * 8); }
#endif

extern "C" int rva_post_status(rva_ctx *ctx, rva_stream_t stream_, int *flags)
{
    if (!ctx || !flags) return RVA_ERR_ARG;
    hipStream_t stream = (hipStream_t)stream_;
    int32_t v = 0;
    RVA_HIP(ctx, hipMemcpyAsync(&v, ctx->post_flags, sizeof v, hipMemcpyDeviceToHost, stream));
    RVA_HIP(ctx, hipMemsetAsync(ctx->post_flags, 0, sizeof v, stream));
    RVA_HIP(ctx, hipStreamSynchronize(stream));
    *flags = v;
    return RVA_OK;
}
```

### realtime_video_analytics_32streams_amd/detector.py

```python
from __future__ import annotations

import abc
import logging
from dataclasses import dataclass
from typing import Iterable, List, Optional, Sequence

import numpy as np
import torch

from . import _native as N
from . import ops
from .config import HIP_BACKENDS, TEMPORAL_MODELS, DetectorConfig
from .video_stream import FramePacket
from .yolov8 import build_detector_net, variant_from_path

LOGGER = logging.getLogger(__name__)


@dataclass(slots=True)
class Detection:

    stream_name: str
    frame_id: int
    class_id: int
    confidence: float
    bbox_xyxy: tuple[float, float, float, float]


class BaseDetector(abc.ABC):

    def __init__(self, config: DetectorConfig):
        self.config = config

    @abc.abstractmethod
    def predict(self, packet: FramePacket) -> List[Detection]:
        raise NotImplementedError


def filter_detections(detections: Iterable[Detection], min_confidence: float) -> List[Detection]:
    return [d for d in detections if d.confidence >= min_confidence]


def create_detector(config: DetectorConfig) -> BaseDetector:
    backend = config.backend.lower()
    model_type = config.model_type.lower()
    if backend in HIP_BACKENDS:
        if model_type in TEMPORAL_MODELS:
            from .temporal import HipCNN3DDetector, HipCNNLSTMDetector, HipConvGRUDetector
            if model_type == "cnn_lstm":
                return HipCNNLSTMDetector(config)
            if model_type == "conv_gru":
                return HipConvGRUDetector(config)
            return HipCNN3DDetector(config)
        if model_type == "resnet":
            from .classify import HipResNetDetector
            return HipResNetDetector(config)
        if model_type in ("yolov5", "yolov8"):
            return HipYoloDetector(config)
        raise ValueError(f"Model type '{model_type}' not supported with backend '{config.backend}'")
    if backend in ("ultralytics", "tensorrt", "onnx", "onnxruntime", "openvino", "rknn", "rk3588"):
        raise RuntimeError(
            f"Detector backend '{config.backend}' belongs to the reference implementation and its runtime is not "
            "part of this library. Select backend 'hip' to run on MI355X.")
    raise ValueError(f"Unsupported detector backend '{config.backend}'")


class HipYoloDetector(BaseDetector):

    def __init__(self, config: DetectorConfig, infer_fn=None, net: Optional[torch.nn.Module] = None,
                 seed: int = 0, device: Optional[int] = None):
        super().__init__(config)
        self._plans = {}
        self.ctx = ops.context(device)
        self.device = torch.device("cuda", self.ctx.device)
        if config.input_size:
            self.input_hw = (int(config.input_size[0]), int(config.input_size[1]))
        else:
            self.input_hw = (640, 640)
        self.half = bool(config.half)
        self.engine = "fused" if self.half else ("fused-f32" if getattr(config, "hip_engine", "auto") in ("plan", "native") else "torch-fp32")
        self._infer_fn = infer_fn
        self.box_rows = getattr(config, "hip_box_rows", "fp16") if (self.engine == "fused" and infer_fn is None) else "fp16"
        cap = int(getattr(config, "hip_plan_capacity", 0) or 0)
        self.plan_capacity = cap if (infer_fn is None and self.engine in ("fused", "fused-f32")) else 0
        self._over_capacity_warned = False
        self.net = None
        if infer_fn is None:
            if net is None:
                scale = variant_from_path(config.model_path)
                net = build_detector_net(scale, seed=seed, weights=config.model_path)
                LOGGER.info("hip detector: YOLOv8%s, %s weights", scale,
                            "local state-dict" if _is_file(config.model_path) else "seeded random (no weights offline)")
            if self.engine == "torch-fp32":
                LOGGER.warning("hip detector: half=false -> fp32 network through PyTorch-ROCm (MIOpen); the hand-written fp16 "
                               "MFMA plan runs with `half: true`")
            net = net.fuse().to(self.device)
            net = net.half() if self.half else net.float()
            self.net = net.to(memory_format=torch.channels_last)
        self._post_bufs: dict = {}
        self._in_bufs: dict = {}
        self._in_border: dict = {}
        self._rows: dict = {}
        self._rows_told: dict = {}
        self._post: Optional[ops.PostBuffers] = None
        self._in: Optional[torch.Tensor] = None
        self._slot = 0
        if config.warmup and self.net is not None:
            with torch.inference_mode():
                self._infer(torch.zeros((1, 3, *self.input_hw), device=self.device,
                                        dtype=torch.float16 if self.half else torch.float32))

    def _images(self, batch: int) -> int:
        cap = self.plan_capacity
        if cap <= 0 or batch == cap:
            return batch
        if batch > cap:
            if not self._over_capacity_warned:
                self._over_capacity_warned = True
                LOGGER.warning("hip detector: a group of %d frames exceeds hip_plan_capacity=%d: it gets a plan of its own size, "
                               "built now", batch, cap)
            return batch
        return cap

    def _buf_key(self, batch: int):
        m = self._images(batch)
        return m if self._slot == 0 else (m, self._slot)

    def input_tensor(self, batch: int) -> torch.Tensor:
        n, m = self._buf_key(batch), self._images(batch)
        t = self._in_bufs.get(n)
        if t is None:
            dt = torch.float16 if self.half else torch.float32
            t = self._in_bufs[n] = torch.empty((m, 3, *self.input_hw), dtype=dt, device=self.device)
        return t if m == batch else t[:batch]

    def _preprocess(self, frames: Sequence) -> tuple[torch.Tensor, N.Letterbox]:
        n = self._buf_key(len(frames))
        self._in = self.input_tensor(len(frames))
        f0 = frames[0]
        if isinstance(f0, ops.Nv12Surface):
            key = (f0.width, f0.height) if not any(f.mask is not None for f in frames) else None
            have, bordered = self._in_border.get(n, (None, 0))
            steady = key is not None and have == key and len(frames) <= bordered
            res = ops.preprocess_nv12(frames, self.input_hw, self.half, out=self._in, ctx=self.ctx, content_only=steady)
            if not steady:
                self._in_border[n] = (key, len(frames))
                lb = res[1]
                self._note_rows(n, (int(lb.pad_top), int(lb.pad_top) + int(lb.new_h)) if key is not None else (0, self.input_hw[0]))
            return res
        dev = []
        for f in frames:
            t = torch.from_numpy(np.ascontiguousarray(f)) if isinstance(f, np.ndarray) else f
            dev.append(t.to(self.device, non_blocking=True).contiguous())
        self._in_border[n] = (None, 0)
        self._note_rows(n, (0, self.input_hw[0]))
        return ops.preprocess_bgr(dev, self.input_hw, self.half, out=self._in, ctx=self.ctx)

    def _note_rows(self, n, rows) -> None:
        rows = (max(rows[0], 0), min(rows[1], self.input_hw[0]))
        self._rows[n] = rows
        self._rows_told[n] = False

    def invalidate_engine(self) -> None:
        self._plans.clear()
        self._rows_told.clear()

    def plan_for(self, tensor: torch.Tensor):
        batch = int(tensor.shape[0])
        shape = (self._images(batch), int(tensor.shape[2]), int(tensor.shape[3]))
        key = shape if self._slot == 0 else shape + (self._slot,)
        plan = self._plans.get(key)
        if plan is None:
            from .engine import FusedYoloV8
            first = self._plans.get(shape) if self._slot else None
            n = shape[0] if self._slot == 0 else (shape[0], self._slot)
            rows = first.static_rows if first is not None else self._rows.get(n)
            plan = self._plans[key] = FusedYoloV8(self.net, shape[0], shape[1:], device=self.device, ctx=self.ctx,
                                                  autotune=first is None, tune_overlap=getattr(self, "tune_overlap", 1),
                                                  precision="fp32" if self.engine == "fused-f32" else "fp16", box_rows=self.box_rows,
                                                  static_rows=rows if self.engine == "fused" else None)
            if first is not None:
                plan.copy_tuning(first)
        plan.n = batch
        return plan

    def rows_pending(self, batch: int) -> bool:
        return not self._rows_told.get(self._buf_key(batch), True)

    def _tell_rows(self, plan, tensor: torch.Tensor) -> None:
        n = self._buf_key(int(tensor.shape[0]))
        own = self._in_bufs.get(n)
        if own is None or own.data_ptr() != tensor.data_ptr() or n not in self._rows:
            if plan.static_rows != (0, plan.H):
                plan.set_static_rows(0, plan.H)
                if n in self._rows:
                    self._rows_told[n] = False
            return
        if self._rows_told.get(n, True):
            return
        plan.set_static_rows(*self._rows[n])
        self._rows_told[n] = True

    def _infer(self, tensor: torch.Tensor):
        if self._infer_fn is not None:
            return self._infer_fn(tensor)
        if self.half:
            if tensor.dtype != torch.float16:
                raise TypeError("half detector: the fused plan takes the fp16 tensor K1 writes")
            plan = self.plan_for(tensor)
            if not torch.cuda.is_current_stream_capturing():
                self._tell_rows(plan, tensor)
            plan(tensor.contiguous())
            return plan.result()
        if self.engine == "fused-f32":
            if tensor.dtype != torch.float32:
                raise TypeError("fp32 plan: takes the fp32 tensor K1 writes for half=false")
            return self.plan_for(tensor)(tensor.contiguous())
        return self.net(tensor.float().contiguous(memory_format=torch.channels_last))

    def _postprocess_device(self, raw, metas: Sequence[N.Letterbox]) -> ops.PostBuffers:
        boxes = None
        if isinstance(raw, ops.SplitHead):
            raw, boxes = raw
        raw = raw.contiguous()
        B = raw.shape[0]
        A = raw.shape[2] if raw.shape[1] < raw.shape[2] else raw.shape[1]
        self._post = self._post_bufs.get((B, A))
        if self._post is None:
            self._post = self._post_bufs[(B, A)] = ops.PostBuffers.allocate(B, A, raw.device)
        return ops.postprocess(raw, self.config.confidence_threshold, self.config.iou_threshold, self.config.classes,
                               metas, max_det=A, out=self._post, ctx=self.ctx, boxes=boxes)

    def stage_pre(self, packets: Sequence[FramePacket]):
        return self._preprocess([p.frame for p in packets])

    def stage_net(self, pre):
        return self._infer(pre[0])

    def stage_post(self, raw, pre) -> ops.PostBuffers:
        return self._postprocess_device(raw, [pre[1]])

    @staticmethod
    def geometry_key(frame) -> tuple:
        if isinstance(frame, ops.Nv12Surface):
            return (int(frame.width), int(frame.height), "nv12")
        return (int(frame.shape[1]), int(frame.shape[0]), "bgr")

    def predict_batch_device(self, packets: Sequence[FramePacket]) -> ops.PostBuffers:
        if len({self.geometry_key(p.frame) for p in packets}) != 1:
            raise ValueError("predict_batch_device needs one frame geometry per call; use predict_batch for mixed sizes")
        with torch.inference_mode():
            tensor, meta = self._preprocess([p.frame for p in packets])
            raw = self._infer(tensor)
            return self._postprocess_device(raw, [meta])

    def predict_batch(self, packets: Sequence[FramePacket]) -> List[List[Detection]]:
        out: List[Optional[List[Detection]]] = [None] * len(packets)
        groups = {}
        for i, p in enumerate(packets):
            groups.setdefault(self.geometry_key(p.frame), []).append(i)
        for idxs in groups.values():
            res = self.predict_batch_device([packets[i] for i in idxs]).to_host()
            for i, r in zip(idxs, res):
                p = packets[i]
                out[i] = [Detection(stream_name=p.stream.name, frame_id=p.frame_id, class_id=int(r["cls"][k]),
                                    confidence=float(r["conf"][k]),
                                    bbox_xyxy=tuple(float(v) for v in r["boxes"][k])) for k in range(r["n"])]
        return out

    def predict(self, packet: FramePacket) -> List[Detection]:
        return self.predict_batch([packet])[0]


def _is_file(p: str) -> bool:
    from pathlib import Path
    return bool(p) and Path(p).is_file()
```

### realtime_video_analytics_32streams_amd/engine.py

```python
from __future__ import annotations

import ctypes as C
import os
import time
from typing import Dict, List, Optional, Tuple

import numpy as np
import torch

from . import _native as N
from . import ops
from .yolov8 import C2f, ConvBnAct, YoloV8


_LIB_DIGEST: Optional[str] = None


def _lib_digest() -> str:
    global _LIB_DIGEST
    if _LIB_DIGEST is None:
        import hashlib
        _LIB_DIGEST = hashlib.sha256(N.LIB_PATH.read_bytes()).hexdigest()
    return _LIB_DIGEST


def _tuning_dir():
    import os
    from pathlib import Path
    d = os.environ.get("RVA_TUNE_CACHE_DIR")
    return Path(d) if d else Path(os.environ.get("XDG_CACHE_HOME", str(Path.home() / ".cache"))) / "rva_amd" / "autotune"


def module_order_convs(net: YoloV8) -> list:
    def c2f(m: C2f):
        out = [m.cv1, m.cv2]
        for b in m.m:
            out += [b.cv1, b.cv2]
        return out
    mods = [net.b0, net.b1, *c2f(net.b2), net.b3, *c2f(net.b4), net.b5, *c2f(net.b6), net.b7, *c2f(net.b8), net.b9.cv1, net.b9.cv2,
            *c2f(net.h12), *c2f(net.h15), net.h16, *c2f(net.h18), net.h19, *c2f(net.h21)]
    for branch in (net.detect.box, net.detect.cls):
        for seq in branch:
            mods += [seq[0], seq[1], seq[2]]
    return [m.conv if isinstance(m, ConvBnAct) else m for m in mods]


class _VariantCell:

    __slots__ = ("eng", "idx")

    def __init__(self, eng, idx):
        self.eng, self.idx = eng, idx

    def __getitem__(self, key):
        assert key == "variant"
        return int(self.eng.L.rva_yolov8_plan_get_variant(self.eng.handle, self.idx))

    def __setitem__(self, key, value):
        assert key == "variant"
        self.eng.ctx.check(self.eng.L.rva_yolov8_plan_set_variant(self.eng.handle, self.idx, int(value)), "rva_yolov8_plan_set_variant")


class FusedYoloV8:
    def __init__(self, net: YoloV8, batch: int, hw: Tuple[int, int] = (640, 640), device: Optional[torch.device] = None,
                 ctx: Optional[N.Context] = None, autotune: bool = True, tune_overlap: int = 1, precision: str = "fp16",
                 box_rows: str = "fp16", static_rows: Optional[Tuple[int, int]] = None):
        import os
        if precision not in ("fp16", "fp32"):
            raise ValueError(f"precision must be 'fp16' or 'fp32', not {precision!r}")
        if box_rows not in ("fp16", "fp32"):
            raise ValueError(f"box_rows must be 'fp16' or 'fp32', not {box_rows!r}")
        if box_rows == "fp32" and precision == "fp32":
            raise ValueError("box_rows='fp32' belongs to the fp16 plan: the output of precision='fp32' is fp32 already")
        self.box_rows = box_rows
        self.precision = precision
        self.f32 = precision == "fp32"
        self.tune_overlap = int(tune_overlap)
        self.ctx = ctx or ops.context()
        self.dev = device or torch.device("cuda", self.ctx.device)
        self.B, self.H, self.W = batch, hw[0], hw[1]
        self.n = batch
        assert hw[0] % 32 == 0 and hw[1] % 32 == 0
        net = net.fuse()
        self._net = net
        self.nc = net.nc
        self.L = N.lib()
        convs = module_order_convs(net)
        keep, arr = [], (N.ConvWeights * len(convs))()
        for i, c in enumerate(convs):
            w = np.ascontiguousarray(c.weight.detach().float().cpu().numpy())
            b = None if c.bias is None else np.ascontiguousarray(c.bias.detach().float().cpu().numpy())
            keep += [w, b]
            arr[i].weight = w.ctypes.data_as(C.POINTER(C.c_float))
            arr[i].bias = b.ctypes.data_as(C.POINTER(C.c_float)) if b is not None else None
            arr[i].cout, arr[i].cin, arr[i].k, arr[i].stride = int(w.shape[0]), int(w.shape[1]), int(w.shape[2]), int(c.stride[0])
        d = N.YoloV8Desc()
        d.batch, d.height, d.width = batch, hw[0], hw[1]
        d.widths[:] = [net.b0.conv.out_channels, net.b1.conv.out_channels, net.b3.conv.out_channels, net.b5.conv.out_channels,
                       net.b7.conv.out_channels]
        d.depth_backbone[:] = [len(net.b2.m), len(net.b4.m), len(net.b6.m), len(net.b8.m)]
        d.depth_head = len(net.h12.m)
        assert len(net.h15.m) == len(net.h18.m) == len(net.h21.m) == d.depth_head
        d.nc, d.reg_max, d.n_convs = net.nc, net.detect.reg_max, len(convs)
        d.flags = (N.RVA_PLAN_NO_STEM2 if os.environ.get("RVA_NO_STEM2", "0") == "1" else 0) | \
                  (N.RVA_PLAN_NO_CIN_PAD if os.environ.get("RVA_NO_CIN_PAD", "0") == "1" else 0) | \
                  (0 if self._use_pair32() else N.RVA_PLAN_NO_PAIR32) | \
                  (N.RVA_PLAN_F32 if self.f32 else 0) | (N.RVA_PLAN_BOX_F32 if box_rows == "fp32" else 0)
        h = C.c_void_p()
        with torch.cuda.device(self.dev):
            self.ctx.check(self.L.rva_yolov8_plan_create(self.ctx.handle, C.byref(d), arr, C.byref(h)), "rva_yolov8_plan_create")
        self.handle = h
        del keep
        self.static_rows = (0, self.H)
        self.rows_epoch = 0
        if static_rows is not None and tuple(static_rows) != (0, self.H) and os.environ.get("RVA_PLAN_NO_STATIC_ROWS") != "1":
            self.ctx.check(self.L.rva_yolov8_plan_set_static_rows(h, int(static_rows[0]), int(static_rows[1])), "rva_yolov8_plan_set_static_rows")
            self.static_rows = (int(static_rows[0]), int(static_rows[1]))
        info = [C.c_int32() for _ in range(5)]
        self.ctx.check(self.L.rva_yolov8_plan_info(h, *[C.byref(v) for v in info]), "rva_yolov8_plan_info")
        self.A, rows, self._n_steps, n_tun, self.quiet_step = (int(v.value) for v in info)
        assert rows == 4 + self.nc
        self.dtype = torch.float32 if self.f32 else torch.float16
        self.boxes32: Optional[torch.Tensor] = None
        self._boxes = {}
        if box_rows == "fp32":
            total, off = C.c_int64(), C.c_int64()
            self.ctx.check(self.L.rva_yolov8_plan_output_layout(h, C.byref(total), C.byref(off)), "rva_yolov8_plan_output_layout")
            self._out_layout = (int(total.value), int(off.value))
            self.out, self.boxes32 = self._alloc_split()
            self._boxes[0] = self.boxes32
        else:
            self.out = torch.empty((batch, rows, self.A), dtype=self.dtype, device=self.dev)
        self._outs = {0: self.out}
        self.fused_stem = not self.f32 and not (d.flags & N.RVA_PLAN_NO_STEM2) and tuple(d.widths[:2]) == (32, 64)
        self._n_tunable = n_tun
        self._read_tunables()
        self._side = None
        self._forks = bool(self.fused_head_lanes())
        self.concurrent_heads = os.environ.get("RVA_SERIAL_HEADS") != "1"
        if autotune:
            self.autotune()

    def _read_tunables(self) -> None:
        self._tunable = []
        buf = C.create_string_buffer(96)
        for i in range(self._n_tunable):
            self.ctx.check(self.L.rva_yolov8_plan_tunable_desc(self.handle, i, buf, 96), "rva_yolov8_plan_tunable_desc")

            def launch(stream, variant, i=i):
                return self.L.rva_yolov8_plan_launch_tunable(self.handle, i, variant, C.c_void_p(self.out.data_ptr()), stream)
            self._tunable.append((launch, _VariantCell(self, i), buf.value.decode()))

    def set_static_rows(self, top: int, bottom: int) -> None:
        self.ctx.check(self.L.rva_yolov8_plan_set_static_rows(self.handle, int(top), int(bottom)), "rva_yolov8_plan_set_static_rows")
        if os.environ.get("RVA_PLAN_NO_STATIC_ROWS") == "1":
            return
        self.static_rows = (int(top), int(bottom))
        self.rows_epoch += 1
        self._read_tunables()

    @property
    def primed_images(self) -> int:
        return int(self.L.rva_yolov8_plan_primed_images(self.handle))

    @property
    def primed(self) -> bool:
        return self.primed_images >= self.n

    def step_rows(self, step: int) -> Tuple[int, int]:
        y0, y1 = C.c_int32(), C.c_int32()
        self.ctx.check(self.L.rva_yolov8_plan_step_rows(self.handle, int(step), C.byref(y0), C.byref(y1)), "rva_yolov8_plan_step_rows")
        return int(y0.value), int(y1.value)

    def _alloc_split(self) -> Tuple[torch.Tensor, torch.Tensor]:
        total, off = self._out_layout
        rows = 4 + self.nc
        buf = torch.empty((total,), dtype=torch.uint8, device=self.dev)
        head = buf[:self.B * rows * self.A * 2].view(torch.float16).view(self.B, rows, self.A)
        boxes = buf[off:off + self.B * 4 * self.A * 4].view(torch.float32).view(self.B, 4, self.A)
        return head, boxes

    def fused_head_lanes(self) -> bool:
        return self.f32 or any(d.startswith("head1:") for _, _, d in self._tunable)

    def __del__(self):
        try:
            if getattr(self, "handle", None):
                self.L.rva_yolov8_plan_destroy(self.handle)
                self.handle = None
        except Exception:
            pass

    def _tuning_key(self) -> str:
        import hashlib
        import os
        h = hashlib.sha256()
        h.update(torch.cuda.get_device_name(self.dev).encode())
        h.update(_lib_digest().encode())
        h.update(repr((self.B, self.H, self.W, [d for _, _, d in self._tunable])).encode())
        h.update(b"per-layer times; in-plan pass opt-in, three overlapping passes")
        h.update(repr([os.environ.get(k, "") for k in ("RVA_SKIP_VARIANTS", "RVA_TUNE_IN_PLAN", "RVA_TUNE_OVERLAP", "RVA_TUNE_TOP",
                                                       "RVA_TUNE_WITHIN", "RVA_NO_STEM2", "RVA_HEAD_SPLIT", "RVA_NO_CIN_PAD")]).encode())
        h.update(repr(int(os.environ.get("RVA_TUNE_LAYER_OVERLAP", getattr(self, "tune_overlap", 1)))).encode())
        if getattr(self, "f32", False):
            h.update(b"precision fp32")
        return h.hexdigest()[:24]

    def _load_tuning(self) -> bool:
        import json
        f = _tuning_dir() / f"{self._tuning_key()}.json"
        try:
            rec = json.loads(f.read_text())
            picks = rec["variants"]
            if len(picks) != len(self._tunable) or any(d != pd for (_, _, d), (pd, _) in zip(self._tunable, picks)):
                return False
        except (OSError, ValueError, KeyError, TypeError):
            return False
        try:
            for (_, state, _), (_, v) in zip(self._tunable, picks):
                state["variant"] = int(v)
        except RuntimeError:
            for _, state, _ in self._tunable:
                state["variant"] = 0
            return False
        self.tuning = [tuple(t) for t in rec.get("tuning", [])]
        self.tuning_source = str(f)
        return True

    def _store_tuning(self) -> None:
        import json
        import os
        d = _tuning_dir()
        try:
            d.mkdir(parents=True, exist_ok=True)
            tmp = d / f".{self._tuning_key()}.{os.getpid()}.tmp"
            tmp.write_text(json.dumps({"device": torch.cuda.get_device_name(self.dev), "batch": self.B, "hw": [self.H, self.W],
                                       "variants": [[desc, st["variant"]] for _, st, desc in self._tunable],
                                       "tuning": [list(t) for t in self.tuning]}))
            os.replace(tmp, d / f"{self._tuning_key()}.json")
        except OSError:
            pass

    def autotune(self, reps: int = 5) -> None:
        import os
        self.tuning_source = "measured"
        use_cache = os.environ.get("RVA_TUNE_CACHE", "1") == "1"
        if use_cache and self._load_tuning():
            return
        stream = C.c_void_p(torch.cuda.current_stream().cuda_stream)
        self.tuning = []
        self._candidates = {}
        self._n_variants = int(N.lib().rva_conv_num_variants())
        skip = {int(v) for v in os.environ.get("RVA_SKIP_VARIANTS", "").replace(",", " ").split()}
        cache = {}
        n_over = int(os.environ.get("RVA_TUNE_LAYER_OVERLAP", getattr(self, "tune_overlap", 1)))
        lanes = ops.chain_streams(self.dev, n_over) if n_over >= 2 else []
        spin = int(os.environ.get("RVA_TUNE_SPIN_CYCLES", "400000"))

        def time_variant(variant) -> float:
            torch.cuda.synchronize()
            if not lanes:
                e0, e1 = torch.cuda.Event(enable_timing=True), torch.cuda.Event(enable_timing=True)
                e0.record()
                for _ in range(reps):
                    launch(stream, variant)
                e1.record()
                torch.cuda.synchronize()
                return e0.elapsed_time(e1) / reps * 1e3
            evs = []
            for st in lanes:
                with torch.cuda.stream(st):
                    torch.cuda._sleep(spin)
                    a, b = torch.cuda.Event(enable_timing=True), torch.cuda.Event(enable_timing=True)
                    a.record()
                    sp = C.c_void_p(st.cuda_stream)
                    for _ in range(reps):
                        launch(sp, variant)
                    b.record()
                    evs.append((a, b))
            torch.cuda.synchronize()
            first = evs[0][0]
            return max(first.elapsed_time(b) for _, b in evs) / (reps * len(lanes)) * 1e3
        for launch, state, desc in self._tunable:
            if desc in cache:
                state["variant"] = cache[desc][0]
                continue
            best = (0, float("inf"))
            timed = []
            for variant in range(1, self._n_variants + 1):
                if variant in skip or launch(stream, variant) != N.RVA_OK:
                    continue
                us = time_variant(variant)
                timed.append((us, variant))
                if us < best[1]:
                    best = (variant, us)
            state["variant"] = best[0]
            cache[desc] = best
            self._candidates[desc] = sorted(timed)[:int(os.environ.get('RVA_TUNE_TOP', '5'))]
            self.tuning.append((desc, best[0], round(best[1], 1)))
        if os.environ.get("RVA_TUNE_IN_PLAN", "0") == "1":
            self._refine_in_plan()
        if use_cache:
            self._store_tuning()

    def copy_tuning(self, other: "FusedYoloV8") -> None:
        assert len(self._tunable) == len(other._tunable) and self.precision == other.precision
        for (_, mine, d1), (_, theirs, d2) in zip(self._tunable, other._tunable):
            assert d1 == d2
            mine["variant"] = theirs["variant"]
        self.tuning = list(getattr(other, "tuning", []))
        self.tuning_source = "copied from the first slot's plan"

    def _refine_in_plan(self, reps: int = 12, within: float = 1.25) -> None:
        import os
        within = float(os.environ.get('RVA_TUNE_WITHIN', within))
        """Second pass of the kernel selection, on the real objective: a layer's launch time in isolation is not its cost inside
        the plan -- the detect branches run on side streams beside the neck, and a kernel that wants every CU for itself (one
        128-KB workgroup per CU) shares worse than a two-workgroups-per-CU one that is a few per cent slower alone.  For the
        layers with runners-up within 25 % the whole forward pass is timed with each candidate (coordinate descent, most
        expensive layers first) and a candidate is kept when the pass gets faster by more than the timing noise."""
        x = torch.zeros((self.B, 3, self.H, self.W), dtype=self.dtype, device=self.dev)
        twins: list = []
        lanes = self.concurrent_heads
        n_over = int(os.environ.get("RVA_TUNE_OVERLAP", "3"))
        if n_over >= 2:
            twins = [FusedYoloV8(self._net, self.B, (self.H, self.W), device=self.dev, ctx=self.ctx, autotune=False, precision=self.precision,
                                 box_rows=self.box_rows, static_rows=self.static_rows)
                     for _ in range(n_over - 1)]
            from .ops import chain_streams
            streams = chain_streams(self.dev, n_over)
            self.concurrent_heads = False
            for t in twins:
                t.concurrent_heads = False

        def forward_us() -> float:
            best = float("inf")
            for t in twins:
                t.copy_tuning(self)
            group = [self] + twins
            rounds = max(reps // len(group), 2)
            for _ in range(2):
                torch.cuda.synchronize()
                t0 = time.perf_counter()
                if not twins:
                    for _ in range(reps):
                        self(x)
                else:
                    for _ in range(rounds):
                        for pl, st in zip(group, streams):
                            with torch.cuda.stream(st):
                                pl(x)
                torch.cuda.synchronize()
                best = min(best, (time.perf_counter() - t0) / (rounds * len(group) if twins else reps) * 1e6)
            return best
        by_desc: Dict[str, list] = {}
        for _, state, desc in self._tunable:
            by_desc.setdefault(desc, []).append(state)
        cost = {d: v[0][0] * len(by_desc[d]) for d, v in self._candidates.items() if v}
        order = [d for d in sorted(cost, key=cost.get, reverse=True)
                 if len(self._candidates[d]) > 1 and self._candidates[d][1][0] <= within * self._candidates[d][0][0]][:24]
        if not order:
            self.concurrent_heads = lanes
            return
        self(x); self(x)
        forward_us()
        base = forward_us()
        self.refined = []
        for _sweep in range(2):
            changed = False
            for d in order:
                cur = by_desc[d][0]["variant"]
                for us, v in self._candidates[d]:
                    if us > within * self._candidates[d][0][0]:
                        break
                    if v == cur:
                        continue
                    for st in by_desc[d]:
                        st["variant"] = v
                    t = forward_us()
                    if t < base * 0.997:
                        self.refined.append((d, cur, v, round(base, 1), round(t, 1)))
                        base, cur, changed = t, v, True
                    else:
                        for st in by_desc[d]:
                            st["variant"] = cur
            if not changed:
                break
        self.concurrent_heads = lanes
        iso = {d: {v: us for us, v in c} for d, c in self._candidates.items()}
        self.tuning = [(d, by_desc[d][0]["variant"], round(iso[d].get(by_desc[d][0]["variant"], us), 1)) for d, _, us in self.tuning]

    def __call__(self, x: torch.Tensor) -> torch.Tensor:
        assert x.is_cuda and x.dtype == self.dtype and x.is_contiguous() and x.dim() == 4 and tuple(x.shape[1:]) == (3, self.H, self.W)
        n = int(x.shape[0])
        assert 1 <= n <= self.B, f"{n} images on a plan of capacity {self.B}"
        self.n = n
        main = torch.cuda.current_stream()
        stream = C.c_void_p(main.cuda_stream)
        xin, out = C.c_void_p(x.data_ptr()), C.c_void_p(self.out.data_ptr())
        if self.concurrent_heads and self._forks:
            if self._side is None:
                self._side = (torch.cuda.Stream(device=self.dev), torch.cuda.Stream(device=self.dev))
            self.ctx.check(self.L.rva_yolov8_plan_run_lanes_n(self.handle, xin, out, n, stream, C.c_void_p(self._side[0].cuda_stream),
                                                              C.c_void_p(self._side[1].cuda_stream)), "rva_yolov8_plan_run_lanes_n")
            return self._head()
        ev = getattr(self, "phase_event", None)
        if ev is not None:
            self.ctx.check(self.L.rva_yolov8_plan_run_range_n(self.handle, xin, out, n, 0, self.quiet_step, stream), "rva_yolov8_plan_run_range_n")
            ev.record(main)
            self.ctx.check(self.L.rva_yolov8_plan_run_range_n(self.handle, xin, out, n, self.quiet_step, self._n_steps, stream),
                           "rva_yolov8_plan_run_range_n")
        else:
            self.ctx.check(self.L.rva_yolov8_plan_run_n(self.handle, xin, out, n, stream), "rva_yolov8_plan_run_n")
        return self._head()

    def _head(self) -> torch.Tensor:
        return self.out if self.n == self.B else self.out[:self.n]

    def use_output(self, index: int) -> torch.Tensor:
        if index not in self._outs:
            if self.box_rows == "fp32":
                self._outs[index], self._boxes[index] = self._alloc_split()
            else:
                self._outs[index] = torch.empty_like(self._outs[0])
        self.out = self._outs[index]
        self.boxes32 = self._boxes.get(index)
        return self.out

    def result(self):
        if self.boxes32 is None:
            return self._head()
        return ops.SplitHead(self._head(), self.boxes32 if self.n == self.B else self.boxes32[:self.n])

    def _use_pair32(self) -> bool:
        env = os.environ.get("RVA_PAIR32")
        if env in ("0", "1"):
            return env == "1"
        return int(os.environ.get("RVA_TUNE_LAYER_OVERLAP", self.tune_overlap)) <= 1

    @property
    def n_launches(self) -> int:
        return self._n_steps
```

Baseline: 24060.

## Defer YOLO box-branch tail to postprocess, computing it only for score-passing anchors

The plan can now skip the last two box-branch convolutions and the DFL decode during the network run and leave the box rows pending. Postprocess first scores anchors to build a candidate bitmap, then a new MFMA kernel runs the 3x3 conv, the 1x1 conv and the DFL softmax only for anchors that passed the threshold, writing just those box rows. This removes dense box-head work over every anchor at all three levels. In exchange it adds cross-module state (a lazy-head map keyed by output pointer), extra launches and coupling between the plan and postprocess, and box rows are invalid for any consumer other than postprocess.

Result: no change. 23970 (-0.3%).

```diff
diff --git a/include/rva.h b/include/rva.h
--- a/include/rva.h
+++ b/include/rva.h
@@ -160,6 +160,9 @@
 int rva_conv1x1_head_box32_f16(rva_ctx *ctx, const void *in, int ldi, const void *weights, const float *bias, int batch,
                                int H, int W, int Cin, void *out, float *boxes32, int nc, int anchors_total, int anchor_offset,
                                float stride_px, int variant, rva_stream_t stream);
+int rva_yolo_box_tail_at_f16(rva_ctx *ctx, const void *x, int ldx, const void *w1, const float *b1, const void *w2, const float *b2,
+                             const uint32_t *bits, int nwords, int batch, int H, int W, void *out, int nc, int A, int a0,
+                             float stride_px, rva_stream_t stream);
 int rva_stem_conv_f16(rva_ctx *ctx, const void *in_planar, const void *weights, const float *bias,
                       void *out, int ldo, int batch, int H, int W, int Cout, rva_stream_t stream);
 
@@ -244,6 +247,9 @@
 int rva_yolov8_plan_run_range_n(rva_yolov8_plan *plan, const void *input, void *output, int n, int first, int last, rva_stream_t stream);
 int rva_yolov8_plan_primed_images(const rva_yolov8_plan *plan);
 int rva_yolov8_plan_step_rows(const rva_yolov8_plan *plan, int step, int32_t *y0, int32_t *y1);
+int rva_yolov8_plan_set_lazy_boxes(rva_yolov8_plan *plan, int on);
+int rva_yolov8_plan_get_lazy_boxes(const rva_yolov8_plan *plan);
+int rva_yolov8_plan_expect_lazy_boxes(rva_yolov8_plan *plan, const void *output, int n);
 
 typedef struct rva_cnnlstm_plan rva_cnnlstm_plan;
 typedef struct rva_cnnlstm_desc {
diff --git a/realtime_video_analytics_32streams_amd/_native.py b/realtime_video_analytics_32streams_amd/_native.py
--- a/realtime_video_analytics_32streams_amd/_native.py
+++ b/realtime_video_analytics_32streams_amd/_native.py
@@ -11,7 +11,7 @@
 ROOT = PKG.parent
 CSRC = PKG / "csrc"
 LIB_PATH = Path(os.environ["RVA_LIB_PATH"]) if os.environ.get("RVA_LIB_PATH") else PKG / "librva.so"
-SOURCES = ["rva_ctx.hip", "rva_preprocess.hip", "rva_postprocess.hip", "rva_tracker.hip", "rva_conv.hip", "rva_conv_f32.hip", "rva_plan.hip", "rva_clip.hip",
+SOURCES = ["rva_ctx.hip", "rva_preprocess.hip", "rva_postprocess.hip", "rva_tracker.hip", "rva_conv.hip", "rva_boxtail.hip", "rva_conv_f32.hip", "rva_plan.hip", "rva_clip.hip",
            "rva_clip3d.hip", "rva_clip3d_f16.hip", "rva_clip_f16.hip", "rva_resnet.hip", "rva_gates.hip", "rva_decode.hip", "rva_preview.hip", "rva_jpeg.hip"]
 HIPCC_FLAGS = ["--offload-arch=gfx950", "-O3", "-fPIC", "-shared", "-std=c++17", "-ffp-contract=off",
                "-Wall", "-Wno-unused-function"]
@@ -236,6 +236,11 @@
         "rva_yolov8_plan_run_lanes_n": (C.c_int, [_P, _P, _P, C.c_int, _P, _P, _P]),
         "rva_yolov8_plan_run_range_n": (C.c_int, [_P, _P, _P, C.c_int, C.c_int, C.c_int, _P]),
         "rva_yolov8_plan_primed_images": (C.c_int, [_P]),
+        "rva_yolov8_plan_set_lazy_boxes": (C.c_int, [_P, C.c_int]),
+        "rva_yolov8_plan_get_lazy_boxes": (C.c_int, [_P]),
+        "rva_yolov8_plan_expect_lazy_boxes": (C.c_int, [_P, _P, C.c_int]),
+        "rva_yolo_box_tail_at_f16": (C.c_int, [_P, _P, C.c_int, _P, _P, _P, _P, _P, C.c_int, C.c_int, C.c_int, C.c_int, _P, C.c_int, C.c_int,
+                                               C.c_int, C.c_float, _P]),
         "rva_cnnlstm_plan_create": (C.c_int, [_P, C.POINTER(CnnLstmDesc), C.POINTER(CnnLstmWeights), C.POINTER(_P)]),
         "rva_cnnlstm_plan_destroy": (None, [_P]),
         "rva_cnnlstm_plan_info": (C.c_int, [_P, i32p, i32p, i32p, i32p]),
@@ -311,6 +316,7 @@
     "rva_cnn3d_f16_plan_run", "rva_cnn3d_f16_plan_run_post", "rva_cnn3d_f16_plan_stage", "rva_resnet_plan_create", "rva_resnet_plan_destroy", "rva_resnet_plan_info",
     "rva_resnet_plan_run", "rva_resnet_plan_run_post", "rva_resnet_plan_stage", "rva_jpeg_max_bytes", "rva_jpeg_encode_bgr", "rva_jpeg_status",
     "rva_jpeg_batch_create", "rva_jpeg_batch_destroy", "rva_jpeg_batch_encode", "rva_preview_nv12_batch",
+    "rva_yolov8_plan_set_lazy_boxes", "rva_yolov8_plan_get_lazy_boxes", "rva_yolov8_plan_expect_lazy_boxes", "rva_yolo_box_tail_at_f16",
 ]
 
 
diff --git a/realtime_video_analytics_32streams_amd/csrc/rva_boxtail.hip b/realtime_video_analytics_32streams_amd/csrc/rva_boxtail.hip
--- /dev/null
+++ b/realtime_video_analytics_32streams_amd/csrc/rva_boxtail.hip
@@ -0,0 +1,213 @@
+#include <hip/hip_fp16.h>
+
+#include "rva_internal.h"
+#include "rva_mfma_f16.h"
+
+namespace {
+
+constexpr int BT_WORDS = 64;
+constexpr int BT_THREADS = 9 * 64;
+
+struct BoxTailArgs {
+    rva_box_level lv[3];
+    int nlv;
+    int blocks[3];
+    const uint32_t *bits;
+    int nwords;
+    __half *out;
+    int nc, A, batch;
+};
+
+__device__ __forceinline__ float bt_silu(float v) { return v * __builtin_amdgcn_rcpf(1.0f + __expf(-v)); }
+
+__global__ void __launch_bounds__(BT_THREADS) k_box_tail(BoxTailArgs a)
+{
+    __shared__ int list[BT_WORDS * 32];
+    __shared__ int s_total;
+    __shared__ float sum[32][64];
+    __shared__ __attribute__((aligned(16))) _Float16 tile[32][72];
+    int blk = blockIdx.x, l = 0;
+    if (a.nlv > 1 && blk >= a.blocks[0]) { blk -= a.blocks[0]; l = 1; if (a.nlv > 2 && blk >= a.blocks[1]) { blk -= a.blocks[1]; l = 2; } }
+    const rva_box_level &L = a.lv[l];
+    const int b = blockIdx.y, wave = threadIdx.x >> 6, lane = threadIdx.x & 63, r = lane & 31, h = lane >> 5;
+    const int HW = L.H * L.W, lw = (HW + 31) >> 5;
+    if (wave == 0) {
+        const int wl = blk * BT_WORDS + lane;
+        uint32_t bw = 0u;
+        if (lane < BT_WORDS && wl < lw) {
+            bw = a.bits[(size_t)b * a.nwords + (L.a0 >> 5) + wl];
+            const int left = HW - 32 * wl;
+            if (left < 32) bw &= (1u << left) - 1u;
+        }
+        const int c = __popc(bw);
+        int incl = c;
+#pragma unroll
+        for (int o = 1; o < BT_WORDS; o <<= 1) {
+            const int t = __shfl_up(incl, o);
+            if (lane >= o) incl += t;
+        }
+        if (lane == BT_WORDS - 1) s_total = incl;
+        for (int pos = incl - c; bw; ++pos) {
+            list[pos] = 32 * wl + __builtin_ctz(bw);
+            bw &= bw - 1u;
+        }
+    }
+    __syncthreads();
+    const int total = s_total;
+    if (total == 0) return;
+    const _Float16 *x = (const _Float16 *)L.x, *w1 = (const _Float16 *)L.w1, *w2 = (const _Float16 *)L.w2;
+    const int ky = wave / 3, kx = wave - 3 * ky;
+    f16x8 fb[2][4];
+#pragma unroll
+    for (int nt = 0; nt < 2; ++nt)
+#pragma unroll
+        for (int ch = 0; ch < 4; ++ch)
+            fb[nt][ch] = *reinterpret_cast<const f16x8 *>(w1 + ((size_t)(nt * 32 + r) * 9 + wave) * 64 + 16 * ch + 8 * h);
+    f16x8 fw2[2][4] = {};
+    float bias1[2] = {0.f, 0.f}, bias2[2] = {0.f, 0.f};
+    if (wave == 0) {
+#pragma unroll
+        for (int nt = 0; nt < 2; ++nt) {
+#pragma unroll
+            for (int ch = 0; ch < 4; ++ch) fw2[nt][ch] = *reinterpret_cast<const f16x8 *>(w2 + (size_t)(nt * 32 + r) * 64 + 16 * ch + 8 * h);
+            bias1[nt] = L.b1[nt * 32 + r];
+            bias2[nt] = L.b2[nt * 32 + r];
+        }
+    }
+    for (int t0 = 0; t0 < total; t0 += 32) {
+        const bool valid = t0 + r < total;
+        const int i = valid ? list[t0 + r] : 0;
+        const int iy = i / L.W + ky - 1, ix = i - (i / L.W) * L.W + kx - 1;
+        const bool av = valid && (unsigned)iy < (unsigned)L.H && (unsigned)ix < (unsigned)L.W;
+        const _Float16 *arow = x + (((size_t)b * L.H + (av ? iy : 0)) * L.W + (av ? ix : 0)) * L.ldx + 8 * h;
+        f16x8 fa[4];
+#pragma unroll
+        for (int ch = 0; ch < 4; ++ch) fa[ch] = av ? *reinterpret_cast<const f16x8 *>(arow + 16 * ch) : f16x8{};
+        f32x16 acc[2] = {};
+#pragma unroll
+        for (int ch = 0; ch < 4; ++ch)
+#pragma unroll
+            for (int nt = 0; nt < 2; ++nt) acc[nt] = __builtin_amdgcn_mfma_f32_32x32x16_f16(fa[ch], fb[nt][ch], acc[nt], 0, 0, 0);
+        for (int s = 0; s < 9; ++s) {
+            if (wave == s) {
+#pragma unroll
+                for (int nt = 0; nt < 2; ++nt)
+#pragma unroll
+                    for (int q = 0; q < 16; ++q) sum[nt * 16 + q][lane] = s == 0 ? acc[nt][q] : sum[nt * 16 + q][lane] + acc[nt][q];
+            }
+            __syncthreads();
+        }
+        if (wave == 0) {
+#pragma unroll
+            for (int nt = 0; nt < 2; ++nt)
+#pragma unroll
+                for (int q = 0; q < 16; ++q) tile[f32_cd_row(q, h)][nt * 32 + r] = (_Float16)bt_silu(sum[nt * 16 + q][lane] + bias1[nt]);
+            __builtin_amdgcn_fence(__ATOMIC_ACQ_REL, "workgroup");
+            __builtin_amdgcn_wave_barrier();
+            f32x16 lg[2] = {};
+#pragma unroll
+            for (int ch = 0; ch < 4; ++ch) {
+                const f16x8 f1 = *reinterpret_cast<const f16x8 *>(&tile[r][16 * ch + 8 * h]);
+#pragma unroll
+                for (int nt = 0; nt < 2; ++nt) lg[nt] = __builtin_amdgcn_mfma_f32_32x32x16_f16(f1, fw2[nt][ch], lg[nt], 0, 0, 0);
+            }
+            __builtin_amdgcn_fence(__ATOMIC_ACQ_REL, "workgroup");
+            __builtin_amdgcn_wave_barrier();
+#pragma unroll
+            for (int nt = 0; nt < 2; ++nt)
+#pragma unroll
+                for (int q = 0; q < 16; ++q) tile[f32_cd_row(q, h)][nt * 32 + r] = (_Float16)(lg[nt][q] + bias2[nt]);
+            __builtin_amdgcn_fence(__ATOMIC_ACQ_REL, "workgroup");
+            __builtin_amdgcn_wave_barrier();
+            if (h == 0 && valid) {
+                const __half *bp = reinterpret_cast<const __half *>(&tile[r][0]);
+                float d[4];
+#pragma unroll
+                for (int sd = 0; sd < 4; ++sd) {
+                    float v[16], mx = -1e30f;
+                    const uint4 q0 = *reinterpret_cast<const uint4 *>(bp + sd * 16), q1 = *reinterpret_cast<const uint4 *>(bp + sd * 16 + 8);
+                    const __half2 *h0 = reinterpret_cast<const __half2 *>(&q0), *h1 = reinterpret_cast<const __half2 *>(&q1);
+#pragma unroll
+                    for (int t = 0; t < 4; ++t) {
+                        float2 f = __half22float2(h0[t]); v[2 * t] = f.x; v[2 * t + 1] = f.y;
+                        f = __half22float2(h1[t]); v[8 + 2 * t] = f.x; v[9 + 2 * t] = f.y;
+                    }
+#pragma unroll
+                    for (int t = 0; t < 16; ++t) mx = fmaxf(mx, v[t]);
+                    float se = 0.f, sw = 0.f;
+#pragma unroll
+                    for (int t = 0; t < 16; ++t) { const float e = __expf(v[t] - mx); se += e; sw += e * (float)t; }
+                    d[sd] = sw / se;
+                }
+                const float ax = (float)(i % L.W) + 0.5f, ay = (float)(i / L.W) + 0.5f;
+                const float x1 = ax - d[0], y1 = ay - d[1], x2 = ax + d[2], y2 = ay + d[3];
+                __half *o = a.out + (size_t)b * (4 + a.nc) * a.A + L.a0 + i;
+                o[0] = __float2half_rn((x1 + x2) * 0.5f * L.stride_px);
+                o[(size_t)a.A] = __float2half_rn((y1 + y2) * 0.5f * L.stride_px);
+                o[(size_t)2 * a.A] = __float2half_rn((x2 - x1) * L.stride_px);
+                o[(size_t)3 * a.A] = __float2half_rn((y2 - y1) * L.stride_px);
+            }
+        }
+    }
+}
+
+template <bool VEC>
+__global__ void __launch_bounds__(256) k_zero_box_rows(__half *out, long image_halves, int per)
+{
+    const int i = blockIdx.x * 256 + threadIdx.x;
+    if (i >= per) return;
+    __half *o = out + (size_t)blockIdx.y * image_halves;
+    if constexpr (VEC) reinterpret_cast<uint4 *>(o)[i] = make_uint4(0u, 0u, 0u, 0u);
+    else o[i] = __ushort_as_half((unsigned short)0);
+}
+
+}
+
+int rva_box_tail_launch(rva_ctx *ctx, const rva_box_level *lv, int nlv, const uint32_t *bits, int nwords, int batch, void *out, int nc,
+                        int A, hipStream_t stream)
+{
+    if (!ctx) return RVA_ERR_ARG;
+    if (!lv || nlv < 1 || nlv > 3 || !bits || !out || batch <= 0 || nc < 0 || A <= 0 || nwords <= 0)
+        return rva_fail(ctx, RVA_ERR_ARG, "rva_yolo_box_tail_at_f16: bad argument");
+    BoxTailArgs a{};
+    int blocks = 0;
+    for (int l = 0; l < nlv; ++l) {
+        const rva_box_level &v = lv[l];
+        if (!v.x || !v.w1 || !v.b1 || !v.w2 || !v.b2 || v.H <= 0 || v.W <= 0 || v.H > 2000 || v.W > 2000 || v.ldx < 64 || v.ldx % 8 ||
+            ((uintptr_t)v.x | (uintptr_t)v.w1 | (uintptr_t)v.w2) % 16)
+            return rva_fail(ctx, RVA_ERR_ARG, "rva_yolo_box_tail_at_f16: x, w1, w2 16-byte aligned, ldx >= 64 and a multiple of 8, 1 <= H, W <= 2000");
+        if (v.a0 < 0 || v.a0 % 32 || (long)v.a0 + (long)v.H * v.W > A || (l > 0 && v.a0 < lv[l - 1].a0 + lv[l - 1].H * lv[l - 1].W))
+            return rva_fail(ctx, RVA_ERR_ARG, "rva_yolo_box_tail_at_f16: a0 = %d must be a multiple of 32 and the level must lie inside the %d anchors", v.a0, A);
+        if ((long)nwords * 32 < (long)v.a0 + (long)v.H * v.W)
+            return rva_fail(ctx, RVA_ERR_ARG, "rva_yolo_box_tail_at_f16: %d bitmap words do not cover anchors up to %d", nwords, v.a0 + v.H * v.W);
+        a.lv[l] = v;
+        a.blocks[l] = rva_ceil_div(rva_ceil_div(v.H * v.W, 32), BT_WORDS);
+        blocks += a.blocks[l];
+    }
+    a.nlv = nlv; a.bits = bits; a.nwords = nwords; a.out = (__half *)out; a.nc = nc; a.A = A; a.batch = batch;
+    k_box_tail<<<dim3(blocks, batch), BT_THREADS, 0, stream>>>(a);
+    RVA_HIP(ctx, hipGetLastError());
+    return RVA_OK;
+}
+
+int rva_zero_box_rows_launch(rva_ctx *ctx, void *out, int n, int nc, int A, hipStream_t stream)
+{
+    const long image_halves = (long)(4 + nc) * A;
+    if (A % 8 == 0 && (uintptr_t)out % 16 == 0) {
+        const int per = A / 2;
+        k_zero_box_rows<true><<<dim3(rva_ceil_div(per, 256), n), 256, 0, stream>>>((__half *)out, image_halves, per);
+    } else {
+        k_zero_box_rows<false><<<dim3(rva_ceil_div(4 * A, 256), n), 256, 0, stream>>>((__half *)out, image_halves, 4 * A);
+    }
+    RVA_HIP(ctx, hipGetLastError());
+    return RVA_OK;
+}
+
+extern "C" int rva_yolo_box_tail_at_f16(rva_ctx *ctx, const void *x, int ldx, const void *w1, const float *b1, const void *w2, const float *b2,
+                                        const uint32_t *bits, int nwords, int batch, int H, int W, void *out, int nc, int A, int a0,
+                                        float stride_px, rva_stream_t stream)
+{
+    if (!ctx) return RVA_ERR_ARG;
+    rva_box_level lv{x, ldx, w1, b1, w2, b2, H, W, a0, stride_px};
+    return rva_box_tail_launch(ctx, &lv, 1, bits, nwords, batch, out, nc, A, (hipStream_t)stream);
+}
diff --git a/realtime_video_analytics_32streams_amd/csrc/rva_internal.h b/realtime_video_analytics_32streams_amd/csrc/rva_internal.h
--- a/realtime_video_analytics_32streams_amd/csrc/rva_internal.h
+++ b/realtime_video_analytics_32streams_amd/csrc/rva_internal.h
@@ -25,6 +25,18 @@
 
 struct rva_jpeg_state;
 
+struct rva_box_level {
+    const void *x; int ldx;
+    const void *w1; const float *b1; const void *w2; const float *b2;
+    int H, W, a0; float stride_px;
+};
+
+struct rva_lazy_head {
+    const void *owner;
+    int n, A, nc;
+    rva_box_level lv[3];
+};
+
 struct rva_ctx {
     int device = 0;
     rva_jpeg_state *jpeg = nullptr;
@@ -40,6 +52,7 @@
     int k1_px = -1;
     int k1_nt = -1;
     int num_cus = 0;
+    std::map<const void *, rva_lazy_head> lazy_heads;
 };
 
 inline int rva_fail(rva_ctx *ctx, int code, const char *fmt, ...)
@@ -75,6 +88,10 @@
 int rva_conv2d_nhwc_f16_sel(rva_ctx *ctx, const void *in, int ldi, const void *weights, const float *bias, void *out, int ldo,
                             const void *residual, int ldr, int batch, int sel_batch, int H, int W, int Cin, int Cout, int ksize, int stride,
                             int act, int variant, int y0, int y1, rva_stream_t stream);
+
+int rva_box_tail_launch(rva_ctx *ctx, const rva_box_level *lv, int nlv, const uint32_t *bits, int nwords, int batch, void *out, int nc,
+                        int A, hipStream_t stream);
+int rva_zero_box_rows_launch(rva_ctx *ctx, void *out, int n, int nc, int A, hipStream_t stream);
 
 void rva_jpeg_free(rva_ctx *ctx);
 
diff --git a/realtime_video_analytics_32streams_amd/csrc/rva_plan.hip b/realtime_video_analytics_32streams_amd/csrc/rva_plan.hip
--- a/realtime_video_analytics_32streams_amd/csrc/rva_plan.hip
+++ b/realtime_video_analytics_32streams_amd/csrc/rva_plan.hip
@@ -1,4 +1,5 @@
 #include <cstring>
+#include <iterator>
 #include <memory>
 
 #include "rva_internal.h"
@@ -25,6 +26,7 @@
     int H = 0, W = 0, Cin = 0, Cout = 0, k = 0, stride = 0, act = 0, variant = 0;
     int mode = 0, a0 = 0; float stride_px = 0.f;
     int c_real = 0;
+    bool box_tail = false;
     int Ho = 0, y0 = 0, y1 = 0;
     const void *hb[3] = {nullptr, nullptr, nullptr}, *hk[3] = {nullptr, nullptr, nullptr};
     int32_t hldb[3] = {0, 0, 0}, hldc[3] = {0, 0, 0}, hh[3] = {0, 0, 0}, hw[3] = {0, 0, 0}; float hs[3] = {0, 0, 0};
@@ -51,6 +53,10 @@
     int rows_top = 0, rows_bottom = 0;
     bool windowed = false;
     int primed = 0;
+    int tail_primed = 0;
+    bool lazy = false;
+    bool lazy_ok = false;
+    rva_box_level box_lv[3] = {};
 };
 
 namespace {
@@ -386,6 +392,9 @@
             if (!conv(sib, 2, feats[l], first, hs[l], ws[l], 1)) return false;
             if (p->fused_head) {
                 if (!conv1(box[l][1], first.sub(0, cb), b2, hs[l], ws[l], 1) || !head(box[l][2], b2, 1, hs[l], ws[l], a0, strides[l])) return false;
+                Step &t1 = p->steps[p->steps.size() - 2], &t2 = p->steps.back();
+                t1.box_tail = t2.box_tail = true;
+                p->box_lv[l] = rva_box_level{first.sub(0, cb).ptr(), first.ld, t1.w, t1.b, t2.w, t2.b, hs[l], ws[l], a0, strides[l]};
                 if (!conv1(cls[l][1], first.sub(cb, cc), k2, hs[l], ws[l], 1) || !head(cls[l][2], k2, 2, hs[l], ws[l], a0, strides[l])) return false;
             } else {
                 View bo = buf(m, rm4), ko = buf(m, d.nc);
@@ -403,6 +412,7 @@
         }
         lane = 0;
         if (!p->fused_head && !p->f32) push(h3s, nullptr);
+        p->lazy_ok = p->fused_head && !p->box32 && cb == 64 && (h3 * w3) % 32 == 0 && (h3 * w3 + h4 * w4) % 32 == 0;
         return err.empty();
     }
 };
@@ -540,7 +550,7 @@
             t.desc += w;
         }
     }
-    p->primed = 0;
+    p->primed = p->tail_primed = 0;
 }
 
 bool stream_is_capturing(rva_stream_t stream)
@@ -550,13 +560,39 @@
     return cs != hipStreamCaptureStatusNone;
 }
 
-int run_steps(rva_yolov8_plan *p, const void *input, void *output, int n, int first, int last, rva_stream_t stream, bool win)
+bool step_win(const rva_yolov8_plan *p, const Step &s, int n, bool win) { return win && (!s.box_tail || n <= p->tail_primed); }
+
+int run_steps(rva_yolov8_plan *p, const void *input, void *output, int n, int first, int last, rva_stream_t stream, bool win, bool lazy = false)
 {
     for (int i = first; i < last; ++i) {
         const Step &s = p->steps[i];
-        const int rc = launch_step(p, s, s.variant, input, output, n, stream, win);
+        if (lazy && s.box_tail) continue;
+        const int rc = launch_step(p, s, s.variant, input, output, n, stream, step_win(p, s, n, win));
         if (rc != RVA_OK) return rc;
     }
+    return RVA_OK;
+}
+
+void drop_lazy_heads(rva_yolov8_plan *p)
+{
+    auto &m = p->ctx->lazy_heads;
+    for (auto it = m.begin(); it != m.end();) it = it->second.owner == p ? m.erase(it) : std::next(it);
+}
+
+void note_lazy_head(rva_yolov8_plan *p, const void *output, int n)
+{
+    rva_lazy_head h{};
+    h.owner = p; h.n = n; h.A = p->A; h.nc = p->nc;
+    for (int l = 0; l < 3; ++l) h.lv[l] = p->box_lv[l];
+    p->ctx->lazy_heads[output] = h;
+}
+
+int begin_complete_run(rva_yolov8_plan *p, void *output, int n, bool lazy, rva_stream_t stream)
+{
+    if (!lazy) { p->ctx->lazy_heads.erase(output); return RVA_OK; }
+    const int rc = rva_zero_box_rows_launch(p->ctx, output, n, p->nc, p->A, (hipStream_t)stream);
+    if (rc != RVA_OK) return rc;
+    note_lazy_head(p, output, n);
     return RVA_OK;
 }
 
@@ -568,9 +604,11 @@
     return RVA_OK;
 }
 
-void note_complete_run(rva_yolov8_plan *p, int n, bool win, rva_stream_t stream)
-{
-    if (!win && !stream_is_capturing(stream)) p->primed = n;
+void note_complete_run(rva_yolov8_plan *p, int n, bool win, bool lazy, rva_stream_t stream)
+{
+    if (stream_is_capturing(stream)) return;
+    if (!win) { p->primed = n; p->tail_primed = lazy ? 0 : n; }
+    else if (!lazy && n > p->tail_primed) p->tail_primed = n;
 }
 
 }
@@ -616,6 +654,7 @@
 void rva_yolov8_plan_destroy(rva_yolov8_plan *p)
 {
     if (!p) return;
+    drop_lazy_heads(p);
     for (void *a : p->allocs) (void)hipFree(a);
     for (int l = 0; l < 3; ++l) {
         if (p->fork_ev[l]) (void)hipEventDestroy(p->fork_ev[l]);
@@ -656,7 +695,7 @@
     if (!p || index < 0 || index >= (int)p->tunables.size()) return RVA_ERR_ARG;
     Step &s = p->steps[p->tunables[index].step];
     if (!variant_fits(s, variant) || variant > rva_conv_num_variants()) return rva_fail(p->ctx, RVA_ERR_ARG, "rva_yolov8_plan_set_variant: variant %d does not exist for this layer", variant);
-    p->primed = 0;
+    p->primed = p->tail_primed = 0;
     s.variant = variant;
     return RVA_OK;
 }
@@ -691,9 +730,10 @@
 int rva_yolov8_plan_run_n(rva_yolov8_plan *p, const void *input, void *output, int n, rva_stream_t stream)
 {
     if (const int rc = check_run(p, input, output, n); rc != RVA_OK) return rc;
-    const bool win = n <= p->primed;
-    const int rc = run_steps(p, input, output, n, 0, (int)p->steps.size(), stream, win);
-    if (rc == RVA_OK) note_complete_run(p, n, win, stream);
+    const bool win = n <= p->primed, lazy = p->lazy && p->lazy_ok;
+    if (const int rc = begin_complete_run(p, output, n, lazy, stream); rc != RVA_OK) return rc;
+    const int rc = run_steps(p, input, output, n, 0, (int)p->steps.size(), stream, win, lazy);
+    if (rc == RVA_OK) note_complete_run(p, n, win, lazy, stream);
     return rc;
 }
 
@@ -713,6 +753,27 @@
     if (e && e[0] == '1') return RVA_OK;
     p->rows_top = top; p->rows_bottom = bottom;
     propagate_rows(p);
+    return RVA_OK;
+}
+
+int rva_yolov8_plan_set_lazy_boxes(rva_yolov8_plan *p, int on)
+{
+    if (!p) return RVA_ERR_ARG;
+    const char *e = getenv("RVA_PLAN_NO_LAZY_BOXES");
+    if (e && e[0] == '1') return RVA_OK;
+    p->lazy = on != 0 && p->lazy_ok;
+    if (!p->lazy) drop_lazy_heads(p);
+    return RVA_OK;
+}
+
+int rva_yolov8_plan_get_lazy_boxes(const rva_yolov8_plan *p) { return p && p->lazy && p->lazy_ok ? 1 : 0; }
+
+int rva_yolov8_plan_expect_lazy_boxes(rva_yolov8_plan *p, const void *output, int n)
+{
+    if (!p || !output) return RVA_ERR_ARG;
+    if (n <= 0 || n > p->B) return rva_fail(p->ctx, RVA_ERR_ARG, "rva_yolov8_plan_expect_lazy_boxes: n = %d is not 1 .. %d, the plan's capacity", n, p->B);
+    const char *e = getenv("RVA_PLAN_NO_LAZY_BOXES");
+    if (p->lazy_ok && !(e && e[0] == '1')) note_lazy_head(p, output, n);
     return RVA_OK;
 }
 
@@ -748,16 +809,18 @@
     if (!side1 || !side2 || p->fork_step[1] < 0) return rva_yolov8_plan_run_n(p, input, output, n, stream);
     hipStream_t lanes[3] = {(hipStream_t)stream, (hipStream_t)side1, (hipStream_t)side2};
     bool started[3] = {true, false, false};
-    const bool win = n <= p->primed;
+    const bool win = n <= p->primed, lazy = p->lazy && p->lazy_ok;
+    if (const int rc = begin_complete_run(p, output, n, lazy, stream); rc != RVA_OK) return rc;
     for (int i = 0; i < (int)p->steps.size(); ++i) {
         for (int l = 1; l <= 2; ++l)
             if (p->fork_step[l] == i) RVA_HIP(p->ctx, hipEventRecord(p->fork_ev[l], lanes[0]));
         const Step &s = p->steps[i];
+        if (lazy && s.box_tail) continue;
         if (s.lane && !started[s.lane]) {
             RVA_HIP(p->ctx, hipStreamWaitEvent(lanes[s.lane], p->fork_ev[s.lane], 0));
             started[s.lane] = true;
         }
-        const int rc = launch_step(p, s, s.variant, input, output, n, (rva_stream_t)lanes[s.lane], win);
+        const int rc = launch_step(p, s, s.variant, input, output, n, (rva_stream_t)lanes[s.lane], step_win(p, s, n, win));
         if (rc != RVA_OK) return rc;
     }
     for (int l = 1; l <= 2; ++l)
@@ -765,8 +828,8 @@
             RVA_HIP(p->ctx, hipEventRecord(p->join_ev[l], lanes[l]));
             RVA_HIP(p->ctx, hipStreamWaitEvent(lanes[0], p->join_ev[l], 0));
         }
-    note_complete_run(p, n, win, stream);
-    return RVA_OK;
-}
-
-}
+    note_complete_run(p, n, win, lazy, stream);
+    return RVA_OK;
+}
+
+}
diff --git a/realtime_video_analytics_32streams_amd/csrc/rva_postprocess.hip b/realtime_video_analytics_32streams_amd/csrc/rva_postprocess.hip
--- a/realtime_video_analytics_32streams_amd/csrc/rva_postprocess.hip
+++ b/realtime_video_analytics_32streams_amd/csrc/rva_postprocess.hip
@@ -31,7 +31,9 @@
 __device__ __forceinline__ float ldf(const float *p) { return *p; }
 __device__ __forceinline__ float ldf(const __half *p) { return __half2float(*p); }
 
-template <typename T, bool SPLIT>
+enum { K2_FUSED = 0, K2_SCORE = 1, K2_BOX = 2 };
+
+template <typename T, bool SPLIT, int PART = K2_FUSED>
 __device__ __forceinline__ void k2_body(const K2Args &a, const float *boxes)
 {
     const int b = blockIdx.y;
@@ -40,8 +42,11 @@
     bool pass = false, odd = false;
     if (anchor < a.A) {
         const T *p = (const T *)a.raw + (long)b * a.sb + (long)anchor * a.sa;
-        float best;
+        float best = 0.f;
         int bi = 0;
+        if constexpr (PART == K2_BOX) {
+            pass = (a.bits[(long)b * a.nwords + (anchor >> 5)] >> (anchor & 31)) & 1u;
+        } else {
         if (a.C > 5) {
             const float obj = ldf(p + 4 * a.sc);
             best = ldf(p + 5 * a.sc) * obj;
@@ -55,7 +60,13 @@
         }
         pass = best >= a.thr;
         if (a.use_cls) pass = pass && bi < 1024 && ((a.cls_mask[bi >> 5] >> (bi & 31)) & 1u);
-        if (pass) {
+        }
+        if (pass && PART != K2_BOX) {
+            const long o = (long)b * a.A + anchor;
+            a.sp_score[o] = best;
+            a.sp_cls[o] = bi;
+        }
+        if (pass && PART != K2_SCORE) {
             const PostMeta m = a.meta[b];
             float cx, cy, w, h;
             if constexpr (SPLIT) {
@@ -72,12 +83,11 @@
             y1 = fminf(fmaxf(y1, 0.0f), m.ymax); y2 = fminf(fmaxf(y2, 0.0f), m.ymax);
             const long o = (long)b * a.A + anchor;
             a.sp_box[o] = make_float4(x1, y1, x2, y2);
-            a.sp_score[o] = best;
-            a.sp_cls[o] = bi;
             odd = !(x1 <= x2) || !(y1 <= y2);
         }
     }
     if (__any(odd) && lane == 0) atomicOr(a.irr + b, 1);
+    if constexpr (PART == K2_BOX) return;
     const unsigned long long mask = __ballot(pass);
     const int a0 = blockIdx.x * 256 + (threadIdx.x & ~63);
     if (lane < 2) {
@@ -91,6 +101,9 @@
 
 template <typename T>
 __global__ void __launch_bounds__(256) k2_decode_split(K2Args a, const float *boxes) { k2_body<T, true>(a, boxes); }
+
+__global__ void __launch_bounds__(256) k2_score(K2Args a) { k2_body<__half, false, K2_SCORE>(a, nullptr); }
+__global__ void __launch_bounds__(256) k2_box(K2Args a) { k2_body<__half, false, K2_BOX>(a, nullptr); }
 
 __device__ __forceinline__ float iou32(const float4 a, const float4 b)
 {
@@ -755,6 +768,17 @@
         return RVA_OK;
     }
     if (C - 5 > 1024 && n_classes > 0) return rva_fail(ctx, RVA_ERR_ARG, "class filter supports at most 1024 classes");
+    const rva_lazy_head *lazy = nullptr;
+    if (!boxes) {
+        const auto it = ctx->lazy_heads.find(raw);
+        if (it != ctx->lazy_heads.end()) {
+            lazy = &it->second;
+            if (raw_dtype != RVA_F16 || !channel_major || batch > lazy->n || A != lazy->A || C != 4 + lazy->nc)
+                return rva_fail(ctx, RVA_ERR_ARG, "rva_postprocess_batch: this head has pending box rows (a lazy plan run of %d images, [%d, %d] "
+                                                  "fp16) and was passed as %d x [%d, %d]%s", lazy->n, 4 + lazy->nc, lazy->A, batch, d1, d2,
+                                raw_dtype == RVA_F16 ? "" : " fp32");
+        }
+    }
     int rc = rva_reserve(ctx, batch, A);
     if (rc != RVA_OK) return rc;
 
@@ -794,6 +818,17 @@
             const float *bx = boxes + (size_t)b0 * 4 * A;
             if (raw_dtype == RVA_F16) k2_decode_split<__half><<<g2, 256, 0, stream>>>(k2, bx);
             else k2_decode_split<float><<<g2, 256, 0, stream>>>(k2, bx);
+        }
+        else if (lazy) {
+            k2_score<<<g2, 256, 0, stream>>>(k2);
+            rva_box_level lv[3];
+            for (int l = 0; l < 3; ++l) {
+                lv[l] = lazy->lv[l];
+                lv[l].x = (const char *)lv[l].x + (size_t)b0 * lv[l].H * lv[l].W * lv[l].ldx * 2;
+            }
+            rc = rva_box_tail_launch(ctx, lv, 3, ctx->cand_bits, nwords, nb, const_cast<void *>(k2.raw), lazy->nc, A, stream);
+            if (rc != RVA_OK) return rc;
+            k2_box<<<g2, 256, 0, stream>>>(k2);
         }
         else if (raw_dtype == RVA_F16) k2_decode<__half><<<g2, 256, 0, stream>>>(k2);
         else k2_decode<float><<<g2, 256, 0, stream>>>(k2);
diff --git a/realtime_video_analytics_32streams_amd/detector.py b/realtime_video_analytics_32streams_amd/detector.py
--- a/realtime_video_analytics_32streams_amd/detector.py
+++ b/realtime_video_analytics_32streams_amd/detector.py
@@ -105,6 +105,7 @@
         self._post: Optional[ops.PostBuffers] = None
         self._in: Optional[torch.Tensor] = None
         self._slot = 0
+        self._lazy_call = False
         if config.warmup and self.net is not None:
             with torch.inference_mode():
                 self._infer(torch.zeros((1, 3, *self.input_hw), device=self.device,
@@ -201,13 +202,14 @@
         plan.set_static_rows(*self._rows[n])
         self._rows_told[n] = True
 
-    def _infer(self, tensor: torch.Tensor):
+    def _infer(self, tensor: torch.Tensor, lazy_boxes: bool = False):
         if self._infer_fn is not None:
             return self._infer_fn(tensor)
         if self.half:
             if tensor.dtype != torch.float16:
                 raise TypeError("half detector: the fused plan takes the fp16 tensor K1 writes")
             plan = self.plan_for(tensor)
+            plan.lazy_boxes = lazy_boxes or self._lazy_call
             if not torch.cuda.is_current_stream_capturing():
                 self._tell_rows(plan, tensor)
             plan(tensor.contiguous())
@@ -234,10 +236,19 @@
     def stage_pre(self, packets: Sequence[FramePacket]):
         return self._preprocess([p.frame for p in packets])
 
+    def _infer_then_post(self, tensor: torch.Tensor):
+        self._lazy_call = True
+        try:
+            return self._infer(tensor)
+        finally:
+            self._lazy_call = False
+
     def stage_net(self, pre):
-        return self._infer(pre[0])
+        return self._infer_then_post(pre[0])
 
     def stage_post(self, raw, pre) -> ops.PostBuffers:
+        if self.engine == "fused" and isinstance(raw, torch.Tensor):
+            any(plan.expect_lazy_boxes(raw) for plan in self._plans.values())
         return self._postprocess_device(raw, [pre[1]])
 
     @staticmethod
@@ -251,7 +262,7 @@
             raise ValueError("predict_batch_device needs one frame geometry per call; use predict_batch for mixed sizes")
         with torch.inference_mode():
             tensor, meta = self._preprocess([p.frame for p in packets])
-            raw = self._infer(tensor)
+            raw = self._infer_then_post(tensor)
             return self._postprocess_device(raw, [meta])
 
     def predict_batch(self, packets: Sequence[FramePacket]) -> List[List[Detection]]:
diff --git a/realtime_video_analytics_32streams_amd/engine.py b/realtime_video_analytics_32streams_amd/engine.py
--- a/realtime_video_analytics_32streams_amd/engine.py
+++ b/realtime_video_analytics_32streams_amd/engine.py
@@ -167,6 +167,21 @@
     def primed(self) -> bool:
         return self.primed_images >= self.n
 
+    @property
+    def lazy_boxes(self) -> bool:
+        return bool(self.L.rva_yolov8_plan_get_lazy_boxes(self.handle))
+
+    @lazy_boxes.setter
+    def lazy_boxes(self, on: bool) -> None:
+        self.ctx.check(self.L.rva_yolov8_plan_set_lazy_boxes(self.handle, int(bool(on))), "rva_yolov8_plan_set_lazy_boxes")
+
+    def expect_lazy_boxes(self, head: torch.Tensor) -> bool:
+        if not any(o.data_ptr() == head.data_ptr() for o in self._outs.values()):
+            return False
+        self.ctx.check(self.L.rva_yolov8_plan_expect_lazy_boxes(self.handle, C.c_void_p(head.data_ptr()), int(head.shape[0])),
+                       "rva_yolov8_plan_expect_lazy_boxes")
+        return True
+
     def step_rows(self, step: int) -> Tuple[int, int]:
         y0, y1 = C.c_int32(), C.c_int32()
         self.ctx.check(self.L.rva_yolov8_plan_step_rows(self.handle, int(step), C.byref(y0), C.byref(y1)), "rva_yolov8_plan_step_rows")
```
